# PolyChord/PolyChordLite

Measured on AMD Instinct MI355X. Metric: likelihood evals/sec, 20D Gaussian nlive=2000, higher is better.
Workload: dtype f64; 1 GPU; configs[1]: 20-D Gaussian, nlive=2000, num_repeats=40, one full run per step; batch_chains=1000, parallelism=repeat-sharded x1, mode=one run at a time per GPU; R runs in step: roofline.in_step

## Files before the change

include/polychord_hip.h:

```cpp
#ifndef POLYCHORD_HIP_H
#define POLYCHORD_HIP_H
#include <stdbool.h>
#ifdef __cplusplus
extern "C" {
#endif


typedef double (*polychord_loglike_fn)(double *theta, int nDims, double *phi, int nDerived);
typedef void (*polychord_prior_fn)(double *cube, double *theta, int nDims);
typedef void (*polychord_dumper_fn)(int ndead, int nlive, int npars, double *live, double *dead,
                                    double *logweights, double logZ, double logZerr);

void polychord_c_interface(
    polychord_loglike_fn loglikelihood, polychord_prior_fn prior, polychord_dumper_fn dumper,
    int nlive, int num_repeats, int nprior, int nfail, bool do_clustering, int feedback,
    double precision_criterion, double logzero, int max_ndead, double boost_posterior,
    bool posteriors, bool equals, bool cluster_posteriors, bool write_resume, bool write_paramnames,
    bool read_resume, bool write_stats, bool write_live, bool write_dead, bool write_prior,
    bool maximise, double compression_factor, bool synchronous, int nDims, int nDerived,
    char *base_dir, char *file_root, int nGrade, double *grade_frac, int *grade_dims, int n_nlives,
    double *loglikes, int *nlives, int seed, int *comm);

void polychord_c_interface_ini(polychord_loglike_fn loglikelihood, void (*setup_loglikelihood)(void),
                               char *inifile, int *comm);


enum { PCHIP_LIKE_CALLBACK = 0, PCHIP_LIKE_GAUSSIAN = 1, PCHIP_LIKE_RASTRIGIN = 2,
       PCHIP_LIKE_TWIN_GAUSSIAN = 3, PCHIP_LIKE_CORR_GAUSSIAN = 4, PCHIP_LIKE_SOURCE = 5 };

double polychord_hip_gaussian(double *theta, int nDims, double *phi, int nDerived);
double polychord_hip_rastrigin(double *theta, int nDims, double *phi, int nDerived);
double polychord_hip_twin_gaussian(double *theta, int nDims, double *phi, int nDerived);
double polychord_hip_corr_gaussian(double *theta, int nDims, double *phi, int nDerived);
void polychord_hip_set_gaussian(double mu, double sigma);
void polychord_hip_set_corr_gaussian(int nDims, const double *invcov_rowmajor, const double *mean, double logdetcov);
void polychord_hip_uniform_prior(double *cube, double *theta, int nDims);
void polychord_hip_set_uniform_prior(int nDims, const double *lo, const double *hi);
enum { PCHIP_PT_UNIFORM = 1, PCHIP_PT_LOG_UNIFORM = 2, PCHIP_PT_POWER_UNIFORM = 3, PCHIP_PT_GAUSSIAN = 4, PCHIP_PT_HALF_GAUSSIAN = 5,
       PCHIP_PT_EXPONENTIAL = 6, PCHIP_PT_SORTED_UNIFORM = 7, PCHIP_PT_SORTED_GAUSSIAN = 8, PCHIP_PT_SORTED_HALF_GAUSSIAN = 9,
       PCHIP_PT_SORTED_EXPONENTIAL = 10 };
typedef struct {
    int type;
    int block;
    int npar;
    double par[3];
} pchip_prior_entry;
void polychord_hip_table_prior(double *cube, double *theta, int nDims);
int  polychord_hip_set_table_prior(int nDims, const pchip_prior_entry *entries, const int *hyper);
typedef void (*polychord_batch_fn)(void *user, int n, int nDims, int nDerived, const double *cube, double *theta, double *phi,
                                   double *logL);
void polychord_hip_set_batch_callback(polychord_batch_fn fn, void *user);
void polychord_hip_request_stop(void);
int polychord_hip_resume_copy(const char *in, const char *out, int *counts);
int polychord_hip_ini_prior(const char *inifile, const double *cube, double *theta, int n);
double polychord_hip_inv_normal_cdf(double p);
void polychord_hip_set_option(const char *name, double value);
void polychord_hip_set_sub_clustering(int n, const int *dims);
int polychord_hip_ini_sub_clustering(const char *inifile, int *dims, int cap);
const char *polychord_hip_last_error(void);
void pchip_inject_fault(int kind);
void pchip_set_capacity(int clusters, int phantom_rows);
void pchip_trim_cache(void);

typedef struct {
    int nDims, nDerived;
    int nlive, num_repeats, nprior, nfail;
    int do_clustering;
    double precision_criterion, logzero;
    int max_ndead;
    double boost_posterior;
    int posteriors, equals, cluster_posteriors;
    double compression_factor;
    int n_nlives; const double *loglikes; const int *nlives;
    int seed;
    int batch;
    int device;
    int feedback;
    int profile;
    int force_general;
    int ablate;
    const char *resume_write;
    int sequential_rng;
    const char *resume_read;
    int nGrade; const int *grade_dims; const int *grade_repeats;
    int epoch_discard;
    int device_records;
    int n_sub_cluster; const int *sub_cluster_dims;
} pchip_settings;

typedef struct {
    int kind;
    double mu, sigma;
    const double *invcov;
    const double *mean;
    double logdetcov;
    polychord_loglike_fn fn;
    int source;
} pchip_like;

enum { PCHIP_PRIOR_CALLBACK = 0, PCHIP_PRIOR_BOX = 1, PCHIP_PRIOR_TABLE = 2, PCHIP_PRIOR_SOURCE = 3 };
typedef struct {
    int kind;
    const double *lo, *hi;
    polychord_prior_fn fn;
    const pchip_prior_entry *table;
    const int *hyper;
} pchip_prior;

typedef struct {
    double logZ, varlogZ;
    long ndead, nlike, niter, nbatches, nrounds, nupdates;
    int ncluster, ncluster_dead, nTotal, batch;
    double t_generate, t_loop, t_final, t_total;
    double t_setup, t_results, t_teardown;
    double k_time_s[8]; long k_launches[8];
    double *dead, *logweights;
    double *entry;
    double *live; int nlive_final;
    double *logZp, *varlogZp; int nZp;
    double *post_mean, *post_var;
    long nlike_grade[8];
    int *live_cluster;
    long nlike_failed;
    int ncluster_peak;
    int epoch_discard;
    double *d_records; long n_records, records_cap; int records_device;
    long path[24];
} pchip_result;
enum { PCHIP_PATH_CONSUME_PAR = 0,
       PCHIP_PATH_CONSUME_CL = 1,
       PCHIP_PATH_CONSUME_GENERAL = 2,
       PCHIP_PATH_CONSUME_FAST = 3,
       PCHIP_PATH_KILLOFF_PAR = 4, PCHIP_PATH_KILLOFF_CL = 5, PCHIP_PATH_KILLOFF_GENERAL = 6, PCHIP_PATH_KILLOFF_FAST = 7,
       PCHIP_PATH_UPDATE_FUSED = 8,
       PCHIP_PATH_UPDATE_STEPS = 9,
       PCHIP_PATH_SLICE_WAVE = 10,
       PCHIP_PATH_SLICE_LANE = 11,
       PCHIP_PATH_NN_LISTS = 12,
       PCHIP_PATH_NN_FALLBACKS = 13,
       PCHIP_PATH_POOL_MODE = 14,
       PCHIP_PATH_DEFER_UPDATE = 15,
       PCHIP_PATH_CONSUME_CL_SERIAL = 16,
       PCHIP_PATH_SUBCLUSTER_PASSES = 17,
       PCHIP_PATH_SUBCLUSTER_SPLITS = 18,
       PCHIP_PATH_SOURCE_KERNELS = 19,
       PCHIP_PATH_DEVICE_PRIOR = 20,
       PCHIP_PATH_SOURCE_TERMS = 21,
       PCHIP_PATH_SLICE_STEP = 22,
       PCHIP_PATH_COUNT = 24 };

typedef struct {
    int final_call;
    long ndiscarded;
    long ndead; int nlive, npars;
    const double *dead;
    const double *logpost;
    const double *live;
    const int *live_cluster;
    double logZ, logZerr;
    long nlike;
    int ngrade; const long *nlike_grade; const int *grade_dims, *grade_repeats;
    int ncluster, ncluster_dead;
    const int *nlive_p;
    const double *logZp, *logZperr;
    const double *logZp_dead, *logZperr_dead;
    const unsigned *dead_cluster;
    const unsigned *cluster_uid, *cluster_uid_dead;
    int nsplit;
    const unsigned *split_child, *split_parent;
    const double *split_logfrac;
    int n_extra; const double *extra, *extra_logpost; const unsigned *extra_cluster;
    const unsigned long long *extra_uid;
} pchip_update;
typedef void (*pchip_update_fn)(void *user, const pchip_update *u);

typedef struct {
    polychord_dumper_fn dumper;
    pchip_update_fn on_update;
    void *user;
} pchip_hooks;

#define PCHIP_ABI_VERSION 9
int  pchip_abi_version(void);
#define PCHIP_SOURCE_MAX_DERIVED 32
int  pchip_source_create(const char *source, const char *options, const double *data, long ndata);
void pchip_source_destroy(int handle);
int  pchip_source_create_terms(const char *source, const char *options, const double *data, long ndata, long nterms);
int  pchip_source_create_prior(const char *source, const char *options, const double *data, long ndata, long nterms);
int  pchip_source_prior_eval(int handle, const double *cubes, long n, int nDims, double *thetas);
int  pchip_source_eval(int handle, const double *thetas, long n, int nDims, int nDerived, double *logL, double *phi);
unsigned long pchip_sizeof(const char *struct_name);
void pchip_settings_default(pchip_settings *s, int nDims, int nDerived);
int  pchip_device_count(void);
int  pchip_run(const pchip_settings *s, const pchip_like *like, const pchip_prior *prior, pchip_result *out);
int  pchip_run_hooks(const pchip_settings *s, const pchip_like *like, const pchip_prior *prior,
                     const pchip_hooks *hooks, pchip_result *out);
void pchip_result_free(pchip_result *r);
int  pchip_maximise(polychord_loglike_fn loglikelihood, polychord_prior_fn prior, int nDims, int nDerived, double logzero,
                    const double *live, const int *live_cluster, int nlive, const double *post_mean, const char *path);
typedef struct {
    double logZ, varlogZ;
    long n; int nTotal, nruns;
    double *rows;
    double *logweights;
    int *nlive;
    double *post_mean, *post_var;
    double t_merge_s, t_runs_s;
    long nlike, ndead_all;
    double runs_logZ_mean, runs_logZ_sem;
    double logZ_replay, varlogZ_replay;
    int evidence_rule, nclustered;
} pchip_merged;
int  pchip_merge_records(int nDims, int nDerived, int nruns, const long *counts, const double *rows, const double *entry,
                         int on_device, int want_rows, pchip_merged *out);
int  pchip_merge_records_ex(int nDims, int nDerived, int nruns, const long *counts, const double *rows, const double *entry,
                            const double *ownw, const double *run_logZ, const double *run_varlogZ, const int *run_clustered,
                            int on_device, int want_rows, pchip_merged *out);
void pchip_merged_free(pchip_merged *m);
int  pchip_merged_write(const pchip_merged *m, int nDims, int nDerived, const char *base_dir, const char *file_root);
int  pchip_run_repeats(const pchip_settings *s, const pchip_like *like, const pchip_prior *prior, int nseeds, const int *seeds,
                       int ndevices, const int *devices, int max_in_flight, pchip_result *results, pchip_merged *merged);
int  pchip_run_repeats_ex(const pchip_settings *s, const pchip_like *like, const pchip_prior *prior, int nseeds, const int *seeds,
                          int ndevices, const int *devices, int max_in_flight, int want_rows, pchip_result *results, pchip_merged *merged);
int  pchip_run_in_step(const pchip_settings *s, const pchip_like *like, const pchip_prior *prior, int nseeds, const int *seeds,
                       int ndevices, const int *devices, int max_in_flight, int want_rows, pchip_result *results, pchip_merged *merged);

typedef struct pchip_comm pchip_comm;
#define PCHIP_COMM_ID_BYTES 128
int  pchip_comm_get_id(char *id128);
int  pchip_comm_create(const char *id128, int nranks, int rank, int device, pchip_comm **out);
void pchip_comm_destroy(pchip_comm *c);
int  pchip_comm_merge(pchip_comm *c, const pchip_result *run, double logzero, int nDims, int nDerived, int want_rows,
                      pchip_merged *out);
int  pchip_comm_merge_many(pchip_comm *c, const pchip_result *runs, int nruns, double logzero, int nDims, int nDerived, int want_rows,
                           pchip_merged *out);
typedef int (*pchip_allgather_fn)(void *user, const void *send, void *recv, unsigned long bytes);
int  pchip_comm_create_with(pchip_allgather_fn all_gather, void *user, int nranks, int rank, int device, pchip_comm **out);
const char *pchip_comm_library(void);

int  pchip_slice_chains(const pchip_settings *s, const pchip_like *like, const pchip_prior *prior,
                        unsigned batch, int nchains, const double *seeds, const double *chol,
                        double contour, double *babies_out, double *nhats_out, int *nlike_out);
int  pchip_prior_transform(const pchip_prior *prior, int nDims, int n, const double *cube, double *theta, int device);
int  pchip_update_factors(const pchip_settings *s, int ncluster, int nlive, const double *live, const int *live_cluster,
                          int nph, const double *phantom, const double *ph_logL, const int *ph_cluster, const double *threshold,
                          const double *shift, int path, double *cov, double *chol, int *count, double *shift_out, int *chol_suspect);

#ifdef __cplusplus
}
#endif
#endif
```

polychordlite_amd/_ctypes_api.py:

```python
import ctypes as C
import os

import numpy as np

_HERE = os.path.dirname(os.path.abspath(__file__))
LIB_PATH = os.environ.get("PCHIP_LIB") or os.path.join(_HERE, "libpolychord_hip.so")

LOGLIKE_FN = C.CFUNCTYPE(C.c_double, C.POINTER(C.c_double), C.c_int, C.POINTER(C.c_double), C.c_int)
PRIOR_FN = C.CFUNCTYPE(None, C.POINTER(C.c_double), C.POINTER(C.c_double), C.c_int)
DUMPER_FN = C.CFUNCTYPE(None, C.c_int, C.c_int, C.c_int, C.POINTER(C.c_double), C.POINTER(C.c_double),
                        C.POINTER(C.c_double), C.c_double, C.c_double)

LIKE_CALLBACK, LIKE_GAUSSIAN, LIKE_RASTRIGIN, LIKE_TWIN_GAUSSIAN, LIKE_CORR_GAUSSIAN, LIKE_SOURCE = range(6)
KERNEL_CLASSES = ("k_nhats", "k_slice", "k_consume", "k_apply", "k_clean", "k_covmats", "k_bases_side")
LIKE_KINDS = {"gaussian": LIKE_GAUSSIAN, "rastrigin": LIKE_RASTRIGIN, "twin_gaussian": LIKE_TWIN_GAUSSIAN,
              "corr_gaussian": LIKE_CORR_GAUSSIAN, "source": LIKE_SOURCE}


class Settings(C.Structure):
    _fields_ = [("nDims", C.c_int), ("nDerived", C.c_int), ("nlive", C.c_int), ("num_repeats", C.c_int),
                ("nprior", C.c_int), ("nfail", C.c_int), ("do_clustering", C.c_int),
                ("precision_criterion", C.c_double), ("logzero", C.c_double), ("max_ndead", C.c_int),
                ("boost_posterior", C.c_double), ("posteriors", C.c_int), ("equals", C.c_int),
                ("cluster_posteriors", C.c_int), ("compression_factor", C.c_double), ("n_nlives", C.c_int),
                ("loglikes", C.POINTER(C.c_double)), ("nlives", C.POINTER(C.c_int)), ("seed", C.c_int),
                ("batch", C.c_int), ("device", C.c_int), ("feedback", C.c_int), ("profile", C.c_int),
                ("force_general", C.c_int), ("ablate", C.c_int),
                ("resume_write", C.c_char_p), ("sequential_rng", C.c_int), ("resume_read", C.c_char_p),
                ("nGrade", C.c_int), ("grade_dims", C.POINTER(C.c_int)), ("grade_repeats", C.POINTER(C.c_int)),
                ("epoch_discard", C.c_int), ("device_records", C.c_int),
                ("n_sub_cluster", C.c_int), ("sub_cluster_dims", C.POINTER(C.c_int))]


class Like(C.Structure):
    _fields_ = [("kind", C.c_int), ("mu", C.c_double), ("sigma", C.c_double), ("invcov", C.POINTER(C.c_double)),
                ("mean", C.POINTER(C.c_double)), ("logdetcov", C.c_double), ("fn", C.c_void_p),
                ("source", C.c_int)]


class PriorEntry(C.Structure):
    _fields_ = [("type", C.c_int), ("block", C.c_int), ("npar", C.c_int), ("par", C.c_double * 3)]


class Prior(C.Structure):
    _fields_ = [("kind", C.c_int), ("lo", C.POINTER(C.c_double)), ("hi", C.POINTER(C.c_double)), ("fn", C.c_void_p),
                ("table", C.POINTER(PriorEntry)), ("hyper", C.POINTER(C.c_int))]


PRIOR_CALLBACK, PRIOR_BOX, PRIOR_TABLE, PRIOR_SOURCE = 0, 1, 2, 3
PRIOR_TYPES = {"uniform": 1, "log_uniform": 2, "power_uniform": 3, "gaussian": 4, "half_gaussian": 5, "exponential": 6,
               "sorted_uniform": 7, "sorted_gaussian": 8, "sorted_half_gaussian": 9, "sorted_exponential": 10}


class Result(C.Structure):
    _fields_ = [("logZ", C.c_double), ("varlogZ", C.c_double), ("ndead", C.c_long), ("nlike", C.c_long),
                ("niter", C.c_long), ("nbatches", C.c_long), ("nrounds", C.c_long), ("nupdates", C.c_long),
                ("ncluster", C.c_int), ("ncluster_dead", C.c_int), ("nTotal", C.c_int), ("batch", C.c_int),
                ("t_generate", C.c_double), ("t_loop", C.c_double), ("t_final", C.c_double), ("t_total", C.c_double),
                ("t_setup", C.c_double), ("t_results", C.c_double), ("t_teardown", C.c_double),
                ("k_time_s", C.c_double * 8), ("k_launches", C.c_long * 8),
                ("dead", C.POINTER(C.c_double)), ("logweights", C.POINTER(C.c_double)), ("entry", C.POINTER(C.c_double)),
                ("live", C.POINTER(C.c_double)), ("nlive_final", C.c_int),
                ("logZp", C.POINTER(C.c_double)), ("varlogZp", C.POINTER(C.c_double)), ("nZp", C.c_int),
                ("post_mean", C.POINTER(C.c_double)), ("post_var", C.POINTER(C.c_double)),
                ("nlike_grade", C.c_long * 8), ("live_cluster", C.POINTER(C.c_int)),
                ("nlike_failed", C.c_long), ("ncluster_peak", C.c_int), ("epoch_discard", C.c_int),
                ("d_records", C.c_void_p), ("n_records", C.c_long), ("records_cap", C.c_long), ("records_device", C.c_int),
                ("path", C.c_long * 24)]


PATH_NAMES = ("consume_par", "consume_cl", "consume_general", "consume_fast", "killoff_par", "killoff_cl", "killoff_general",
              "killoff_fast", "update_fused", "update_steps", "slice_wave", "slice_lane", "nn_lists", "nn_fallbacks", "pool_mode",
              "defer_update", "consume_cl_serial", "subcluster_passes", "subcluster_splits", "source_kernels", "device_prior", "source_terms", "slice_step")


_lib = None


def load():
    global _lib
    if _lib is not None:
        return _lib
    if not os.path.exists(LIB_PATH):
        raise ImportError(f"{LIB_PATH} is missing: build it with `python -m polychordlite_amd.build` "
                          "(hipcc --offload-arch=gfx950).  There is no CPU fallback.")
    lib = C.CDLL(LIB_PATH, mode=C.RTLD_GLOBAL)
    lib.pchip_settings_default.argtypes = [C.POINTER(Settings), C.c_int, C.c_int]
    lib.pchip_settings_default.restype = None
    lib.pchip_device_count.restype = C.c_int
    lib.pchip_run.argtypes = [C.POINTER(Settings), C.POINTER(Like), C.POINTER(Prior), C.POINTER(Result)]
    lib.pchip_run.restype = C.c_int
    lib.pchip_result_free.argtypes = [C.POINTER(Result)]
    lib.pchip_result_free.restype = None
    lib.pchip_slice_chains.argtypes = [C.POINTER(Settings), C.POINTER(Like), C.POINTER(Prior), C.c_uint, C.c_int,
                                       C.POINTER(C.c_double), C.POINTER(C.c_double), C.c_double,
                                       C.POINTER(C.c_double), C.POINTER(C.c_double), C.POINTER(C.c_int)]
    lib.pchip_slice_chains.restype = C.c_int
    lib.polychord_hip_set_gaussian.argtypes = [C.c_double, C.c_double]
    lib.polychord_hip_set_uniform_prior.argtypes = [C.c_int, C.POINTER(C.c_double), C.POINTER(C.c_double)]
    lib.polychord_hip_set_corr_gaussian.argtypes = [C.c_int, C.POINTER(C.c_double), C.POINTER(C.c_double), C.c_double]
    lib.polychord_hip_set_option.argtypes = [C.c_char_p, C.c_double]
    lib.polychord_hip_set_sub_clustering.argtypes = [C.c_int, C.POINTER(C.c_int)]
    lib.polychord_hip_set_sub_clustering.restype = None
    lib.polychord_hip_ini_sub_clustering.argtypes = [C.c_char_p, C.POINTER(C.c_int), C.c_int]
    lib.polychord_hip_ini_sub_clustering.restype = C.c_int
    lib.pchip_source_create.argtypes = [C.c_char_p, C.c_char_p, C.POINTER(C.c_double), C.c_long]
    lib.pchip_source_create.restype = C.c_int
    lib.pchip_source_create_terms.argtypes = [C.c_char_p, C.c_char_p, C.POINTER(C.c_double), C.c_long, C.c_long]
    lib.pchip_source_create_terms.restype = C.c_int
    lib.pchip_source_create_prior.argtypes = [C.c_char_p, C.c_char_p, C.POINTER(C.c_double), C.c_long, C.c_long]
    lib.pchip_source_create_prior.restype = C.c_int
    lib.pchip_source_prior_eval.argtypes = [C.c_int, C.POINTER(C.c_double), C.c_long, C.c_int, C.POINTER(C.c_double)]
    lib.pchip_source_prior_eval.restype = C.c_int
    lib.pchip_source_eval.argtypes = [C.c_int, C.POINTER(C.c_double), C.c_long, C.c_int, C.c_int, C.POINTER(C.c_double), C.POINTER(C.c_double)]
    lib.pchip_source_eval.restype = C.c_int
    lib.pchip_source_destroy.argtypes = [C.c_int]
    lib.pchip_source_destroy.restype = None
    lib.pchip_rtc_embedded_source.argtypes = [C.c_int, C.POINTER(C.c_char_p)]
    lib.pchip_rtc_embedded_source.restype = C.c_char_p
    lib.pchip_rtc_compile_check.argtypes = [C.c_int, C.c_char_p, C.c_char_p, C.c_char_p, C.c_int, C.POINTER(C.c_double)]
    lib.pchip_rtc_compile_check.restype = C.c_int
    lib.pchip_rtc_stats.argtypes = [C.POINTER(C.c_long), C.POINTER(C.c_double)]
    lib.pchip_rtc_stats.restype = None
    lib.polychord_hip_last_error.restype = C.c_char_p
    lib.polychord_hip_set_table_prior.argtypes = [C.c_int, C.POINTER(PriorEntry), C.POINTER(C.c_int)]
    lib.polychord_hip_set_table_prior.restype = C.c_int
    lib.polychord_hip_table_prior.argtypes = [C.POINTER(C.c_double), C.POINTER(C.c_double), C.c_int]
    lib.polychord_hip_table_prior.restype = None
    lib.pchip_prior_transform.argtypes = [C.POINTER(Prior), C.c_int, C.c_int, C.POINTER(C.c_double), C.POINTER(C.c_double), C.c_int]
    lib.pchip_prior_transform.restype = C.c_int
    pi = C.POINTER(C.c_int); pd = C.POINTER(C.c_double)
    lib.pchip_update_factors.argtypes = [C.POINTER(Settings), C.c_int, C.c_int, pd, pi, C.c_int, pd, pd, pi, pd, pd, C.c_int, pd, pd, pi, pd, pi]
    lib.pchip_update_factors.restype = C.c_int
    lib.pchip_sizeof.argtypes = [C.c_char_p]
    lib.pchip_sizeof.restype = C.c_ulong
    for name, cls in (("settings", Settings), ("result", Result), ("like", Like), ("prior", Prior)):
        if lib.pchip_sizeof(name.encode()) != C.sizeof(cls):
            raise ImportError(f"{LIB_PATH}: pchip_{name} is {lib.pchip_sizeof(name.encode())} bytes, this binding's mirror {C.sizeof(cls)} "
                              f"(library ABI version {lib.pchip_abi_version()}): rebuild with `python -m polychordlite_amd.build`")
    _lib = lib
    return lib


def dptr(a):
    return a.ctypes.data_as(C.POINTER(C.c_double))


def source_create(source, options=(), data=None, nterms=None, prior=False):
    lib = load()
    d = None if data is None else np.ascontiguousarray(np.ravel(data), dtype=np.float64)
    opts = " ".join(options) if not isinstance(options, str) else options
    args = (source.encode(), opts.encode(), dptr(d) if d is not None and d.size else None, 0 if d is None else int(d.size))
    if prior:
        h = lib.pchip_source_create_prior(*args, 0 if nterms is None else int(nterms))
    else:
        h = lib.pchip_source_create(*args) if nterms is None else lib.pchip_source_create_terms(*args, int(nterms))
    if h <= 0:
        log = lib.polychord_hip_last_error()
        raise RuntimeError("device source does not compile:\n" + (log.decode(errors="replace") if log else "(no log)"))
    return h


def source_eval(handle, thetas, nDerived=0):
    lib = load()
    t = np.ascontiguousarray(np.atleast_2d(thetas), dtype=np.float64)
    logL = np.empty(t.shape[0])
    phi = np.empty((t.shape[0], nDerived))
    rc = lib.pchip_source_eval(handle, dptr(t), t.shape[0], t.shape[1], nDerived, dptr(logL), dptr(phi) if nDerived > 0 else None)
    if rc != 0:
        msg = lib.polychord_hip_last_error()
        raise RuntimeError(f"pchip_source_eval failed with code {rc}" + (": " + msg.decode(errors="replace") if rc == 1 and msg else ""))
    return logL, phi


def source_prior_eval(handle, cubes):
    lib = load()
    c = np.ascontiguousarray(np.atleast_2d(cubes), dtype=np.float64)
    th = np.empty_like(c)
    rc = lib.pchip_source_prior_eval(handle, dptr(c), c.shape[0], c.shape[1], dptr(th))
    if rc != 0:
        msg = lib.polychord_hip_last_error()
        raise RuntimeError(f"pchip_source_prior_eval failed with code {rc}" + (": " + msg.decode(errors="replace") if rc == 1 and msg else ""))
    return th


def prior_table(entries, hyper=None):
    arr = (PriorEntry * len(entries))()
    for i, e in enumerate(entries):
        t, block, pars = (e[0], 1, e[1]) if len(e) == 2 else e
        pars = [float(v) for v in np.atleast_1d(pars)]
        arr[i].type = PRIOR_TYPES[t] if isinstance(t, str) else int(t)
        arr[i].block, arr[i].npar = int(block), len(pars)
        for k, v in enumerate(pars[:3]):
            arr[i].par[k] = v
    hy = None if hyper is None else np.ascontiguousarray(hyper, dtype=np.int32)
    return arr, hy


def set_table_prior(entries, hyper=None):
    lib = load()
    arr, hy = prior_table(entries, hyper)
    if lib.polychord_hip_set_table_prior(len(arr), arr, hy.ctypes.data_as(C.POINTER(C.c_int)) if hy is not None else None) != 0:
        msg = lib.polychord_hip_last_error()
        raise ValueError(msg.decode(errors="replace") if msg else "prior table refused")


def table_prior(cube):
    lib = load()
    c = np.ascontiguousarray(cube, dtype=np.float64)
    th = np.empty_like(c)
    lib.polychord_hip_table_prior(dptr(c), dptr(th), int(c.size))
    return th


def prior_transform(entries, cubes, hyper=None, device=-1):
    lib = load()
    c = np.ascontiguousarray(np.atleast_2d(cubes), dtype=np.float64)
    th = np.empty_like(c)
    arr, hy = prior_table(entries, hyper)
    P = Prior()
    P.kind, P.table = PRIOR_TABLE, arr
    if hy is not None:
        P.hyper = hy.ctypes.data_as(C.POINTER(C.c_int))
    rc = lib.pchip_prior_transform(C.byref(P), c.shape[1], c.shape[0], dptr(c), dptr(th), device)
    if rc != 0:
        msg = lib.polychord_hip_last_error()
        raise RuntimeError(f"pchip_prior_transform failed with code {rc}" + (": " + msg.decode(errors="replace") if rc == 1 and msg else ""))
    return th


def update_factors(live, live_cluster, phantom, ph_logL, ph_cluster, threshold, path, shift=None, ablate=0, device=-1):
    lib = load()
    x = np.ascontiguousarray(np.atleast_2d(live), dtype=np.float64)
    D = x.shape[1]
    ph = np.ascontiguousarray(np.reshape(phantom, (-1, D)), dtype=np.float64)
    lc = np.ascontiguousarray(live_cluster, dtype=np.int32)
    pl = np.ascontiguousarray(ph_logL, dtype=np.float64)
    pc = np.ascontiguousarray(ph_cluster, dtype=np.int32)
    thr = np.ascontiguousarray(np.atleast_1d(threshold), dtype=np.float64)
    nc = thr.size
    assert lc.shape == (x.shape[0],) and pl.shape == (ph.shape[0],) and pc.shape == (ph.shape[0],)
    sh = None if shift is None else np.ascontiguousarray(shift, dtype=np.float64)
    assert sh is None or sh.shape == (D,)
    s = Settings(); lib.pchip_settings_default(C.byref(s), D, 0)
    s.ablate, s.device = ablate, device
    cov = np.full((nc, D, D), np.nan); chol = np.full((nc, D, D), np.nan)
    count = np.full(nc, -1, dtype=np.int32); sho = np.full(D, np.nan); sus = C.c_int(-1)
    ip = lambda a: a.ctypes.data_as(C.POINTER(C.c_int))
    rc = lib.pchip_update_factors(C.byref(s), nc, x.shape[0], dptr(x), ip(lc), ph.shape[0], dptr(ph), dptr(pl), ip(pc), dptr(thr),
                                  dptr(sh) if sh is not None else None, path, dptr(cov), dptr(chol), ip(count), dptr(sho), C.byref(sus))
    if rc != 0:
        msg = lib.polychord_hip_last_error()
        raise RuntimeError(f"pchip_update_factors failed with code {rc}" + (": " + msg.decode(errors="replace") if rc == 1 and msg else ""))
    return dict(cov=cov, chol=chol, count=count, shift=sho, chol_suspect=sus.value)


def make_problem(kind, nDims, nDerived=0, lo=None, hi=None, mu=0.5, sigma=0.1, invcov=None, mean=None, logdet=0.0, source=0,
                 prior_table=None, hyper=None, prior_source=False):
    keep = []
    L = Like()
    L.kind = LIKE_KINDS[kind]
    L.source = source
    L.mu, L.sigma, L.logdetcov = mu, sigma, logdet
    if invcov is not None:
        ic = np.ascontiguousarray(invcov, dtype=np.float64)
        mn = np.ascontiguousarray(mean, dtype=np.float64)
        keep += [ic, mn]
        L.invcov, L.mean = dptr(ic), dptr(mn)
    P = Prior()
    P.kind = 1
    if prior_source:
        P.kind = PRIOR_SOURCE
        return L, P, keep
    if prior_table is not None:
        arr, hy = globals()["prior_table"](prior_table, hyper)
        keep += [arr, hy]
        P.kind, P.table = PRIOR_TABLE, arr
        if hy is not None:
            P.hyper = hy.ctypes.data_as(C.POINTER(C.c_int))
        return L, P, keep
    if lo is not None:
        lo_a = np.ascontiguousarray(np.broadcast_to(lo, (nDims,)), dtype=np.float64)
        hi_a = np.ascontiguousarray(np.broadcast_to(hi, (nDims,)), dtype=np.float64)
        keep += [lo_a, hi_a]
        P.lo, P.hi = dptr(lo_a), dptr(hi_a)
    return L, P, keep


def set_grades(settings, dims, repeats):
    gd = np.array(dims, dtype=np.int32)
    gr = np.array(repeats, dtype=np.int32)
    settings.nGrade = len(dims)
    settings.grade_dims = gd.ctypes.data_as(C.POINTER(C.c_int))
    settings.grade_repeats = gr.ctypes.data_as(C.POINTER(C.c_int))
    return gd, gr


def set_sub_clustering(settings, dims):
    sd = np.array(list(dims), dtype=np.int32)
    settings.n_sub_cluster = len(sd)
    settings.sub_cluster_dims = sd.ctypes.data_as(C.POINTER(C.c_int)) if len(sd) else None
    return sd


class _Owner:

    def __init__(self, lib, res):
        self.lib, self.res = lib, res

    def __del__(self):
        try:
            self.lib.pchip_result_free(C.byref(self.res))
        except Exception:
            pass


class _View:

    def __init__(self, owner, ptr, shape):
        self.owner = owner
        addr = C.cast(ptr, C.c_void_p).value or 0
        self.__array_interface__ = {"data": (addr, False), "shape": tuple(shape), "typestr": "<f8", "version": 3}


def _view(owner, ptr, shape):
    if int(np.prod(shape)) == 0:
        return np.zeros(shape)
    return np.asarray(_View(owner, ptr, shape))


def run(settings, like, prior):
    lib = load()
    r = Result()
    rc = lib.pchip_run(C.byref(settings), C.byref(like), C.byref(prior), C.byref(r))
    if rc != 0:
        raise RuntimeError(f"pchip_run failed with code {rc}")
    return result_dict(r, settings)


def result_dict(r, settings):
    lib = load()
    own = _Owner(lib, r)
    nT, nd, D = r.nTotal, r.ndead, settings.nDims
    out = dict(logZ=r.logZ, logZerr=float(np.sqrt(abs(r.varlogZ))), varlogZ=r.varlogZ, ndead=nd, nlike=r.nlike,
               niter=r.niter, nbatches=r.nbatches, nrounds=r.nrounds, nupdates=r.nupdates, ncluster=r.ncluster,
               ncluster_dead=r.ncluster_dead, nTotal=nT, batch=r.batch, t_generate=r.t_generate, t_loop=r.t_loop,
               t_final=r.t_final, t_total=r.t_total, t_setup=r.t_setup, t_results=r.t_results, t_teardown=r.t_teardown,
               kernel_time={n: {"total_s": r.k_time_s[i], "launches": r.k_launches[i]}
                            for i, n in enumerate(KERNEL_CLASSES) if r.k_launches[i] > 0},
               dead=_view(own, r.dead, (nd, nT)),
               logweights=_view(own, r.logweights, (nd,)),
               entry=_view(own, r.entry, (nd,)),
               live=_view(own, r.live, (r.nlive_final, nT)),
               logZp=np.ctypeslib.as_array(r.logZp, shape=(max(r.nZp, 1),))[:r.nZp].copy(),
               post_mean=np.ctypeslib.as_array(r.post_mean, shape=(D + settings.nDerived,)).copy(),
               post_var=np.ctypeslib.as_array(r.post_var, shape=(D + settings.nDerived,)).copy(),
               nlike_grade=[int(v) for v in r.nlike_grade], nlike_failed=r.nlike_failed, ncluster_peak=r.ncluster_peak, epoch_discard=r.epoch_discard, n_records=int(r.n_records) if r.d_records else None,
               path={n: int(r.path[i]) for i, n in enumerate(PATH_NAMES)},
               varlogZp=np.ctypeslib.as_array(r.varlogZp, shape=(max(r.nZp, 1),))[:r.nZp].copy(),
               logzero=settings.logzero,
               _owner=own)
    return out
```

polychordlite_amd/csrc/pc_engine.hip:

```cpp
#include "pc_state.h"
#include "pc_resume.h"
#include "pc_prior_table.h"
#include "pc_launch.h"
#include "pc_plan.h"
#include <cstdio>
#include <cstdlib>
#include <cstring>
#include <cstdarg>
#include <cstdint>
#include <new>
#include <cmath>
#include <vector>
#include <memory>
#include <string>
#include <chrono>
#include <algorithm>
#include <map>
#include <unordered_map>
#include <atomic>
#include <mutex>
#include <thread>
#include <functional>
#include <exception>
#include <ucontext.h>
// ... 212 lines not shown
    return two < 170e-6;
}
struct StreamClasses {
    std::mutex mm;
    std::map<void *, int> cls;
    std::vector<hipStream_t> reps;
    int known(hipStream_t x) { std::lock_guard<std::mutex> g(mm); auto it = cls.find((void *)x); return it == cls.end() ? -1 : it->second; }
    int classify(hipStream_t x)
    {
        std::lock_guard<std::mutex> g(mm);
        auto it = cls.find((void *)x);
        if (it != cls.end()) return it->second;
        int c = -1;
        for (size_t r = 0; r < reps.size() && c < 0; ++r) if (!streams_overlap_test(reps[r], x)) c = (int)r;
        if (c < 0) { c = (int)reps.size(); reps.push_back(x); }
        cls[(void *)x] = c;
        return c;
    }
};
static StreamClasses &sclasses() { static StreamClasses *p = new StreamClasses; return *p; }
static hipStream_t stream_avoiding(std::vector<int> avoid, bool known_only = false);
static hipStream_t stream_beside(std::initializer_list<hipStream_t> others, bool known_only = false)
{
    if (pc_env().side_pick_off) return hpool().get_stream();
    std::vector<int> avoid;
    for (hipStream_t o : others) if (o) { const int c = known_only ? sclasses().known(o) : sclasses().classify(o); if (c >= 0) avoid.push_back(c); }
    return stream_avoiding(avoid, known_only);
}
static hipStream_t stream_avoiding(std::vector<int> avoid, bool known_only)
{
    auto fits = [&](int c) { return c >= 0 && std::find(avoid.begin(), avoid.end(), c) == avoid.end(); };
    if (hipStream_t k = hpool().take_stream_if([&](hipStream_t x) { return fits(sclasses().known(x)); })) return k;
    if (known_only) {
        if (hipStream_t k = hpool().take_stream_if([&](hipStream_t x) { return sclasses().known(x) >= 0; })) return k;
        return hpool().get_stream();
    }
    std::vector<hipStream_t> tried;
    hipStream_t pick = nullptr;
    for (int k = 0; k < 8 && !pick; ++k) {
        hipStream_t c = hpool().take_stream_if([&](hipStream_t x) { return sclasses().known(x) < 0; });
        const bool dbg = pc_env().debug == 5;
        const auto q0 = std::chrono::steady_clock::now();
        const bool made = !c;
        if (!c) { HIPCHK(hipStreamCreate(&c)); }
        const auto q1 = std::chrono::steady_clock::now();
        const int cc = sclasses().classify(c);
        if (dbg) std::fprintf(stderr, "polychord_hip dbg stream_beside: try %d, %s stream %p (%.2f ms), class %d (%.2f ms), avoid %d\n", k, made ? "new" : "pooled", (void *)c, std::chrono::duration<double>(q1 - q0).count() * 1e3, cc, std::chrono::duration<double>(std::chrono::steady_clock::now() - q1).count() * 1e3, avoid.empty() ? -1 : avoid[0]);
        if (fits(cc)) pick = c; else tried.push_back(c);
    }
    if (!pick) { pick = tried.back(); tried.pop_back(); }
    for (hipStream_t t : tried) hpool().put_stream(t);
    return pick;
}
static hipStream_t side_stream_for(hipStream_t main_st) { return stream_beside({main_st}); }
struct CohortStreams {
    std::mutex m;
    std::vector<std::pair<int, int>> used;
    std::vector<int> busy(int dev, bool mains_only = false)
    {
        std::vector<int> b;
        for (auto &u : used) if (u.first == dev && (!mains_only || u.second >= 1000)) b.push_back(u.second % 1000);
        return b;
    }
    void take(int dev, int c, bool main_stream = false) { if (c >= 0) used.emplace_back(dev, c + (main_stream ? 1000 : 0)); }
    void give(int dev, int c, bool main_stream = false)
    {
        if (c < 0) return;
        const int v = c + (main_stream ? 1000 : 0);
        for (size_t i = 0; i < used.size(); ++i) if (used[i].first == dev && used[i].second == v) { used.erase(used.begin() + (long)i); return; }
    }
};
static CohortStreams &cstreams() { static CohortStreams *p = new CohortStreams; return *p; }
struct CohortLease {
    int dev, cls_main = -1, cls_side = -1; bool held = false;
    explicit CohortLease(int d) : dev(d) {}
    void hold(int cm, int cs) { cls_main = cm; cls_side = cs; held = true; }
    void release() { if (!held) return; held = false; std::lock_guard<std::mutex> gq(cstreams().m); cstreams().give(dev, cls_main, true); cstreams().give(dev, cls_side); }
    ~CohortLease() { release(); }
};
extern "C" void pc_prepare_streams(int dev, int want)
{
    if (hipSetDevice(dev) != hipSuccess) return;
    (void)hipDeviceSynchronize();
    std::lock_guard<std::mutex> gq(cstreams().m);
    std::vector<hipStream_t> have;
    while (hipStream_t k = hpool().take_stream_if([](hipStream_t x) { return sclasses().known(x) >= 0; })) have.push_back(k);
    for (int tries = 0; (int)have.size() < want && tries < 4 * want; ++tries) {
        hipStream_t c = hpool().take_stream_if([](hipStream_t x) { return sclasses().known(x) < 0; });
        if (!c && hipStreamCreate(&c) != hipSuccess) break;
        (void)sclasses().classify(c);
        have.push_back(c);
    }
    for (hipStream_t k : have) hpool().put_stream(k);
}
std::atomic<int> g_active_runs{0};
std::atomic<int> g_active_dev[64];

struct Timing { double t_gen = 0, t_loop = 0, t_final = 0, t_total = 0; long rounds = 0, updates = 0, batches = 0, compactions = 0; };

enum { KT_NHATS = 0, KT_SLICE, KT_CONSUME, KT_APPLY, KT_CLEAN, KT_COV, KT_SIDE , KT_N };
struct KTimer {
    bool on = false;
    unsigned mask = 0xFFFFFFFFu;
    unsigned stride = 1; unsigned seen[KT_N] = {0};
    hipStream_t st = nullptr;
    std::vector<hipEvent_t> pool; size_t used = 0;
    struct Span { int k; hipEvent_t a, b; bool side; };
    std::vector<Span> open;
    double total_ms[KT_N] = {0}; long launches[KT_N] = {0};
    hipEvent_t get() { if (used == pool.size()) pool.push_back(hpool().get_event()); return pool[used++]; }
    hipEvent_t begin(int k) { if (!on || !((mask >> k) & 1u) || (seen[k]++ % stride) != 0 || open.size() >= MAX_OPEN) return nullptr; hipEvent_t e = get(); HIPCHK(hipEventRecord(e, st)); return e; }
    void end(int k, hipEvent_t a) { if (!on || !a) return; hipEvent_t e = get(); HIPCHK(hipEventRecord(e, st)); open.push_back({k, a, e, false}); }
    hipEvent_t begin_on(int k, hipStream_t s2) { if (!on || !((mask >> k) & 1u) || (seen[k]++ % stride) != 0 || open.size() >= MAX_OPEN) return nullptr; hipEvent_t e = get(); HIPCHK(hipEventRecord(e, s2)); return e; }
    void end_on(int k, hipEvent_t a, hipStream_t s2) { if (!on || !a) return; hipEvent_t e = get(); HIPCHK(hipEventRecord(e, s2)); open.push_back({k, a, e, true}); }
    static constexpr size_t MAX_OPEN = 8192;
    void collect() {
        if (!on) return;
        for (auto &sp : open) { float ms = 0; if (sp.side) HIPCHK(hipEventSynchronize(sp.b)); HIPCHK(hipEventElapsedTime(&ms, sp.a, sp.b)); total_ms[sp.k] += ms; launches[sp.k]++; }
        open.clear(); used = 0;
    }
    void destroy() { for (auto e : pool) hpool().put_event(e); pool.clear(); }
};

static void h_philox(uint32_t c0, uint32_t c1, uint32_t c2, uint32_t c3, uint32_t k0, uint32_t k1, uint32_t o[4])
{
    for (int r = 0; r < 10; ++r) {
        const uint64_t p0 = (uint64_t)0xD2511F53u * c0, p1 = (uint64_t)0xCD9E8D57u * c2;
        const uint32_t n0 = (uint32_t)(p1 >> 32) ^ c1 ^ k0, n1 = (uint32_t)p1, n2 = (uint32_t)(p0 >> 32) ^ c3 ^ k1, n3 = (uint32_t)p0;
        c0 = n0; c1 = n1; c2 = n2; c3 = n3; k0 += 0x9E3779B9u; k1 += 0xBB67AE85u;
    }
    o[0] = c0; o[1] = c1; o[2] = c2; o[3] = c3;
}
static double h_uniform(uint32_t k0, uint32_t k1, uint32_t dom, uint32_t shi, uint32_t slo, uint32_t idx)
{
    uint32_t o[4];
    h_philox(idx >> 1, slo, shi, dom, k0, k1, o);
    const uint64_t w = (idx & 1u) ? (((uint64_t)o[2] << 32) | o[3]) : (((uint64_t)o[0] << 32) | o[1]);
    return ((double)(w >> 11) + 0.5) * (1.0 / 9007199254740992.0);
}

#include "pc_fiber.h"

#include "pc_cohort.h"

#include "pc_split.h"

struct DbgSpan {
    std::atomic<long long> &ns; std::chrono::steady_clock::time_point t0 = std::chrono::steady_clock::now();
    ~DbgSpan() { ns += std::chrono::duration_cast<std::chrono::nanoseconds>(std::chrono::steady_clock::now() - t0).count(); }
};
static std::atomic<long long> g_dbg_compact_ns{0}, g_dbg_nursery_ns{0}, g_dbg_capacity_ns{0}, g_dbg_endb_ns{0}, g_dbg_destroy_ns{0}, g_dbg_evwait_ns{0}, g_dbg_d1{0}, g_dbg_d2{0};
struct Engine {
    Cohort *co = nullptr;
    Fiber *fib = nullptr;
    pchip_settings cfg{};
    std::atomic<int> stop{0};
    polychord_batch_fn batch_fn = nullptr; void *batch_user = nullptr;
    polychord_loglike_fn cb_like = nullptr; polychord_prior_fn cb_prior = nullptr;
    bool callback_mode = false;
    void *d_cs = nullptr; double *d_x0s = nullptr, *d_prop = nullptr;
    int *d_decks = nullptr;
    double *hp_prop = nullptr, *hp_ans = nullptr, *d_ans = nullptr; int *hp_need = nullptr;
    long long cb_evals = 0; long cb_ticks = 0;
    std::vector<int> cb_idx; std::vector<double> cb_c, cb_t, cb_p, cb_l;
    polychord_dumper_fn dumper = nullptr;
    pchip_update_fn on_update = nullptr; void *hook_user = nullptr;
    long ndiscarded = 0;
    bool resume_static = true; unsigned resume_batch0 = 0;
    bool nph_stale = false;
    std::vector<double> hm_dead, hm_logw; int hm_ndead = 0;
    std::vector<unsigned> hm_cuid;
    std::vector<double> pp_rows, pp_logpost; std::vector<unsigned> pp_cuid; std::vector<unsigned long long> pp_uid; int nd_last_update = 0;
    std::vector<unsigned> split_child, split_parent; std::vector<double> split_logfrac;
    std::vector<double> h_lo, h_hi;
    PcState S{};
    hipStream_t st = nullptr;
    hipStream_t st_copy = nullptr;
    bool st_copy_shared = false;
    hipStream_t st_side = nullptr;
    hipEvent_t ev_main = nullptr;
    static constexpr int RAW_RING = 4;
    struct RawSlot { hipEvent_t ready = nullptr, consumed = nullptr; unsigned batch = 0; int B = 0; bool valid = false, waited = false, used = false; int co_seq = 0; };
    RawSlot ring[RAW_RING];
    int raw_depth = 2;
    double *h_dead = nullptr; size_t h_dead_cap = 0, h_dead_copied = 0;
    PcCtl *h_ctl = nullptr;
    PcCtl *h_note = nullptr;
    unsigned note_seq = 0;
    hipEvent_t ev_apply = nullptr;
    double *raw_buf[RAW_RING] = {nullptr, nullptr, nullptr, nullptr};
    double *ph2 = nullptr, *phL2 = nullptr; unsigned *phC2 = nullptr; unsigned long long *phU2 = nullptr;
    unsigned char *keep = nullptr; int *blk = nullptr, *d_total = nullptr;
    double *psum = nullptr, *mean = nullptr, *pcov = nullptr; int *pcnt = nullptr, *count = nullptr;
    size_t cov_chunks_cap = 0;
    double *upd_part = nullptr, *upd_shift = nullptr; size_t upd_part_cap = 0;
    PcPriorTable ptab; bool have_ptab = false;
    double *d_lo = nullptr, *d_hi = nullptr, *d_invcovT = nullptr, *d_mean = nullptr, *d_src = nullptr;
    double *d_dynL = nullptr; int *d_dynN = nullptr; double *d_logn = nullptr;
    ClusterUpdate<Engine> clus{*this};
    Engine() = default; Engine(const Engine &) = delete; Engine &operator=(const Engine &) = delete;
    std::vector<int> sub_dims; int *c_subdims = nullptr;
    long nsplits = 0; int ncluster_peak = 1;
    bool src_terms = false;
    long path[PCHIP_PATH_COUNT] = {};
    Cohort::Note step_note;
    Timing tm;
    KTimer kt;
    int B = 0, dev = 0;
    bool cb_auto_batch = false; int B_small = 1; double cb_eval_seconds = -1.0;
    long long nlike_g[PC_MAX_GRADE] = {0};
    std::vector<int> h_nlike_g;

    void alloc_phantom_side(int Pcap)
    {
        ph2 = dalloc<double>((size_t)Pcap * S.nT); phL2 = dalloc<double>(Pcap); phC2 = dalloc<unsigned>(Pcap);
        phU2 = dalloc<unsigned long long>(Pcap); keep = dalloc<unsigned char>(Pcap); blk = dalloc<int>((Pcap + 255) / 256 + 1);
    }

    std::vector<void *> setup_staged;
    void upload(void *dst, const void *src, size_t bytes)
    {
        void *h = halloc<char>(bytes);
        setup_staged.push_back(h);
        std::memcpy(h, src, bytes);
        HIPCHK(hipMemcpyAsync(dst, h, bytes, hipMemcpyHostToDevice, st));
    }
    void setup(const pchip_settings &c, const pchip_like &like, const pchip_prior &prior)
    {
        cfg = c;
        { std::lock_guard<std::mutex> g(g_cb_mutex); batch_fn = g_batch_fn; batch_user = g_batch_user; }
        int ndev = 0;
        if (hipGetDeviceCount(&ndev) != hipSuccess || ndev == 0) {
            engine_fail(PC_RC_DEVICE, "no HIP device available -- this engine has no CPU path");
        }
        dev = c.device >= 0 ? c.device % ndev : 0;
        HIPCHK(hipSetDevice(dev));
        st = co ? co->st : hpool().get_stream();
        st_copy = (co && co->stc[0]) ? co->stc[(co->n_stc++) & 1] : (co ? hpool().get_stream() : stream_beside({st}));
        st_copy_shared = co && co->stc[0];
        kt.on = c.profile != 0 && !co; kt.st = st;
        kt.mask = (c.profile == 1) ? 0xFFFFFFFFu : (((unsigned)c.profile >> 1) & 0x7Fu);
        kt.stride = std::max(1u, ((unsigned)c.profile >> 8) & 0xFFu);
        const int D = c.nDims, nDer = c.nDerived;
        S.D = D; S.nDer = nDer; S.nT = 2 * D + nDer + 2; S.nr = c.num_repeats; S.N = c.nlive;
        S.ngrade = 1; S.g_off[0] = 0; S.g_nr[0] = c.num_repeats;
        for (int g = 1; g < PC_MAX_GRADE; ++g) { S.g_off[g] = 0; S.g_nr[g] = 0; }
        if (c.nGrade > 1 && c.grade_dims && c.grade_repeats) {
            if (c.nGrade > PC_MAX_GRADE) engine_fail(PC_RC_SETTINGS, "at most %d parameter grades", PC_MAX_GRADE);
            S.ngrade = c.nGrade;
            int off = 0, tot = 0;
            for (int g = 0; g < c.nGrade; ++g) {
                if (c.grade_dims[g] < 1 || c.grade_repeats[g] < 1) engine_fail(PC_RC_SETTINGS, "every grade needs at least one parameter and one repeat");
                S.g_off[g] = off; off += c.grade_dims[g]; S.g_nr[g] = c.grade_repeats[g]; tot += c.grade_repeats[g];
            }
            if (off != D) engine_fail(PC_RC_SETTINGS, "grade_dims must sum to nDims");
            S.nr = tot; cfg.num_repeats = tot;
        }
        S.nb_total = 0; S.n_dev = 0;
        for (int g = 0, col = 0; g < PC_MAX_GRADE; ++g) {
            const int Dg = D - S.g_off[g];
            S.g_nb[g] = g < S.ngrade ? (S.g_nr[g] + Dg - 1) / Dg : 0;
            S.g_col0[g] = col; S.g_e0[g] = (int)S.n_dev;
            col += S.g_nr[g]; S.nb_total += S.g_nb[g]; S.n_dev += (unsigned)S.g_nb[g] * Dg * Dg;
        }
        sub_dims.clear();
        if (c.n_sub_cluster < 0 || (c.n_sub_cluster > 0 && !c.sub_cluster_dims)) engine_fail(PC_RC_SETTINGS, "n_sub_cluster = %d without a list of coordinates", c.n_sub_cluster);
        for (int k = 0; k < c.n_sub_cluster; ++k) {
            const int d = c.sub_cluster_dims[k];
            if (d < 0 || d >= D) engine_fail(PC_RC_SETTINGS, "sub-clustering coordinate %d out of range (nDims = %d; the indices are 0-based)", d, D);
            if (std::find(sub_dims.begin(), sub_dims.end(), d) != sub_dims.end()) engine_fail(PC_RC_SETTINGS, "sub-clustering coordinate %d given twice", d);
            sub_dims.push_back(d);
        }
        S.ch_nlike_g = nullptr;
        std::memset(nlike_g, 0, sizeof(nlike_g));
        S.p0 = D; S.d0 = 2 * D; S.b0 = 2 * D + nDer; S.l0 = S.b0 + 1;
        int nmax = c.nlive;
        for (int i = 0; i < c.n_nlives; ++i) nmax = std::max(nmax, c.nlives[i]);
        const int nprior = c.nprior <= 0 ? c.nlive : c.nprior;
        S.Ncap = std::max(nmax, nprior);
        B = c.batch > 0 ? c.batch : std::max(1, std::min(1024, c.nlive / 2));
        if (B > 65535) engine_fail(PC_RC_LIMIT, "batch = %d chains per nursery: at most 65535", B);
        if (c.sequential_rng) B = 1;
        cb_auto_batch = c.batch <= 0 && !c.sequential_rng && (like.kind == PC_LIKE_CALLBACK || (prior.kind != 1 && prior.kind != PCHIP_PRIOR_TABLE && prior.kind != PCHIP_PRIOR_SOURCE));
        if (cb_auto_batch) B_small = std::max(1, std::min(64, c.nlive / 4));
        S.B = B;
        S.maxc = c.do_clustering ? std::max(2, g_cap_clusters.load()) : 4;
        S.maxc_dead = 4096;
        S.Pcap = (int)std::min<long long>(2000000000LL / S.nT, 4LL * S.nr * S.Ncap + 4LL * B * S.nr + 1024);
        if (g_cap_phantoms.load() > 0) S.Pcap = std::max(g_cap_phantoms.load(), B * S.nr + 16);
        S.Dcap = 64 * S.Ncap + 4 * B + 1024;
        S.k0 = (uint32_t)c.seed; S.k1 = 0x504F4C59u;
        S.logzero = c.logzero; S.use_prec = c.precision_criterion > 0;
        S.log_prec = S.use_prec ? std::log(c.precision_criterion) : 0.0;
        S.log_cf = std::log(c.compression_factor);
        S.max_ndead = c.max_ndead; S.nfail = c.nfail <= 0 ? c.nlive : c.nfail;
        S.seed_override = 0; S.ablate = c.ablate; S.seq_mode = c.sequential_rng ? 1 : 0;
        S.epoch_discard = c.epoch_discard ? 1 : 0;
        if (S.seq_mode) { cfg.batch = 1; cfg.force_general = 1; }
        S.n_nlives = c.n_nlives;
        if (c.n_nlives > 0) {
            d_dynL = dalloc<double>(c.n_nlives); d_dynN = dalloc<int>(c.n_nlives);
            upload(d_dynL, c.loglikes, sizeof(double) * c.n_nlives);
            upload(d_dynN, c.nlives, sizeof(int) * c.n_nlives);
        }
        S.dyn_loglikes = d_dynL; S.dyn_nlives = d_dynN;
        S.like.kind = like.kind; S.like.mu = like.mu; S.like.sigma = like.sigma; S.like.logdetcov = like.logdetcov;
// ... 875 lines not shown
    void write_resume()
    {
        if (!cfg.resume_write) return;
        PcResume r;
        export_resume(r);
        std::string err;
        if (!pc_resume_write(cfg.resume_write, r, cfg.logzero, err)) engine_fail(PC_RC_RESUME, "%s", err.c_str());
        write_sidecar(std::string(cfg.resume_write) + ".hip", r.ndead, r.ncluster, r.ncluster_dead);
    }

    bool import_resume(const PcResume &r, std::string &err)
    {
        const int D = S.D, nT = S.nT, nc = r.ncluster, Ncap = S.Ncap;
        if (r.nDims != D || r.nDerived != S.nDer) { err = "resume file has different nDims / nDerived"; return false; }
        if (nc > S.maxc) grow_clusters(nc);
        if (r.ncluster_dead + nc + 8 > S.maxc_dead) grow_dead_clusters(2 * (r.ncluster_dead + nc + 8));
        const int maxc = S.maxc;
        int ntot = 0, nph = 0;
        for (int c = 0; c < nc; ++c) { ntot += r.nlive[c]; nph += r.nphantom[c]; }
        if (ntot > Ncap || (nc >= 1 && ntot < 1)) { err = "resume file: live point counts do not fit this run's settings"; return false; }
        if (nph + (long long)B * S.nr > S.Pcap) { h_ctl->nphantom = 0; grow_phantoms(nph + (long long)B * S.nr); }
        if ((long long)r.ndead + B + Ncap + 16 > S.Dcap) { h_ctl->ndead = 0; grow_dead(2 * (r.ndead + B + Ncap + 16)); }
        std::vector<double> rows((size_t)Ncap * nT, 0.0), lL(Ncap, PC_HUGE), entry(Ncap, cfg.logzero);
        std::vector<int> lc(Ncap, -1), lp(Ncap, 0), cl((size_t)maxc * Ncap, 0), cn(maxc, 0), imin(maxc, 0);
        std::vector<unsigned> uid(maxc, 0u);
        const Sidecar sc = cfg.resume_read ? read_sidecar(std::string(cfg.resume_read) + ".hip", r.ndead, nc, std::min(r.ncluster_dead, S.maxc_dead)) : Sidecar{};
        std::vector<double> logLp(maxc, cfg.logzero), lref(maxc, 0.0), lsum(maxc, 0.0);
        int slot = 0;
        for (int c = 0; c < nc; ++c) {
            cn[c] = r.nlive[c]; uid[c] = sc.ok ? sc.uid[c] : (unsigned)(c + 1);
            double lo = PC_HUGE, hi = -PC_HUGE;
            for (int k = 0; k < r.nlive[c]; ++k, ++slot) {
                const double *row = r.live[c].data() + (size_t)k * nT;
                std::memcpy(rows.data() + (size_t)slot * nT, row, sizeof(double) * nT);
                lL[slot] = row[S.l0]; lc[slot] = c; lp[slot] = k; entry[slot] = row[S.b0]; cl[(size_t)c * Ncap + k] = slot;
                if (row[S.l0] < lo) { lo = row[S.l0]; imin[c] = slot; }
                hi = std::max(hi, row[S.l0]);
            }
            logLp[c] = r.nlive[c] ? lo : cfg.logzero;
            lref[c] = r.nlive[c] ? hi : 0.0;
            for (int k = 0; k < r.nlive[c]; ++k) lsum[c] += std::exp(r.live[c][(size_t)k * nT + S.l0] - lref[c]);
        }
        ul(S.live, rows); ul(S.live_logL, lL); ul(S.live_entry, entry); ul(S.live_cluster, lc); ul(S.live_pos, lp);
        { std::vector<int> none(Ncap, -1); ul(S.slot_src, none); }
        ul(S.cl_list, cl); ul(S.cl_n, cn); ul(S.cl_uid, uid); ul(S.imin_slot, imin); ul(S.logLp, logLp); ul(S.lse_ref, lref); ul(S.lse_sum, lsum);
        auto put = [&](double *dst, const std::vector<double> &v) { std::vector<double> t(maxc, cfg.logzero); std::copy(v.begin(), v.end(), t.begin()); ul(dst, t); };
        put(S.logZp, r.logZp); put(S.logZXp, r.logZXp); put(S.logZp2, r.logZp2); put(S.logZpXp, r.logZpXp);
        { std::vector<double> t(maxc, 0.0); std::copy(r.logXp.begin(), r.logXp.end(), t.begin()); ul(S.logXp, t); }
        std::vector<double> xq((size_t)maxc * maxc, 0.0);
        for (int q = 0; q < nc; ++q) for (int p = 0; p < nc; ++p) xq[(size_t)p * maxc + q] = r.logXpXq[(size_t)q * nc + p];
        ul(S.XpXq, xq);
        std::vector<double> cov((size_t)maxc * D * D, 0.0), ch((size_t)maxc * D * D, 0.0);
        for (int c = 0; c < maxc; ++c) for (int a = 0; a < D; ++a) { cov[((size_t)c * D + a) * D + a] = 1.0; ch[((size_t)c * D + a) * D + a] = 1.0; }
        for (int c = 0; c < nc; ++c) for (int j = 0; j < D; ++j) for (int a = 0; a < D; ++a) {
            cov[((size_t)c * D + a) * D + j] = r.covmat[((size_t)c * D + j) * D + a];
            ch[((size_t)c * D + a) * D + j] = r.cholesky[((size_t)c * D + j) * D + a];
        }
        ul(S.cov, cov); ul(S.chol, ch);
        const int ncd = std::min(r.ncluster_dead, S.maxc_dead);
        { std::vector<double> a(r.logZp_dead.begin(), r.logZp_dead.begin() + ncd), b(r.logZp2_dead.begin(), r.logZp2_dead.begin() + ncd); ul(S.logZp_dead, a); ul(S.logZp2_dead, b); }
        if (sc.ok) ul(S.cl_uid_dead, sc.uid_dead);
        std::vector<double> ph((size_t)std::max(1, nph) * nT), phL(std::max(1, nph));
        std::vector<unsigned> phC(std::max(1, nph)); std::vector<unsigned long long> phU(std::max(1, nph));
        int j = 0;
        for (int c = 0; c < nc; ++c)
            for (int k = 0; k < r.nphantom[c]; ++k, ++j) {
                std::memcpy(ph.data() + (size_t)j * nT, r.phantom[c].data() + (size_t)k * nT, sizeof(double) * nT);
                phL[j] = ph[(size_t)j * nT + S.l0]; phC[j] = uid[c]; phU[j] = 0xFFFFFFFF00000000ull | (unsigned)j;
            }
        if (nph) { ul(S.phantom, ph); ul(S.ph_logL, phL); ul(S.ph_cuid, phC); ul(S.ph_uid, phU); }
        if (r.ndead) {
            ul(S.dead, r.dead); ul(S.dead_logw, r.logweights);
            std::vector<double> z(r.ndead, 0.0), en(r.ndead);
            for (int i = 0; i < r.ndead; ++i) en[i] = r.dead[(size_t)i * nT + S.b0];
            ul(S.dead_postX, z); ul(S.dead_postZ, z); ul(S.dead_entry, en);
            std::vector<unsigned> du(r.ndead, 0u);
            if (sc.ok) du = sc.dead_cuid;
            ul(S.dead_cuid, du);
        }
        PcCtl c0 = *h_ctl;
        c0.status = nc >= 1 ? PC_ST_RUNNING : PC_ST_DONE; c0.ncluster = nc; c0.ncluster_dead = ncd; c0.ndead = r.ndead; c0.nphantom = nph;
        c0.logZ = r.logZ; c0.logZ2 = r.logZ2; c0.logX_last_update = r.logX_last_update; c0.next_cluster_uid = sc.ok ? sc.next_uid : (unsigned)nc + 1;
        c0.nlike = 0;
        for (size_t g = 0; g < r.nlike.size(); ++g) { c0.nlike += r.nlike[g]; if (g >= 1 && g < PC_MAX_GRADE) nlike_g[g] = r.nlike[g]; }
        c0.nlike_device = c0.nlike; c0.i_nursery = 0; c0.failures = 0;
        HIPCHK(hipMemcpy(S.ctl, &c0, sizeof(PcCtl), hipMemcpyHostToDevice));
        *h_ctl = c0;
        return true;
    }

    struct ActiveRun {
        int d; std::atomic<int> *flag;
        ActiveRun(int dv, std::atomic<int> *f) : d(dv & 63), flag(f) { g_active_runs.fetch_add(1); g_active_dev[d].fetch_add(1); std::lock_guard<std::mutex> g(g_run_mutex); g_run_stop.push_back(flag); }
        ~ActiveRun() { g_active_runs.fetch_sub(1); g_active_dev[d].fetch_sub(1); std::lock_guard<std::mutex> g(g_run_mutex); g_run_stop.erase(std::find(g_run_stop.begin(), g_run_stop.end(), flag)); }
    };
    std::unique_ptr<ActiveRun> active_run;
    using clk = std::chrono::steady_clock;
    clk::time_point r_t0, r_t1, r_t2;
    unsigned r_batch = 0; bool r_sort_valid = false, r_fresh = false; int r_nursery_left = 0;
    PcRunPlan plan{};
    int r_rc = 0;

    int run(pchip_result *out)
    {
        int rc = begin();
        if (rc >= 0) return rc;
        while (true) {
            if (!round_enqueue()) break;
            while (!round_ready()) __builtin_ia32_pause();
            if (!round_finish()) break;
        }
        if (r_rc != 0) return r_rc;
        return end(out);
    }

    int begin()
    {
        active_run.reset(new ActiveRun(dev, &stop));
        r_t0 = clk::now();
        h_dead_cap = (size_t)S.Dcap; h_dead = halloc<double>(h_dead_cap * S.nT); h_dead_copied = 0;
        bool resumed = false;
        if (cfg.resume_read) {
            if (FILE *probe = std::fopen(cfg.resume_read, "r")) {
                std::fclose(probe);
                PcResume rs; std::string err;
                if (!pc_resume_read(cfg.resume_read, rs, err) || !import_resume(rs, err)) { std::fprintf(stderr, "polychord_hip: %s\n", err.c_str()); return 6; }
                resumed = true;
                int ntot = 0;
                for (int v : rs.nlive) ntot += v;
                if (ntot > cfg.nlive && rs.ncluster == 1) { pc_count(path, PcTrimLive{}); pc_launch_consume(&S, 2, 0, st); read_ctl(); ntot = cfg.nlive; }
                resume_static = (ntot == cfg.nlive);
                resume_batch0 = (unsigned)rs.ndead;
            }
        }
        if (!resumed) { if (callback_mode) generate_live_callback(); else generate_live(); }
        if (stop.load(std::memory_order_relaxed)) return 5;
        if (cb_auto_batch && !(cb_eval_seconds >= 0.0 && cb_eval_seconds < 2e-6)) { B = B_small; S.B = B; }
        r_t1 = clk::now();
        r_batch = resume_batch0;
        r_sort_valid = false;
        r_nursery_left = 0;
        make_plan();
        S.defer_update = plan.defer ? 1 : 0; S.pool = plan.pool ? 1 : 0;
        if (S.pool) {
            pool_cursor = h_ctl->nphantom;
            babies_own = S.babies;
            if (g_cap_phantoms.load() <= 0) {
                size_t free_b = 0, total_b = 0;
                (void)hipMemGetInfo(&free_b, &total_b);
                const double need = 2.0 * 2.0 * (double)S.Pcap * ((double)S.nT * 8.0 + 24.0);
                if (need < 0.4 * (double)free_b) grow_phantoms(2LL * S.Pcap);
            }
        }
        r_rc = 0;
        return -1;
    }

    void make_plan()
    {
        const int nprior0 = cfg.nprior <= 0 ? cfg.nlive : cfg.nprior;
        PcRunFacts f{};
        f.ablate = cfg.ablate; f.force_general = cfg.force_general;
        f.fixed_nlive = (cfg.n_nlives == 0) && (nprior0 >= cfg.nlive) && resume_static;
        f.par_fits = pc_par_fits(&S) != 0; f.fast_fits = pc_fast_fits(&S) != 0; f.fused_fits_one = pc_update_fused_ok(&S, 1) != 0;
        f.clustering = cfg.do_clustering != 0; f.boost = cfg.boost_posterior != 0.0;
        f.dumper = dumper != nullptr; f.on_update = on_update != nullptr; f.resume_write = cfg.resume_write != nullptr;
        f.seq_mode = S.seq_mode != 0; f.posteriors = cfg.posteriors || cfg.equals;
        f.callback = callback_mode;
        plan = pc_plan_run(f);
    }
    bool other_active() const { return g_active_dev[dev & 63].load(std::memory_order_relaxed) > 1; }
    bool cohort_general_ok() const
    {
        return !pc_env().cohort_general_off && S.ngrade <= 1 && !S.seq_mode && S.like.kind != PC_LIKE_CORR_GAUSSIAN && S.like.kind != PC_LIKE_CALLBACK;
    }
    PcNurseryFacts nursery_facts(unsigned batch) const
    {
        PcNurseryFacts f{};
        f.in_step = co != nullptr; f.other_active = other_active(); f.callback = callback_mode; f.D = S.D;
        f.ring = raw_buf[1] != nullptr;
        const RawSlot &rs = ring[batch % raw_depth];
        f.slot_ready = rs.valid && rs.batch == batch && rs.B == B;
        f.second_stream = co && co->st2 && raw_depth >= 2;
        f.splittable = pc_nhats_splittable(&S) != 0; f.fusable = pc_slice_fusable(&S) != 0; f.bases_t = pc_bases_t_ok(&S) != 0;
        f.slice_t = pc_slice_t_ok(&S, h_ctl->ncluster) != 0;
        f.cohort_general = cohort_general_ok();
        f.traits = launch_traits();
        return f;
    }
    bool enqueue_nursery()
    {
        unsigned &batch = r_batch; int &nursery_left = r_nursery_left;
        if (S.pool) {
            if (pool_cursor + (long long)B * S.nr > S.Pcap) pool_compact();
            S.pool_base = (int)pool_cursor; S.pool_rows = B * S.nr; S.babies = S.phantom + (size_t)pool_cursor * S.nT;
            pool_cursor += (long long)B * S.nr;
        }
        {
            hipEvent_t e0 = kt.begin(KT_NHATS);
            const PcNurseryChoice ch = pc_choose_nursery(plan, nursery_facts(batch));
            pc_count(path, ch);
            pc_count_step(path, ch);
            int bases_seq = 0;
            switch (ch.bases) {
            case PC_BASES_READY: case PC_BASES_PART1: case PC_BASES_PART1_STEP: {
                RawSlot &rs = ring[batch % raw_depth];
                S.nhat_raw = raw_buf[batch % raw_depth];
                if (ch.bases == PC_BASES_READY) { if (!rs.waited) HIPCHK(hipStreamWaitEvent(st, rs.ready, 0)); bases_seq = rs.co_seq; }
                else {
                    if (rs.valid) HIPCHK(hipStreamWaitEvent(st, rs.ready, 0));
                    if (ch.bases == PC_BASES_PART1_STEP) co->rec(rec_bases(S, batch, B));
                    else (void)pc_launch_nhats_part(&S, batch, B, 1, st, ch.packed ? 1 : 0);
                }
                rs.valid = false;
                if (ch.part2) { if (co) { co->flush(); co->wait_next(); } (void)pc_launch_nhats_part(&S, batch, B, 2, st, 0); }
                break;
            }
            case PC_BASES_NHATS_G: co->rec(rec_nhats_g(S, batch, B)); break;
            case PC_BASES_WHOLE:
                if (co) co->flush();
                if (pc_launch_nhats(&S, batch, B, st)) { std::fprintf(stderr, "polychord_hip: nDims unsupported\n"); r_rc = 3; return false; }
                break;
            }
            kt.end(KT_NHATS, e0);
            hipEvent_t e1 = kt.begin(KT_SLICE);
            switch (ch.sampler) {
            case PC_SAMPLER_CALLBACK:
                if (co) co->flush();
                slice_callback(batch);
                if (stop.load(std::memory_order_relaxed)) { r_rc = 5; return false; }
                break;
            case PC_SAMPLER_LANE: { Cohort::Rec r = rec_slice(S, batch, B, bases_seq); r.note = co ? &step_note : nullptr; (void)stage(r); break; }
            case PC_SAMPLER_WAVE_STEP: co->rec(rec_slice_g(S, batch, B, ch.fused, ch.fused ? bases_seq : 0, &step_note)); break;
            case PC_SAMPLER_WAVE:
                if (co) { co->flush(); co->wait_next(); }
                if (ch.fused ? pc_launch_slice_fused(&S, batch, B, st) : pc_launch_slice(&S, batch, B, st)) {
                    if (pc_rtc_wanted(&S) && pc_rtc_error()) { std::fprintf(stderr, "polychord_hip: %s\n", pc_rtc_error()); r_rc = 1; return false; }
                    std::fprintf(stderr, "polychord_hip: nDims unsupported\n"); r_rc = 3; return false;
                }
                break;
            }
            if (ch.ahead == PC_AHEAD_STEP) bases_ahead(batch);
            kt.end(KT_SLICE, e1);
            if (ch.ahead == PC_AHEAD_SIDE) side_prefetch(batch);
            if (S.ngrade > 1) HIPCHK(hipMemcpyAsync(h_nlike_g.data(), S.ch_nlike_g, sizeof(int) * h_nlike_g.size(), hipMemcpyDeviceToHost, st));
            batch++; tm.batches++;
            S.nn_valid = 0; nursery_left = B;
        }
        return true;
    }

    void bases_ahead(unsigned cur)
    {
        const unsigned x = cur + 1;
        RawSlot &rn = ring[x % raw_depth];
        if (rn.valid && rn.batch == x && rn.B == B) return;
        PcState S1 = S; S1.nhat_raw = raw_buf[x % raw_depth];
        co->rec(rec_bases_next(S1, x, B));
        rn.valid = true; rn.batch = x; rn.B = B; rn.waited = true; rn.co_seq = co->seq_for_next();
    }

    void ensure_side()
    {
        if (st_side) return;
        st_side = stream_beside({st, st_copy}); ev_main = hpool().get_sync_event();
        for (int r = 0; r < raw_depth; ++r) { ring[r].ready = hpool().get_sync_event(); ring[r].consumed = hpool().get_sync_event(); }
    }
    hipEvent_t ev_presort_a = nullptr, ev_presort_b = nullptr;
    bool presorted = false;
    void presort_live()
    {
        presorted = false;
        if (pc_env().presort_off || co || other_active() || callback_mode || S.seq_mode || !S.nn_list || h_ctl->ncluster < 2) return;
        ensure_side();
        if (!ev_presort_a) { ev_presort_a = hpool().get_sync_event(); ev_presort_b = hpool().get_sync_event(); }
        HIPCHK(hipEventRecord(ev_presort_a, st)); HIPCHK(hipStreamWaitEvent(st_side, ev_presort_a, 0));
        if (pc_launch_sort_live(&S, st_side) != 0) return;
        HIPCHK(hipEventRecord(ev_presort_b, st_side));
        presorted = true;
    }
    void side_prefetch(unsigned cur)
    {
        const unsigned batch = cur;
        {
        ensure_side();
        const bool side_free = pc_env().side_free || (S.D > 64 && !pc_env().side_ordered);
        RawSlot &cur = ring[batch % raw_depth];
        if (side_free) { HIPCHK(hipEventRecord(cur.consumed, st)); cur.used = true; }
        if (!side_free) { HIPCHK(hipEventRecord(ev_main, st)); HIPCHK(hipStreamWaitEvent(st_side, ev_main, 0)); }
        const unsigned xmax = batch + (unsigned)raw_depth - (side_free ? 0u : 1u);
        for (unsigned x = batch + 1; x <= xmax; ++x) {
            RawSlot &rs = ring[x % raw_depth];
            if (rs.valid && rs.batch == x && rs.B == B) continue;
            if (rs.valid) continue;
            if (rs.used) HIPCHK(hipStreamWaitEvent(st_side, rs.consumed, 0));
            PcState S1 = S; S1.nhat_raw = raw_buf[x % raw_depth];
            hipEvent_t es = kt.begin_on(KT_SIDE, st_side);
            (void)pc_launch_nhats_part(&S1, x, B, 1, st_side, (cfg.ablate & PC_ABL_BASES_PACKED) ? 1 : 0);
            kt.end_on(KT_SIDE, es, st_side);
            HIPCHK(hipEventRecord(rs.ready, st_side));
            rs.valid = true; rs.batch = x; rs.B = B; rs.waited = false;
        }
    }
    }

    PcContractFacts contract_facts(int nursery_left) const
    {
        PcContractFacts f{};
        f.ncluster = h_ctl->ncluster; f.nursery_left = nursery_left;
        f.in_step = co != nullptr; f.cohort_general = cohort_general_ok();
        f.nn_lists = S.nn_list && !pc_env().nn_lists_off; f.nn_valid = S.nn_valid != 0;
        f.cl_fits = f.ncluster > 1 && pc_consume_cl_fits(&S, f.ncluster) != 0;
        f.clp_fits = f.cl_fits && pc_consume_clp_fits(&S, f.ncluster) != 0;
        return f;
    }
    bool round_enqueue()
    {
        unsigned &batch = r_batch; bool &sort_valid = r_sort_valid; int &nursery_left = r_nursery_left;
        {
            if (h_ctl->status == PC_ST_DONE) return false;
            if (h_ctl->status == PC_ST_ERROR) { std::fprintf(stderr, "polychord_hip: device error %d\n", h_ctl->error); r_rc = 2; return false; }
            if (step_note.failed) {
                if (pc_rtc_wanted(&S) && pc_rtc_error()) { std::fprintf(stderr, "polychord_hip: %s\n", pc_rtc_error()); r_rc = 1; return false; }
                std::fprintf(stderr, "polychord_hip: nDims unsupported\n"); r_rc = 3; return false;
            }
            bool fresh_nursery = false;
            if (h_ctl->i_nursery == 0) {
                fresh_nursery = true;
                DbgSpan dbg_t{g_dbg_nursery_ns};
                if (plan.cl_ok) presort_live();
                if (!enqueue_nursery()) return false;
            }
            if (fresh_nursery) { DbgSpan dbg_t{g_dbg_capacity_ns}; ensure_capacity(); }
            hipEvent_t e2 = kt.begin(KT_CONSUME);
            int rc2 = 0;
            const PcContractChoice ch = pc_choose_contract(plan, contract_facts(nursery_left));
            pc_count(path, ch);
            launch_stamp();
            if (presorted && (co || !(h_ctl->ncluster > 1))) { HIPCHK(hipStreamWaitEvent(st, ev_presort_b, 0)); presorted = false; }
            switch (ch.kind) {
            case PC_CONTRACT_PAR:
                S.nn_valid = 0;
                if (!sort_valid) { rc2 = stage(rec_sort(S)); sort_valid = true; }
                rc2 = rc2 || stage(rec_consume(S));
                break;
            case PC_CONTRACT_FAST:
                if (co) co->flush();
                sort_valid = false; S.nn_valid = 0;
                rc2 = pc_launch_consume_fast(&S, 0, st); pc_launch_ph_prepare(&S, st);
                break;
            case PC_CONTRACT_CL_STEP:
                sort_valid = false;
                if (ch.want_nn) { co->rec(rec_nn(S, nursery_left)); S.nn_valid = 1; }
                co->rec(rec_sort(S));
                co->rec(rec_consume_cl(S, h_ctl->ncluster > 64));
                break;
            case PC_CONTRACT_CL: case PC_CONTRACT_GENERAL: {
                sort_valid = false;
                if (co) co->flush();
                bool sorted_now = false;
                if (presorted) { HIPCHK(hipStreamWaitEvent(st, ev_presort_b, 0)); sorted_now = fresh_nursery; presorted = false; }
                if (ch.want_nn) {
                    if (!sorted_now) sorted_now = pc_launch_sort_live(&S, st) == 0;
                    pc_launch_nn_lists(&S, nursery_left, sorted_now ? 1 : 0, st);
                    S.nn_valid = 1;
                }
                if (ch.kind == PC_CONTRACT_CL) rc2 = (sorted_now ? 0 : pc_launch_sort_live(&S, st)) || pc_launch_consume_cl(&S, h_ctl->ncluster, st);
                else rc2 = pc_launch_consume(&S, 0, (h_ctl->ncluster > 1) ? 1 : 0, st);
                break;
            }
            }
            if (rc2) { std::fprintf(stderr, "polychord_hip: nlive too large for the LDS-resident contraction\n"); r_rc = 4; return false; }
            kt.end(KT_CONSUME, e2);
            hipEvent_t e3 = kt.begin(KT_APPLY);
            (void)stage(rec_apply(S, batch - 1, B));
            kt.end(KT_APPLY, e3);
            if (st_side) { RawSlot &rs = ring[batch % raw_depth]; if (rs.valid && rs.batch == batch && !rs.waited) { HIPCHK(hipStreamWaitEvent(st, rs.ready, 0)); rs.waited = true; } }
            r_fresh = fresh_nursery;
            ready_spins = 0;
        }
        return true;
    }

    bool finish_may_wait() const
    {
        const bool upd = h_ctl->status == PC_ST_UPDATE || (h_ctl->upd_pending && h_ctl->status == PC_ST_RUNNING);
        return upd && pc_choose_update(plan, update_facts(1)).may_wait;
    }
    bool round_finish()
    {
        unsigned &batch = r_batch; int &nursery_left = r_nursery_left; const bool fresh_nursery = r_fresh;
        (void)batch;
        {
            if (fresh_nursery && h_ctl->status == PC_ST_DONE && h_ctl->i_nursery == B) tm.batches--;
            nursery_left = h_ctl->i_nursery;
            tally_grades();
            tm.rounds++;
            if (h_ctl->status == PC_ST_UPDATE || (h_ctl->upd_pending && h_ctl->status == PC_ST_RUNNING)) {
                do_update(h_ctl->status != PC_ST_UPDATE); h_ctl->status = PC_ST_RUNNING; h_ctl->upd_pending = 0;
                if ((size_t)h_ctl->ndead >= h_dead_copied + 4 * (size_t)cfg.nlive) {
                if (!ev_apply) ev_apply = hpool().get_sync_event();
                HIPCHK(hipEventRecord(ev_apply, st));
                stream_dead();
                }
            }
        }
        return true;
    }

    struct EndState {
        double *hlive = nullptr; int *hcl = nullptr; double *d_pmax = nullptr, *h_part = nullptr, *h_zp = nullptr;
        int nc_end = 0, ncd_max = 0, pmD = 0, pm_nb = 0, pm_pw = 0; clk::time_point t2;
    } es;
    hipStream_t st_fin = nullptr; hipEvent_t ev_fin = nullptr;
    void end_a(bool fused_final = false)
    {
        if (co && !fused_final) co->flush();
        bool &sort_valid = r_sort_valid;
        es.t2 = clk::now();
        st_fin = st;
        if (co && fused_final && !pc_env().cohort_final_aside_off && st_copy && st_copy != st && h_ctl->ncluster > 1) {
            ev_fin = hpool().get_sync_event();
            HIPCHK(hipEventRecord(ev_fin, st));
            HIPCHK(hipStreamWaitEvent(st_copy, ev_fin, 0));
            st_fin = st_copy;
        }
        hipStream_t st = st_fin;
        const int nT = S.nT;
        es.hlive = halloc<double>((size_t)S.Ncap * nT); es.hcl = halloc<int>(S.Ncap);
        HIPCHK(hipMemcpyAsync(es.hlive, S.live, sizeof(double) * (size_t)S.Ncap * nT, hipMemcpyDeviceToHost, st));
        HIPCHK(hipMemcpyAsync(es.hcl, S.live_cluster, sizeof(int) * S.Ncap, hipMemcpyDeviceToHost, st));
        es.nc_end = h_ctl->ncluster;
        if (h_ctl->ncluster == 0) {
        } else if (plan.par_ok && h_ctl->ncluster == 1) {
            path[PCHIP_PATH_KILLOFF_PAR]++;
            if (co && sort_valid) { co->rec(rec_final(S)); if (!fused_final) co->flush(); }
            else {
            if (!sort_valid) (void)pc_launch_sort_live(&S, st);
            (void)pc_launch_final_par(&S, st);
            }
        } else if (h_ctl->ncluster > 1 && pc_launch_killoff_cl(&S, h_ctl->ncluster, st) == 0) {
            path[PCHIP_PATH_KILLOFF_CL]++;
        } else if (plan.fast_ok && h_ctl->ncluster == 1 && pc_launch_consume_fast(&S, 1, st) == 0) path[PCHIP_PATH_KILLOFF_FAST]++;
        else { path[PCHIP_PATH_KILLOFF_GENERAL]++; pc_launch_consume(&S, 1, (h_ctl->ncluster > 1 && !S.seq_mode) ? 1 : 0, st); }
        if (!fused_final) end_a2();
    }
    void end_a2()
    {
        hipStream_t st = st_fin ? st_fin : this->st;
        es.pmD = S.D + S.nDer; es.pm_nb = pc_post_blocks(); es.pm_pw = 3 * es.pmD + 1;
        es.ncd_max = std::min(h_ctl->ncluster_dead + h_ctl->ncluster, S.maxc_dead);
        es.d_pmax = dalloc<double>(2 * (size_t)es.pm_nb); es.h_part = halloc<double>((size_t)es.pm_nb * es.pm_pw);
        es.h_zp = halloc<double>(2 * (size_t)std::max(1, es.ncd_max));
        pc_launch_post_moments(&S, -1, es.d_pmax, es.h_part, st);
        if (es.ncd_max > 0) {
            HIPCHK(hipMemcpyAsync(es.h_zp, S.logZp_dead, sizeof(double) * es.ncd_max, hipMemcpyDeviceToHost, st));
            HIPCHK(hipMemcpyAsync(es.h_zp + es.ncd_max, S.logZp2_dead, sizeof(double) * es.ncd_max, hipMemcpyDeviceToHost, st));
        }
        HIPCHK(hipMemcpyAsync(h_ctl, S.ctl, sizeof(PcCtl), hipMemcpyDeviceToHost, st));
        if (ev_fin) HIPCHK(hipEventRecord(ev_fin, st));
    }
    void end_wait_aside() { if (ev_fin) { HIPCHK(hipEventSynchronize(ev_fin)); hpool().put_sync_event(ev_fin); ev_fin = nullptr; } }
    int end(pchip_result *out) { end_a(); HIPCHK(hipStreamSynchronize(st)); end_wait_aside(); return end_b(out); }
    int end_b(pchip_result *out)
    {
        struct HostBuf { EndState &e; ~HostBuf() { if (e.hlive) hfree(e.hlive); if (e.hcl) hfree(e.hcl); e.hlive = nullptr; e.hcl = nullptr; } } hb{es};
        double *hlive = es.hlive; int *hcl = es.hcl; double *d_pmax = es.d_pmax, *h_part = es.h_part, *h_zp = es.h_zp;
        const int nc_end = es.nc_end, ncd_max = es.ncd_max, pmD = es.pmD, pm_nb = es.pm_nb, pm_pw = es.pm_pw, nT = S.nT;
        const auto t0 = r_t0, t1 = r_t1; auto t2 = es.t2;
        HIPCHK(hipGetLastError());
        nph_stale = false;
        kt.collect();
        if (cfg.boost_posterior != 0.0 && (cfg.posteriors || cfg.equals) && h_ctl->nphantom > 0) {
            pc_launch_clean(&S, h_ctl->nphantom, keep, blk, d_total, ph2, phL2, phC2, phU2, nullptr, st);
            collect_phantom_posteriors(h_ctl->nphantom);
        }
        call_dumper(1);
        write_resume();
        auto t3 = clk::now();
        tm.t_gen = std::chrono::duration<double>(t1 - t0).count();
        tm.t_loop = std::chrono::duration<double>(t2 - t1).count();
        tm.t_final = std::chrono::duration<double>(t3 - t2).count();
        tm.t_total = std::chrono::duration<double>(t3 - t0).count();
        std::memset(out, 0, sizeof(*out));
        out->logZ = std::max(-PC_HUGE, 2 * h_ctl->logZ - 0.5 * h_ctl->logZ2);
        out->varlogZ = h_ctl->logZ2 - 2 * h_ctl->logZ;
        out->ndead = h_ctl->ndead; out->nlike = h_ctl->nlike; out->niter = h_ctl->niter;
        out->nlike_failed = h_ctl->nlike_failed; out->ncluster_peak = ncluster_peak; out->epoch_discard = S.epoch_discard;
        path[PCHIP_PATH_NN_FALLBACKS] = (long)h_ctl->nn_fallbacks; path[PCHIP_PATH_POOL_MODE] = S.pool; path[PCHIP_PATH_DEFER_UPDATE] = S.defer_update;
        path[PCHIP_PATH_SLICE_STEP] = step_note.shared;
        for (int k = 0; k < PCHIP_PATH_COUNT; ++k) out->path[k] = path[k];
        grade_counts(out->nlike_grade);
        out->ncluster = nc_end; out->ncluster_dead = h_ctl->ncluster_dead; out->nbatches = tm.batches;
        out->nrounds = tm.rounds; out->nupdates = tm.updates; out->nTotal = nT; out->batch = B;
        out->t_generate = tm.t_gen; out->t_loop = tm.t_loop; out->t_final = tm.t_final; out->t_total = tm.t_total;
        for (int k = 0; k < KT_N; ++k) { out->k_time_s[k] = kt.total_ms[k] * 1e-3; out->k_launches[k] = kt.launches[k]; }
        const int dbg_lvl = pc_env().debug;
        if (dbg_lvl >= 3) std::fprintf(stderr, "polychord_hip dbg general: term %lld identify %lld kill+add %lld tail %lld cycles; %lld chains identified from the candidate lists, %lld of them fell back to the full search\n", h_ctl->gen_cyc[0], h_ctl->gen_cyc[1], h_ctl->gen_cyc[2], h_ctl->gen_cyc[3], h_ctl->nn_walks, h_ctl->nn_fallbacks);
        if (dbg_lvl == 4) std::fprintf(stderr, "polychord_hip dbg par: stage+search %lld rank-sort %lld accept %lld merge+slots %lld evidence %lld triggers %lld publish %lld cycles\n", h_ctl->dbg[0], h_ctl->dbg[1], h_ctl->dbg[2], h_ctl->dbg[3], h_ctl->dbg[4], h_ctl->dbg[5], h_ctl->dbg[6]);
        if (dbg_lvl == 4) std::fprintf(stderr, "polychord_hip dbg par: %lld evidence scans as pairs (terms beyond one scale)\n", h_ctl->dbg[7]);
        if (dbg_lvl == 4 && h_ctl->wave_cyc[0]) std::fprintf(stderr, "polychord_hip dbg clp (several clusters; the line above then reads: decisions | order of deaths + slots | counts + volumes | volume sum + step 0's phantoms | prefix sums + commit | waves 1-3 | write back | passes): wave 1 %lld wave 2 %lld wave 3 %lld phantom wave %lld cycles\n", h_ctl->wave_cyc[0], h_ctl->wave_cyc[1], h_ctl->wave_cyc[2], h_ctl->wave_cyc[3]);
        if (dbg_lvl == 2) std::fprintf(stderr, "polychord_hip dbg: loop cycles %lld passB %lld (%lld flushes) accept-steps %lld (%lld) ins-rescan %lld (%lld) reject-steps cycles %lld\n", h_ctl->dbg[0], h_ctl->dbg[1], h_ctl->dbg[4], h_ctl->dbg[2], h_ctl->dbg[3], h_ctl->dbg[5], h_ctl->dbg[6], h_ctl->dbg[7]);
        if ((size_t)h_ctl->ndead > h_dead_cap) {
            HIPCHK(hipStreamSynchronize(st_copy));
            hfree(h_dead); h_dead_cap = (size_t)h_ctl->ndead; h_dead = halloc<double>(h_dead_cap * nT); h_dead_copied = 0;
        }
        stream_dead();
        out->dead = h_dead; h_dead = nullptr;
        out->logweights = halloc<double>(std::max(1, h_ctl->ndead));
        HIPCHK(hipMemcpyAsync(out->logweights, S.dead_logw, sizeof(double) * h_ctl->ndead, hipMemcpyDeviceToHost, st_copy));
        out->entry = halloc<double>(std::max(1, h_ctl->ndead));
        HIPCHK(hipMemcpyAsync(out->entry, S.dead_entry, sizeof(double) * h_ctl->ndead, hipMemcpyDeviceToHost, st_copy));
        int nl = 0;
        for (int s = 0; s < S.Ncap; ++s) nl += hcl[s] >= 0;
        out->nlive_final = nl;
        out->live = (double *)std::malloc(sizeof(double) * (size_t)std::max(1, nl) * nT);
        out->live_cluster = (int *)std::malloc(sizeof(int) * (size_t)std::max(1, nl));
        for (int s = 0, k = 0; s < S.Ncap; ++s) if (hcl[s] >= 0) { std::memcpy(out->live + (size_t)k * nT, hlive + (size_t)s * nT, sizeof(double) * nT); out->live_cluster[k] = hcl[s]; k++; }
        const int ncd = std::min(h_ctl->ncluster_dead, S.maxc_dead);
        out->nZp = ncd;
        out->logZp = (double *)std::malloc(sizeof(double) * std::max(1, ncd));
        out->varlogZp = (double *)std::malloc(sizeof(double) * std::max(1, ncd));
        if (ncd > ncd_max) engine_fail(PC_RC_DEVICE, "more retired clusters (%d) than the final stage could have left (%d)", ncd, ncd_max);
        for (int i = 0; i < ncd; ++i) { const double zp = h_zp[i], zp2 = h_zp[ncd_max + i]; out->logZp[i] = 2 * zp - 0.5 * zp2; out->varlogZp[i] = zp2 - 2 * zp; }
        hfree(h_zp);
        const int D = pmD, nb = pm_nb, pw = pm_pw;
        out->post_mean = (double *)std::calloc(D, sizeof(double)); out->post_var = (double *)std::calloc(D, sizeof(double));
        double sw = 0.0;
        for (int b = 0; b < nb; ++b) {
            sw += h_part[(size_t)b * pw + 2 * D];
            for (int d = 0; d < D; ++d) { out->post_mean[d] += h_part[(size_t)b * pw + d]; out->post_var[d] += h_part[(size_t)b * pw + D + d]; }
        }
        for (int d = 0; d < D; ++d) {
            const double dm = out->post_mean[d] / sw;
            out->post_mean[d] = h_part[2 * D + 1 + d] + dm;
            out->post_var[d] = std::max(0.0, out->post_var[d] / sw - dm * dm);
        }
        dfree(d_pmax); hfree(h_part);
        long long *h_nrec = nullptr;
        if (cfg.device_records && h_ctl->ndead > 0) {
            const long long cap = h_ctl->ndead;
            double *blk_rec = (double *)pc_cache_dev_alloc(pc_records_block_bytes(cap, nT));
            if (!blk_rec) engine_fail(PC_RC_MEMORY, "no device memory for the run's records (%lld rows)", cap);
            h_nrec = halloc<long long>(1);
            if (pc_pack_lived_device(S.dead, S.dead_logw, S.dead_entry, cap, nT, cfg.logzero, blk_rec, cap, h_nrec, st_copy) != 0) { pc_cache_dev_free(blk_rec); hfree(h_nrec); engine_fail(PC_RC_DEVICE, "packing the run's records"); }
            out->d_records = blk_rec; out->records_cap = (long)cap; out->records_device = dev;
        }
        HIPCHK(hipStreamSynchronize(st_copy));
        if (h_nrec) { out->n_records = (long)*h_nrec; hfree(h_nrec); }
        active_run.reset();
        return 0;
    }

    void destroy(bool streams_idle = false)
    {
        active_run.reset();
        if (!streams_idle) {
        if (st) (void)hipStreamSynchronize(st);
        if (st_copy) (void)hipStreamSynchronize(st_copy);
        if (st_side) (void)hipStreamSynchronize(st_side);
        }
        const auto dq0 = std::chrono::steady_clock::now();
        std::vector<void *> blocks; blocks.reserve(160);
        struct Batch { std::vector<void *> &b; Batch(std::vector<void *> &v) : b(v) { tl_dfree_batch = &b; } ~Batch() { tl_dfree_batch = nullptr; dcache().put_many(b); b.clear(); } };
        {
        Batch batch_guard(blocks);
        if (raw_buf[0]) { S.nhat_raw = raw_buf[0]; for (int r = 1; r < RAW_RING; ++r) dfree(raw_buf[r]); raw_buf[0] = nullptr; }
        if (babies_own) { S.babies = babies_own; babies_own = nullptr; }
        double **dd[] = { &S.live, &S.live_logL, &S.logZp, &S.logXp, &S.logZXp, &S.logZp2, &S.logZpXp, &S.logLp, &S.XpXq,
                          &S.lse_ref, &S.lse_sum, &S.death_thr, &S.chol, &S.cov, &S.logZp_dead, &S.logZp2_dead, &S.phantom,
                          &S.ph_logL, &S.dead, &S.dead_logw, &S.dead_postX, &S.dead_postZ, &S.babies, &S.baby_logL, &S.baby_logL_T,
                          &S.ch_contour, &S.nhat, &S.nhat_w, &S.nhat_raw, &S.nhat_Ms, &S.ch_My, &S.live_entry, &S.dead_entry, &ph2, &phL2, &psum, &mean,
                          &pcov, &d_lo, &d_hi, &d_invcovT, &d_mean, &d_dynL, &d_src };
        for (auto p : dd) dfree(*p);
        int **ii[] = { &S.live_cluster, &S.live_pos, &S.cl_list, &S.cl_n, &S.imin_slot, &S.ch_cluster, &S.ch_epoch, &S.ch_nlike,
                       &S.ch_seed_slot, &S.slot_src, &S.slot_step, &S.slot_dead, &S.sort_slot, &blk, &d_total, &pcnt, &count, &d_dynN };
        for (auto p : ii) dfree(*p);
        { char *cs = (char *)d_cs; dfree(cs); d_cs = nullptr; }
        dfree(d_x0s); dfree(d_prop); dfree(d_ans); dfree(d_decks);
        if (hp_prop) { hfree(hp_prop); hp_prop = nullptr; } if (hp_ans) { hfree(hp_ans); hp_ans = nullptr; } if (hp_need) { hfree(hp_need); hp_need = nullptr; }
        dfree(upd_part); dfree(upd_shift); upd_part_cap = 0;
        clus.release(); dfree(c_subdims);
        for (void *h : staged_up) hfree(h);
        staged_up.clear();
        for (const Fetch &f : fetching) hfree(f.h);
        fetching.clear();
        dfree(d_logn); dfree(S.ch_nlike_g); dfree(S.nn_list); dfree(S.nn_slot_owner); dfree(S.nn_chain_slot); dfree(S.nn_pts); dfree(S.nn_code);
        unsigned **uu[] = { &S.cl_uid, &S.ph_cuid, &S.dead_cuid, &phC2, &S.cl_uid_dead };
        for (auto p : uu) dfree(*p);
        dfree(S.ph_uid); dfree(S.sort_key); dfree(S.plan); dfree(phU2); dfree(keep); dfree(S.ctl);
        }
        const auto dq1 = std::chrono::steady_clock::now();
        kt.destroy();
        if (h_dead) { hfree(h_dead); h_dead = nullptr; }
        for (void *h : setup_staged) hfree(h);
        setup_staged.clear();
        if (h_ctl) hfree(h_ctl); h_ctl = nullptr;
        if (h_note) hfree((void *)h_note); h_note = nullptr;
        if (ev_apply) { hpool().put_sync_event(ev_apply); ev_apply = nullptr; }

        if (st) { if (!streams_idle) (void)hipStreamSynchronize(st); if (!co) hpool().put_stream(st); } st = nullptr;
        if (st_copy) { if (!streams_idle) (void)hipStreamSynchronize(st_copy); if (!st_copy_shared) hpool().put_stream(st_copy); } st_copy = nullptr;
        if (st_side) {
            if (!streams_idle) (void)hipStreamSynchronize(st_side); hpool().put_stream(st_side); hpool().put_sync_event(ev_main);
            if (ev_presort_a) { hpool().put_sync_event(ev_presort_a); hpool().put_sync_event(ev_presort_b); ev_presort_a = ev_presort_b = nullptr; }
            for (int r = 0; r < RAW_RING; ++r) { if (ring[r].ready) hpool().put_sync_event(ring[r].ready); if (ring[r].consumed) hpool().put_sync_event(ring[r].consumed); ring[r] = RawSlot(); }
        }
        st_side = nullptr; ev_main = nullptr;
        const auto dq2 = std::chrono::steady_clock::now();
        g_dbg_d1 += std::chrono::duration_cast<std::chrono::nanoseconds>(dq1 - dq0).count();
        g_dbg_d2 += std::chrono::duration_cast<std::chrono::nanoseconds>(dq2 - dq1).count();
    }
};

}

#include "pc_step.h"

extern "C" {

void polychord_hip_request_stop(void) { std::lock_guard<std::mutex> g(g_run_mutex); for (auto *f : g_run_stop) f->store(1); }
void pchip_inject_fault(int kind) { g_inject_fault = kind; }
void *pc_cache_dev_alloc(size_t bytes) { try { return dcache().get(bytes); } catch (const EngineError &) { (void)hipGetLastError(); return nullptr; } }
void pc_cache_dev_free(void *p) { if (p && !dcache().put(p)) (void)hipFree(p); }
void *pc_cache_host_alloc(size_t bytes) { try { return hcache().get(bytes); } catch (const EngineError &) { (void)hipGetLastError(); return nullptr; } }
void pc_cache_host_free(void *p) { if (p && !hcache().put(p)) (void)hipHostFree(p); }
void pchip_trim_cache(void) { (void)hipDeviceSynchronize(); dcache().trim(); hcache().trim(); }
void pchip_set_capacity(int clusters, int phantom_rows) { if (clusters > 0) g_cap_clusters = clusters; if (phantom_rows >= 0) g_cap_phantoms = phantom_rows; }
void polychord_hip_set_batch_callback(polychord_batch_fn fn, void *user) { std::lock_guard<std::mutex> g(g_cb_mutex); g_batch_fn = fn; g_batch_user = user; }

double polychord_hip_keyed_uniform(unsigned seed, unsigned dom, unsigned shi, unsigned slo, unsigned idx)
{
    return h_uniform(seed, 0x504F4C59u, dom, shi, slo, idx);
}

void pchip_settings_default(pchip_settings *s, int nDims, int nDerived)
{
    std::memset(s, 0, sizeof(*s));
    s->nDims = nDims; s->nDerived = nDerived; s->nlive = 500; s->num_repeats = 5 * nDims; s->nprior = -1; s->nfail = -1;
    s->precision_criterion = 0.001; s->logzero = -1e30; s->max_ndead = -1; s->compression_factor = 0.36787944117144233;
    s->seed = -1; s->batch = 0; s->device = -1;
}

int pchip_device_count(void)
{
    int n = 0;
    if (hipGetDeviceCount(&n) != hipSuccess) return 0;
    return n;
}

int pchip_run(const pchip_settings *s, const pchip_like *like, const pchip_prior *prior, pchip_result *out)
{
    return pchip_run_hooks(s, like, prior, nullptr, out);
}

int pchip_run_hooks(const pchip_settings *s, const pchip_like *like, const pchip_prior *prior, const pchip_hooks *hooks, pchip_result *out)
{
    if (s->num_repeats < 1) { std::fprintf(stderr, "polychord_hip: You need to set num_repeats. Suggestion: 5*nDims\n"); return 1; }
    if (s->num_repeats > 64 * PC_MASK_WORDS) { std::fprintf(stderr, "polychord_hip: num_repeats > %d unsupported\n", 64 * PC_MASK_WORDS); return 1; }
    if (like->kind == PC_LIKE_CALLBACK && !like->fn) { std::fprintf(stderr, "polychord_hip: callback likelihood without a function pointer\n"); return 1; }
    using clk = std::chrono::steady_clock;
    auto t0 = clk::now();
    std::memset(out, 0, sizeof(*out));
    Engine E;
    if (hooks) { E.dumper = hooks->dumper; E.on_update = hooks->on_update; E.hook_user = hooks->user; }
    int rc;
    auto t1 = t0, t2 = t0;
    try {
        E.setup(*s, *like, *prior);
        t1 = clk::now();
        rc = E.run(out);
        t2 = clk::now();
    } catch (const EngineError &e) {
        std::fprintf(stderr, "polychord_hip: %s\n", e.msg.c_str());
        (void)hipGetLastError();
        rc = e.code;
        pchip_result_free(out);
        t2 = clk::now();
    } catch (const std::bad_alloc &) {
        std::fprintf(stderr, "polychord_hip: out of host memory\n");
        rc = PC_RC_MEMORY;
        pchip_result_free(out);
        t2 = clk::now();
    } catch (...) {
        pchip_result_free(out);
        E.destroy();
        throw;
    }
    E.destroy();
    auto t3 = clk::now();
    if (rc == 0) {
        out->t_setup = std::chrono::duration<double>(t1 - t0).count();
        out->t_teardown = std::chrono::duration<double>(t3 - t2).count();
        out->t_results = std::chrono::duration<double>(t2 - t1).count() - out->t_total;
    }
    return rc;
}

void pchip_result_free(pchip_result *r)
{
    hfree(r->dead); hfree(r->logweights); hfree(r->entry); std::free(r->live); std::free(r->logZp); std::free(r->varlogZp);
    if (r->d_records) pc_cache_dev_free(r->d_records);
    std::free(r->post_mean); std::free(r->post_var); std::free(r->live_cluster);
    std::memset(r, 0, sizeof(*r));
}

int pchip_slice_chains(const pchip_settings *s, const pchip_like *like, const pchip_prior *prior, unsigned batch,
                       int nchains, const double *seeds, const double *chol, double contour, double *babies_out,
                       double *nhats_out, int *nlike_out)
{
    if (like->kind == PCHIP_LIKE_SOURCE || (s->ablate & PC_ABL_RTC_BUILTINS)) {
        std::fprintf(stderr, "polychord_hip: pchip_slice_chains does not take a device source likelihood (or settings.ablate bit 15)\n");
        return 1;
    }
    pchip_settings c = *s;
    c.nlive = nchains; c.nprior = nchains; c.batch = nchains; c.do_clustering = 0;
    Engine E;
    int rc;
    try {
        E.setup(c, *like, *prior);
        PcState &S = E.S;
        const int nT = S.nT, D = S.D, nr = S.nr;
        HIPCHK(hipMemcpy(S.live, seeds, sizeof(double) * (size_t)nchains * nT, hipMemcpyHostToDevice));
        std::vector<double> ll(nchains); std::vector<int> idn(nchains), zero(nchains, 0);
        for (int i = 0; i < nchains; ++i) { ll[i] = seeds[(size_t)i * nT + S.l0]; idn[i] = i; }
        HIPCHK(hipMemcpy(S.live_logL, ll.data(), sizeof(double) * nchains, hipMemcpyHostToDevice));
        HIPCHK(hipMemcpy(S.live_cluster, zero.data(), sizeof(int) * nchains, hipMemcpyHostToDevice));
        HIPCHK(hipMemcpy(S.live_pos, idn.data(), sizeof(int) * nchains, hipMemcpyHostToDevice));
        HIPCHK(hipMemcpy(S.cl_list, idn.data(), sizeof(int) * nchains, hipMemcpyHostToDevice));
        HIPCHK(hipMemcpy(S.cl_n, &nchains, sizeof(int), hipMemcpyHostToDevice));
        HIPCHK(hipMemcpy(S.logLp, &contour, sizeof(double), hipMemcpyHostToDevice));
        HIPCHK(hipMemcpy(S.chol, chol, sizeof(double) * D * D, hipMemcpyHostToDevice));
        S.seed_override = 1;
        rc = pc_launch_nhats(&S, batch, nchains, E.st) || pc_launch_slice(&S, batch, nchains, E.st);
// ... 194 lines not shown
```

polychordlite_amd/csrc/pc_launch.h:

```cpp
#pragma once
#include "pc_state.h"
#include "../../include/polychord_hip.h"
#include <cstddef>

static inline int pc_slice_phi_lds(const PcState *S)
{
    const size_t sh0 = sizeof(double) * ((size_t)S->D + S->nr) + 16, tb = sizeof(double) * (size_t)S->nr * (S->D + 1);
    return (S->nDer > 0 && sh0 + tb <= 48 * 1024) ? 1 : 0;
}

extern "C" {

void pc_abi_set_last_error(const char *msg);
void pc_launch_slice_tick(const PcState *S, unsigned batch, int nchains, void *cs, double *x0s, int *decks, double *prop, const double *ev_logL,
                          const double *ev_theta, const double *ev_phi, int first, double *prop_host, int *need_host, hipStream_t st);
size_t pc_chain_state_size(void);
int pc_launch_killoff_cl(const PcState *S, int nc, hipStream_t st);
int pc_consume_cl_fits(const PcState *S, int nc);
int pc_consume_clp_fits(const PcState *S, int nc);
int pc_launch_consume_cl_many(const PcState *S, const PcManyRec *dR, int R, int wide, hipStream_t st);
int pc_launch_consume_cl(const PcState *S, int nc, hipStream_t st);
int pc_launch_knn_cluster_sub(const int *d_desc, int nb, int mmax, const double *Sm, const int *pool, int *knn, int *labels, int *out, hipStream_t st);
int pc_launch_knn_cluster_sub_many(const PcManyRec *dR, int R, int nb_max, int mmax, hipStream_t st);
void pc_launch_remap_chains(const PcState *S, const int *map, int nold, int n, hipStream_t st);
void pc_launch_shift_mats(const PcState *S, int p, int nc, hipStream_t st);
int pc_launch_knn_cluster_batch(const PcState *S, const int *h_desc, const int *d_desc, int nd, double *Sm, int *knn, int *labels, int *out, const int *dims, int ndims, hipStream_t st);
int pc_launch_knn_cluster_batch_dev(const PcState *S, const int *d_desc, int nd, int nmax, double *Sm, int *knn, int *labels, int *out, const int *dims, int ndims, hipStream_t st);
int pc_launch_knn_cluster_batch_many(const PcState *S, const PcManyRec *dR, int R, int nd_max, int nmax, int any_sub, hipStream_t st);
void pc_launch_rebuild(const PcState *S, int nc, hipStream_t st);
void pc_launch_ph_rehome(const PcState *S, int nph, int nc, const unsigned *old_uids, int nold_uids, int *counts, hipStream_t st);
void pc_launch_nn_lists(const PcState *S, int nleft, int use_rank, hipStream_t st);
int pc_launch_nn_lists_many(const PcState *S, const PcManyRec *dR, int R, int nleft_max, int use_rank, hipStream_t st);
int pc_launch_consume(const PcState *S, int final_mode, int wide, hipStream_t st);
void pc_launch_apply(const PcState *S, unsigned batch, int nchains, hipStream_t st);
int pc_launch_apply_many(const PcState *S, const PcManyRec *dR, int R, unsigned batch, int nchains, hipStream_t st);
int pc_launch_clean_many(const PcManyRec *dR, int R, int nblk_max, hipStream_t st);
void pc_launch_install_live(const PcState *S, const double *rows, int n, hipStream_t st);
void pc_launch_clean(const PcState *S, int nph, unsigned char *keep, int *blk, int *d_total, double *ph2, double *phL2, unsigned *phC2, unsigned long long *phU2, int *dst_index, hipStream_t st);
void pc_launch_reset_thresholds(const PcState *S, hipStream_t st);
int pc_launch_reset_thresholds_many(const PcState *S, const PcManyRec *dR, int R, hipStream_t st);
int pc_cov_nchunk(const PcState *S, int nph);
int pc_launch_covmats(const PcState *S, int nph, int nc, double *psum, int *pcnt, double *mean, int *count, double *pcov, hipStream_t st);
void pc_launch_scan_blocks(int *blk, int nblk, int *total, int *total2, hipStream_t st);
void pc_launch_chol_only(const PcState *S, const double *ncov, const int *count, hipStream_t st);
void pc_launch_init_state(const PcState *S, double logzero, hipStream_t st);
int pc_post_blocks(void);
void pc_launch_post_moments(const PcState *S, int nd, double *pmax, double *part, hipStream_t st);
void pc_prepare_streams(int dev, int want);
void *pc_cache_dev_alloc(size_t bytes);
void pc_cache_dev_free(void *p);
void *pc_cache_host_alloc(size_t bytes);
void pc_cache_host_free(void *p);
int pc_run_many(const pchip_settings *s, const pchip_like *like, const pchip_prior *prior, int nseeds, const int *seeds, int device, int max_in_flight, pchip_result *results);
int pc_fast_fits(const PcState *S);
int pc_launch_sort_live(const PcState *S, hipStream_t st);
int pc_launch_sort_live_many(const PcState *S, const PcManyRec *dR, int R, hipStream_t st);
int pc_launch_consume_fast(const PcState *S, int final_mode, hipStream_t st);
void pc_launch_ph_prepare(const PcState *S, hipStream_t st);
size_t pc_records_block_bytes(long long cap, int nT);
int pc_pack_lived_device(const double *dead, const double *logw, const double *entry, long long nd, int nT, double logzero, double *block, long long cap, long long *h_count, hipStream_t st);
int pc_par_fits(const PcState *S);
int pc_launch_consume_par(const PcState *S, hipStream_t st);
int pc_launch_consume_par_many(const PcState *S, const PcManyRec *dR, int R, hipStream_t st);
int pc_launch_final_par(const PcState *S, hipStream_t st);
int pc_launch_final_par_many(const PcManyRec *dR, int R, hipStream_t st);
int pc_rtc_launch(const PcState *S, const char *expr, dim3 grid, dim3 block, size_t sh, hipStream_t st, void **args);
const char *pc_rtc_error(void);
int pc_rtc_source_data(int id, const double **data, long long *n);
long pc_rtc_source_terms(int id);
int pc_rtc_source_has_prior(int id);
int pc_rtc_wanted(const PcState *S);
int pc_launch_generate_live(const PcState *S, int attempt0, int n, double *rows, double *rows_logL, hipStream_t st);
int pc_nhats_splittable(const PcState *S);
int pc_launch_nhats_part(const PcState *S, unsigned batch, int nchains, int part, hipStream_t st, int packed);
int pc_launch_nhats(const PcState *S, unsigned batch, int nchains, hipStream_t st);
int pc_slice_fusable(const PcState *S);
int pc_launch_slice_fused(const PcState *S, unsigned batch, int nchains, hipStream_t st);
int pc_launch_slice_many(const PcState *S, const PcManyRec *dR, int R, int nchains, int fused, hipStream_t st);
int pc_launch_slice_step(const PcState *S, const PcManyRec *dR, int R, int nchains, int fused, hipStream_t st);
int pc_launch_nhats_many(const PcState *S, const PcManyRec *dR, int R, int nchains, hipStream_t st);
int pc_launch_slice(const PcState *S, unsigned batch, int nchains, hipStream_t st);
int pc_launch_prior_transform(const PcState *S, int n, const double *cubes, double *thetas, hipStream_t st);
int pc_launch_source_eval(const PcState *S, int n, const double *thetas, double *logL, double *phi, hipStream_t st);
int pc_launch_source_prior_eval(const PcState *S, int n, const double *cubes, double *thetas, hipStream_t st);
int pc_bases_t_ok(const PcState *S);
int pc_launch_bases_t(const PcState *S, unsigned batch, int nchains, hipStream_t st);
int pc_launch_bases_t_many(const PcState *S, const PcManyRec *dR, int R, unsigned batch, int nchains, hipStream_t st);
int pc_slice_t_ok(const PcState *S, int ncluster);
int pc_launch_slice_t(const PcState *S, unsigned batch, int nchains, hipStream_t st);
int pc_launch_slice_t_many(const PcState *S, const PcManyRec *dR, int R, unsigned batch, int nchains, hipStream_t st);
int pc_update_fused_ok(const PcState *S, int nc);
int pc_update_fused_blocks(const PcState *S, int nph);
int pc_update_fused_entries(const PcState *S);
#define PC_UPD_CTR_INTS 2048
void pc_launch_update_fused(const PcState *S, int nph, unsigned char *keep, int *blk, int *d_total, double *ph2, double *phL2, unsigned *phC2,
                            unsigned long long *phU2, double *part, double *shift, int deferred, hipStream_t st);
int pc_update_fused_grid(const PcState *S, int nph, int deferred);
int pc_launch_update_fused_many(const PcState *S, const PcManyRec *dR, int R, int nblk_max, int G, int deferred, hipStream_t st);

}
```

polychordlite_amd/csrc/pc_par.hip:

```cpp
#include "pc_state.h"
#include "pc_launch.h"
#include "pc_keys.h"

typedef unsigned long long u64;
#define PAR_NT 1024
#define PAR_W 16

__device__ __forceinline__ int prefix_bits(const u64 *words, int t)
{
    int c = 0;
    const int wq = t >> 6;
    #pragma unroll
    for (int x = 0; x < PAR_W; ++x) {
        u64 v = words[x];
        if (x > wq) v = 0ull; else if (x == wq) v &= (1ull << (t & 63)) - 1ull;
        c += __popcll(v);
    }
    return c;
}

__device__ __forceinline__ int prefix_cum(const u64 *words, const int *cum, int t)
{
    const int wq = t >> 6;
    return (wq >= PAR_W) ? cum[PAR_W] : cum[wq] + __popcll(words[wq] & ((1ull << (t & 63)) - 1ull));
}
#define PAR_WAVE_ORDER() asm volatile("" ::: "memory")

__device__ __forceinline__ void ls_comb(double &m, double &s, double m2, double s2)
{
    const double e = exp(-fabs(m - m2));
    s = (m >= m2) ? s + s2 * e : s * e + s2;
    m = fmax(m, m2);
}
__device__ __forceinline__ double ls_val(double m, double s) { return s > 0.0 ? m + log(s) : NEGBIG; }

#define PAR_SCAN_LEVEL(AM, AS, BM, BS, CTRL, PRED) { \
        const double oam = dpp_f64<CTRL>(AM), oas = dpp_f64<CTRL>(AS), obm = dpp_f64<CTRL>(BM), obs = dpp_f64<CTRL>(BS); \
        double nam = AM, nas = AS, nbm = BM, nbs = BS; \
        ls_comb(nam, nas, oam, oas); ls_comb(nbm, nbs, obm, obs); \
        if (PRED) { AM = nam; AS = nas; BM = nbm; BS = nbs; } }
#define PAR_SCAN_LEVEL1(AM, AS, CTRL, PRED) { \
        const double oam = dpp_f64<CTRL>(AM), oas = dpp_f64<CTRL>(AS); \
        double nam = AM, nas = AS; \
        ls_comb(nam, nas, oam, oas); \
        if (PRED) { AM = nam; AS = nas; } }
__device__ __forceinline__ void block_scan_ls3(double &am, double &as, double &bm, double &bs, double &cm, double &cs, int tid, int nact,
                                               double *X0, double *X1, double *X2, double *X3, double *Xc, double *Xcs, double *wtot)
{
    const int lane = tid & 63, wv = tid >> 6;
    const bool three = Xc != nullptr;
    X0[tid] = am; X1[tid] = as; X2[tid] = bm; X3[tid] = bs;
    if (three) { Xc[tid] = cm; Xcs[tid] = cs; }
    __syncthreads();
    double a_m[4], a_s[4], b_m[4], b_s[4];
    double tam = NEGBIG, tas = 0.0, tbm = NEGBIG, tbs = 0.0;
    const int t4 = (tid & 255) * 4;
    const bool has = t4 < nact;
    const int lr = lane & 15;
    if (wv < 4) {
        #pragma unroll
        for (int u = 0; u < 4; ++u) {
            a_m[u] = has ? X0[t4 + u] : NEGBIG; a_s[u] = has ? X1[t4 + u] : 0.0;
            b_m[u] = has ? X2[t4 + u] : NEGBIG; b_s[u] = has ? X3[t4 + u] : 0.0;
        }
        #pragma unroll
        for (int u = 1; u < 4; ++u) { ls_comb(a_m[u], a_s[u], a_m[u - 1], a_s[u - 1]); ls_comb(b_m[u], b_s[u], b_m[u - 1], b_s[u - 1]); }
        tam = a_m[3]; tas = a_s[3]; tbm = b_m[3]; tbs = b_s[3];
        PAR_SCAN_LEVEL(tam, tas, tbm, tbs, 0x111, lr >= 1)
        PAR_SCAN_LEVEL(tam, tas, tbm, tbs, 0x112, lr >= 2)
        PAR_SCAN_LEVEL(tam, tas, tbm, tbs, 0x114, lr >= 4)
        PAR_SCAN_LEVEL(tam, tas, tbm, tbs, 0x118, lr >= 8)
        PAR_SCAN_LEVEL(tam, tas, tbm, tbs, 0x142, (lane >> 4) & 1)
        PAR_SCAN_LEVEL(tam, tas, tbm, tbs, 0x143, lane >= 32)
        if (lane == 63) { wtot[wv] = tam; wtot[4 + wv] = tas; wtot[8 + wv] = tbm; wtot[12 + wv] = tbs; }
    } else if (three && wv < 8) {
        #pragma unroll
        for (int u = 0; u < 4; ++u) { a_m[u] = has ? Xc[t4 + u] : NEGBIG; a_s[u] = has ? Xcs[t4 + u] : 0.0; }
        #pragma unroll
        for (int u = 1; u < 4; ++u) ls_comb(a_m[u], a_s[u], a_m[u - 1], a_s[u - 1]);
        tam = a_m[3]; tas = a_s[3];
        PAR_SCAN_LEVEL1(tam, tas, 0x111, lr >= 1)
        PAR_SCAN_LEVEL1(tam, tas, 0x112, lr >= 2)
        PAR_SCAN_LEVEL1(tam, tas, 0x114, lr >= 4)
        PAR_SCAN_LEVEL1(tam, tas, 0x118, lr >= 8)
        PAR_SCAN_LEVEL1(tam, tas, 0x142, (lane >> 4) & 1)
        PAR_SCAN_LEVEL1(tam, tas, 0x143, lane >= 32)
        if (lane == 63) { wtot[16 + wv - 4] = tam; wtot[20 + wv - 4] = tas; }
    }
    __syncthreads();
    if (wv < 4) {
        double eam = __shfl_up(tam, 1), eas = __shfl_up(tas, 1), ebm = __shfl_up(tbm, 1), ebs = __shfl_up(tbs, 1);
        if (lane == 0) { eam = NEGBIG; eas = 0.0; ebm = NEGBIG; ebs = 0.0; }
        for (int x = 0; x < wv; ++x) { ls_comb(eam, eas, wtot[x], wtot[4 + x]); ls_comb(ebm, ebs, wtot[8 + x], wtot[12 + x]); }
        if (has) {
            #pragma unroll
            for (int u = 0; u < 4; ++u) {
                ls_comb(a_m[u], a_s[u], eam, eas); ls_comb(b_m[u], b_s[u], ebm, ebs);
                X0[t4 + u] = a_m[u]; X1[t4 + u] = a_s[u]; X2[t4 + u] = b_m[u]; X3[t4 + u] = b_s[u];
            }
        }
    } else if (three && wv < 8) {
        double eam = __shfl_up(tam, 1), eas = __shfl_up(tas, 1);
        if (lane == 0) { eam = NEGBIG; eas = 0.0; }
        for (int x = 0; x < wv - 4; ++x) ls_comb(eam, eas, wtot[16 + x], wtot[20 + x]);
        if (has) {
            #pragma unroll
            for (int u = 0; u < 4; ++u) { ls_comb(a_m[u], a_s[u], eam, eas); Xc[t4 + u] = a_m[u]; Xcs[t4 + u] = a_s[u]; }
        }
    }
    __syncthreads();
    am = X0[tid]; as = X1[tid]; bm = X2[tid]; bs = X3[tid];
    if (three) { cm = Xc[tid]; cs = Xcs[tid]; }
    __syncthreads();
}
__device__ __forceinline__ void block_scan_ls2(double &am, double &as, double &bm, double &bs, int tid, int nact,
                                               double *X0, double *X1, double *X2, double *X3, double *wtot)
{
    double cm = NEGBIG, cs = 0.0;
    block_scan_ls3(am, as, bm, bs, cm, cs, tid, nact, X0, X1, X2, X3, nullptr, nullptr, wtot);
}

__device__ __forceinline__ int wave_scan_i32(int v, int lane)
{
    v += dpp_i32<0x111>(v); v += dpp_i32<0x112>(v); v += dpp_i32<0x114>(v); v += dpp_i32<0x118>(v);
    { const int t = dpp_i32<0x142>(v); if ((lane >> 4) & 1) v += t; }
    { const int t = dpp_i32<0x143>(v); if (lane >= 32) v += t; }
    return v;
}
__device__ __forceinline__ double wave_scan_f64(double v, int lane)
{
    v += dpp_f64<0x111>(v); v += dpp_f64<0x112>(v); v += dpp_f64<0x114>(v); v += dpp_f64<0x118>(v);
    { const double t = dpp_f64<0x142>(v); if ((lane >> 4) & 1) v += t; }
    { const double t = dpp_f64<0x143>(v); if (lane >= 32) v += t; }
    return v;
}
#define PAR_LIN_SPAN 300.0
template <int NSEQ, int NC>
__device__ __forceinline__ bool block_scan_lin(double (&m)[NSEQ], double (&s)[NSEQ], int tid, double *sc ,
                                               const double *cv = nullptr, const int *cq = nullptr, double *uexp = nullptr)
{
    const int lane = tid & 63, wv = tid >> 6;
    double *ref = sc + NSEQ * PAR_W;
    if (tid == 0) {
        #pragma unroll
        for (int q = 0; q < NSEQ; ++q) ref[q] = m[q];
        ref[NSEQ] = 0.0;
    }
    pc_lds_barrier();
    if (NC > 0 && wv == PAR_W - 1 && lane < NC) uexp[lane] = exp(-fabs(ref[cq[lane]] - cv[lane]));
    double inc[NSEQ], R[NSEQ];
    bool bad = false;
    #pragma unroll
    for (int q = 0; q < NSEQ; ++q) {
        R[q] = ref[q];
        const bool has = s[q] != 0.0 && m[q] > 0.5 * NEGBIG;
        const double d = m[q] - R[q];
        bad = bad || (has && !(fabs(d) <= PAR_LIN_SPAN));
        inc[q] = wave_scan_f64(has ? s[q] * exp(d) : 0.0, lane);
        if (lane == 63) sc[q * PAR_W + wv] = inc[q];
    }
    if (__ballot(bad) != 0ull && lane == 0) ref[NSEQ] = 1.0;
    pc_lds_barrier();
    const bool ok = ref[NSEQ] == 0.0;
    if (ok) {
        #pragma unroll
        for (int q = 0; q < NSEQ; ++q) {
            const double t = sc[q * PAR_W + (lane & 15)];
            double pre = t;
            pre += dpp_f64<0x111>(pre); pre += dpp_f64<0x112>(pre); pre += dpp_f64<0x114>(pre); pre += dpp_f64<0x118>(pre);
            s[q] = inc[q] + readlane_f64(pre - t, wv);
            m[q] = R[q];
        }
    }
    pc_lds_barrier();
    return ok;
}

__device__ __forceinline__ double block_scan_add(double v, int lane, int wv, double *wtot)
{
    v = wave_scan_f64(v, lane);
    if (lane == 63) wtot[wv] = v;
    __syncthreads();
    double p = 0.0;
    for (int x = 0; x < wv; ++x) p += wtot[x];
    __syncthreads();
    return v + p;
}

__device__ __forceinline__ void consume_par_body(const PcState &S)
{
    extern __shared__ __attribute__((aligned(16))) char smem[];
    const int tid = threadIdx.x, lane = tid & 63, wv = tid >> 6;
    const int Ncap = S.Ncap, nr = S.nr, NS = (Ncap + 63) & ~63;
    const int Bh = S.B;
    double bl = 0.0; int ep = 0, nl = 0;
    if (tid < Bh) { const int wh = Bh - 1 - tid; bl = S.baby_logL_T[(size_t)(nr - 1) * Bh + wh]; ep = S.ch_epoch[wh]; nl = S.ch_nlike[wh]; }
    PcCtl *ctl = S.ctl;
    const int T = ctl->i_nursery;
    const int n = S.cl_n[0];
    u64 *sSortK = (u64 *)smem;
    u64 *cK = sSortK + NS;
    u64 *srtK = cK + PAR_NT;
    u64 *uKey = srtK + PAR_NT;
    u64 *Gm = uKey + PAR_NT + 64;
    u64 *accR = Gm + PAR_NT;
    u64 *amask = accR + PAR_W;
    u64 *vmask = amask + PAR_W;
    double *sZi = (double *)(vmask + PAR_W);
    double *wtot = sZi + PAR_NT;
    double *fin = wtot + 64;
    int *sSort = (int *)(fin + 16);
    int *srtT = sSort + NS;
    int *rnk = srtT + PAR_NT;
    int *rlo = rnk + PAR_NT;
    int *uSrc = rlo + PAR_NT;
    int *slotA = uSrc + PAR_NT + 64;
    int *parA = slotA + PAR_NT;
    int *accStep = parA + PAR_NT;
    int *ish = accStep + PAR_NT;
    int *hist = ish + 16;
    double *X5 = (double *)(hist + NS + 64);
    double *sLse = (double *)Gm;

    const int epoch = ctl->admin_epoch;
    const int ndead0 = ctl->ndead, fail0 = ctl->failures, nph0 = ctl->nphantom;
    const long long nlike0 = ctl->nlike, niter0 = ctl->niter;
    const double logZ0 = ctl->logZ, logZ20 = ctl->logZ2;
    const double Xp0 = S.logXp[0], Zp0 = S.logZp[0], ZXp0 = S.logZXp[0], Zp20 = S.logZp2[0], ZpXp0 = S.logZpXp[0], XX0 = S.XpXq[0];
    const double lseRef0 = S.lse_ref[0], lseSum0 = S.lse_sum[0];
    const unsigned cuid = S.cl_uid[0];
    const double log2v = 0.6931471805599453;
    __shared__ int cumA[PAR_W + 1], cumV[PAR_W + 1], cumR[PAR_W + 1];
    __shared__ double ulog[4];
    if (wv == PAR_W - 1 && lane < 4) ulog[lane] = log(lane == 3 ? lseSum0 : (double)n + (double)lane);

    long long cyc[9]; int ncy = 0;
    cyc[ncy++] = clock64();
    for (int s = tid; s < Ncap; s += PAR_NT) { S.slot_src[s] = -1; if (S.defer_update) S.slot_step[s] = -1; }
    for (int i = tid; i < NS; i += PAR_NT) { sSortK[i] = (i < n) ? S.sort_key[i] : KEY_HUGE; sSort[i] = S.sort_slot[i]; }
    const bool inT = tid < T;
    const int w = T - 1 - tid;
    u64 ck = KEY_HUGE; bool valid = false;
    if (T != Bh && inT) { bl = S.baby_logL_T[(size_t)(nr - 1) * S.B + w]; ep = S.ch_epoch[w]; nl = S.ch_nlike[w]; }
    if (inT) { ck = d2key(bl); valid = ep == epoch; } else nl = 0;
    cK[tid] = ck;
    for (int i = tid; i < NS + 64; i += PAR_NT) hist[i] = 0;
    {
        const u64 vm = __ballot(valid);
        if (lane == 0) { vmask[wv] = vm; accR[wv] = 0ull; amask[wv] = 0ull; }
    }
    if (tid == 0) { ish[0] = (T << 2) | 3; ish[1] = 0; ish[3] = 0; }
    __syncthreads();
    const double l0 = ulog[0], l1 = ulog[1], l2 = ulog[2], d01 = l0 - l1, d02 = l0 - l2;

    int rl = 0, rp = 0;
    if (inT) {
        int lo = 0, hi = n;
        while (lo < hi) { const int mid = (lo + hi) >> 1; if (sSortK[mid] < ck) lo = mid + 1; else hi = mid; }
        rl = lo; rp = lo;
        while (rp < n && sSortK[rp] == ck) rp++;
    }
    rlo[tid] = rl;

    cyc[ncy++] = clock64();
    int myoff = 0;
    if (inT) myoff = atomicAdd(&hist[rl], 1);
    __syncthreads();
    {
        const int nb = n + 2;
        const int per = (nb + PAR_NT - 1) / PAR_NT, b0 = tid * per;
        int sum = 0;
        for (int x = 0; x < per; ++x) if (b0 + x < nb) sum += hist[b0 + x];
        int inc = sum;
        inc = wave_scan_i32(inc, lane);
        if (lane == 63) accStep[wv] = inc;
        __syncthreads();
        int run = inc - sum;
        for (int x = 0; x < wv; ++x) run += accStep[x];
        for (int x = 0; x < per; ++x) if (b0 + x < nb) { const int cnt = hist[b0 + x]; hist[b0 + x] = run; run += cnt; }
    }
    __syncthreads();
    if (inT) srtT[hist[rl] + myoff] = tid;
    __syncthreads();
    int rho = tid;
    if (inT) {
        const int g0 = hist[rl], g1 = hist[rl + 1];
        int below = 0;
        for (int x = g0; x < g1; ++x) {
            const int o = srtT[x];
            const u64 ko = cK[o];
            below += (ko < ck) || (ko == ck && o > tid);
        }
        rho = g0 + below;
    }
    rnk[tid] = rho;

    cyc[ncy++] = clock64();
    {
        u64 G = 0ull;
        #pragma unroll
        for (int j = 0; j < 64; ++j) {
            const int rj = __builtin_amdgcn_readlane(rho, j);
            if (j < lane && rj > rho) G |= 1ull << j;
        }
        Gm[tid] = G;
    }
    __syncthreads();
    if (wv == 0) {
        const int nch = (T + 63) >> 6;
        int *cum = accStep;
        if (lane < PAR_W) cum[lane] = 0;
        __threadfence_block();
        int rho_t = rnk[lane], r = rlo[lane], tot = 0;
        u64 Gt = Gm[lane];
        for (int c = 0; c < nch; ++c) {
            const int tn = (c + 1 < nch) ? (c + 1) * 64 + lane : lane;
            const int nrho = rnk[tn], nr2 = rlo[tn];
            const u64 nG = Gm[tn];
            const bool v = (vmask[c] >> lane) & 1ull;
            const int wq = rho_t >> 6, bq = rho_t & 63;
            const int P = tot - cum[wq] - __popcll(accR[wq] & (((1ull << bq) << 1) - 1ull));
            u64 am = __ballot(v && r > P);
            for (int it = 0; it < 66; ++it) {
                const bool a = v && r > P + __popcll(Gt & am);
                const u64 nm = __ballot(a);
                if (nm == am) break;
                am = nm;
            }
            if ((am >> lane) & 1ull) atomicOr(&accR[wq], 1ull << bq);
            if (lane == 0) amask[c] = am;
            tot += __popcll(am);
            PAR_WAVE_ORDER();
            {
                int cw = (lane < PAR_W) ? __popcll(accR[lane]) : 0, inc = cw;
                inc += dpp_i32<0x111>(inc); inc += dpp_i32<0x112>(inc); inc += dpp_i32<0x114>(inc); inc += dpp_i32<0x118>(inc);
                if (lane < PAR_W) cum[lane] = inc - cw;
            }
            PAR_WAVE_ORDER();
            rho_t = nrho; r = nr2; Gt = nG;
        }
        {
            const int ca = (lane < PAR_W) ? __popcll(amask[lane]) : 0, cv = (lane < PAR_W) ? __popcll(vmask[lane]) : 0,
                      cr = (lane < PAR_W) ? __popcll(accR[lane]) : 0;
            int ia = ca, iv = cv, ir = cr;
            ia += dpp_i32<0x111>(ia); ia += dpp_i32<0x112>(ia); ia += dpp_i32<0x114>(ia); ia += dpp_i32<0x118>(ia);
            iv += dpp_i32<0x111>(iv); iv += dpp_i32<0x112>(iv); iv += dpp_i32<0x114>(iv); iv += dpp_i32<0x118>(iv);
            ir += dpp_i32<0x111>(ir); ir += dpp_i32<0x112>(ir); ir += dpp_i32<0x114>(ir); ir += dpp_i32<0x118>(ir);
            if (lane < PAR_W) { cumA[lane] = ia - ca; cumV[lane] = iv - cv; cumR[lane] = ir - cr; }
            if (lane == PAR_W - 1) { cumA[PAR_W] = ia; cumV[PAR_W] = iv; cumR[PAR_W] = ir; }
        }
    }
    __syncthreads();

    cyc[ncy++] = clock64();
    const u64 amw = amask[wv], ltm = (1ull << lane) - 1ull;
    const bool acc = (amw >> lane) & 1ull;
    const int kt = cumA[wv] + __popcll(amw & ltm);
    const int K = cumA[PAR_W];
    const int vp = cumV[wv] + __popcll(vmask[wv] & ltm);
    int pos = 0, q = 0;
    if (acc) {
        q = cumR[rho >> 6] + __popcll(accR[rho >> 6] & ((1ull << (rho & 63)) - 1ull));
        pos = q + rp;
        accStep[kt] = tid; srtK[q] = ck;
    }
    __syncthreads();
    const u64 *aK = srtK;

    for (int idx = tid; idx <= K && idx < n; idx += PAR_NT) {
        const u64 sk = sSortK[idx];
        int lo = 0, hi = K;
        while (lo < hi) { const int mid = (lo + hi) >> 1; if (aK[mid] < sk) lo = mid + 1; else hi = mid; }
        const int p2 = idx + lo;
        if (p2 <= K) { uKey[p2] = sk; uSrc[p2] = sSort[idx]; }
    }
    if (acc && pos <= K) { uKey[pos] = ck; uSrc[pos] = -(1 + tid); }
    __syncthreads();

    const u64 gk = inT ? uKey[kt] : KEY_HUGE;
    const int src = acc ? uSrc[kt] : 0;
    slotA[tid] = (acc && src >= 0) ? src : -1;
    parA[tid] = (acc && src < 0) ? (-src - 1) : -1;
    __syncthreads();
    for (int it = 0; it < 12; ++it) {
        const int p = parA[tid];
        int ns = -1, np = -1;
        const bool act = p >= 0;
        if (act) { const int pp = parA[p]; if (pp < 0) ns = slotA[p]; else np = pp; }
        if (!__syncthreads_or(act)) break;
        if (act) { if (np < 0) { slotA[tid] = ns; parA[tid] = -1; } else parA[tid] = np; }
        __syncthreads();
    }

    cyc[ncy++] = clock64();
#ifdef PAR_DBG_EVID
    long long ecy[9]; ecy[0] = clock64();
#endif
    const bool isd = tid < K;
    double L = NEGBIG, Ladd = NEGBIG;
    if (isd) { L = key2d(uKey[tid]); Ladd = key2d(cK[accStep[tid]]); }
    const double jd = (double)tid;
    const double Xb = Xp0 + jd * d01, XXb = XX0 + jd * d02;
    const double Sd = (jd + 1.0) * d01;
#ifdef PAR_DBG_EVID
    ecy[1] = clock64();
#endif
    double tM = isd ? Xb + L - l1 : NEGBIG, tS = isd ? 1.0 : 0.0;
    double vM = isd ? (XXb + L + l0 - l1 - l2) - Sd : NEGBIG, vS = tS;
    double *X0 = (double *)srtK, *X1 = (double *)Gm, *X2 = sZi, *X3 = (double *)rnk;
    double lsM = NEGBIG, lsS = 0.0;
    if (isd) {
        const double dl = L - Ladd, e = exp(-fabs(dl));
        lsM = fmax(Ladd, L); lsS = (dl <= 0.0) ? 1.0 - e : e - 1.0;
    }
    __shared__ double lsc[4 * PAR_W];
    const bool lin_on = !(S.ablate & PC_ABL_PAIR_SCANS);
    __shared__ double ucv[4], uexp[4];
    __shared__ int ucq[4];
    bool lin1 = false;
    auto comb_u = [&](double &m, double &s, double m2, double s2, int c) __attribute__((always_inline)) {
        if (lin1) { const double e = uexp[c]; s = (m >= m2) ? s + s2 * e : s * e + s2; m = fmax(m, m2); }
        else ls_comb(m, s, m2, s2);
    };
    int npair = 0;
    {
        double mm[3] = {tM, vM, lsM}, ss[3] = {tS, vS, lsS};
        if (tid < 4) { ucv[tid] = tid == 0 ? logZ0 : tid == 1 ? ZXp0 : tid == 2 ? ZpXp0 : lseRef0; ucq[tid] = tid == 0 ? 0 : tid == 3 ? 2 : 1; }
        lin1 = lin_on && block_scan_lin<3, 4>(mm, ss, tid, lsc, ucv, ucq, uexp);
        if (lin1) { tM = mm[0]; tS = ss[0]; vM = mm[1]; vS = ss[1]; lsM = mm[2]; lsS = ss[2]; }
        else {
            npair++;
            __syncthreads();
            block_scan_ls3(tM, tS, vM, vS, lsM, lsS, tid, K, X0, X1, X2, X3, (double *)cK, X5, wtot);
        }
    }
#ifdef PAR_DBG_EVID
    ecy[2] = clock64();
#endif
    const bool wact = wv * 64 < K;
    double Zi = NEGBIG;
    double zxM = vM, zxS = vS, zpxM = vM, zpxS = vS;
    if (wact) {
        double ziM = tM, ziS = tS;
        comb_u(ziM, ziS, logZ0, 1.0, 0);
        Zi = ls_val(ziM, ziS);
        comb_u(zxM, zxS, ZXp0, 1.0, 1); comb_u(zpxM, zpxS, ZpXp0, 1.0, 2);
    }
    if (lane == 63) { wtot[wv] = zxM; wtot[PAR_W + wv] = zxS; wtot[2 * PAR_W + wv] = zpxM; wtot[3 * PAR_W + wv] = zpxS; }
    __syncthreads();
    double pzxM = __shfl_up(zxM, 1), pzxS = __shfl_up(zxS, 1), pzpxM = __shfl_up(zpxM, 1), pzpxS = __shfl_up(zpxS, 1);
    if (lane == 0) {
        pzxM = wv ? wtot[wv - 1] : ZXp0; pzxS = wv ? wtot[PAR_W + wv - 1] : 1.0;
        pzpxM = wv ? wtot[2 * PAR_W + wv - 1] : ZpXp0; pzpxS = wv ? wtot[3 * PAR_W + wv - 1] : 1.0;
    }
    __syncthreads();
#ifdef PAR_DBG_EVID
    ecy[3] = clock64();
#endif
    const double cz = log2v + XXb + 2 * L - l1 - l2;
    const double cw = log2v + L - l1 + jd * d01;
    double wM = isd ? cw + pzxM : NEGBIG, wS = isd ? pzxS : 0.0;
    double wpM = isd ? cw + pzpxM : NEGBIG, wpS = isd ? pzpxS : 0.0;
    if (isd) { ls_comb(wM, wS, cz, 1.0); ls_comb(wpM, wpS, cz, 1.0); }
    {
        double mm[2] = {wM, wpM}, ss[2] = {wS, wpS};
        if (lin_on && block_scan_lin<2, 0>(mm, ss, tid, lsc)) { wM = mm[0]; wS = ss[0]; wpM = mm[1]; wpS = ss[1]; }
        else { npair++; block_scan_ls2(wM, wS, wpM, wpS, tid, K, X0, X1, X2, X3, wtot); }
    }
#ifdef PAR_DBG_EVID
    ecy[4] = clock64();
#endif
    if (wact) comb_u(lsM, lsS, lseRef0, lseSum0, 3);
#ifdef PAR_DBG_EVID
    ecy[5] = clock64(); ecy[6] = ecy[5];
#endif
    const double lse_log0 = lseRef0 + ulog[3];
    const double lsei = wact ? lsM + log(lsS) : NEGBIG;
    sZi[tid] = Zi; sLse[tid] = lsei;
    __syncthreads();
#ifdef PAR_DBG_EVID
    ecy[7] = clock64();
#endif

    cyc[ncy++] = clock64();
    const bool defer = S.defer_update != 0;
    int kupd = 0x7fffffff;
    {
        const double tx = ctl->logX_last_update + S.log_cf;
        double kf = ceil((Xp0 - tx) / (-d01));
        if (kf < 1.0) kf = 1.0;
        if (kf < 2.0e9) {
            kupd = (int)kf;
            while (kupd > 1 && Xp0 + (double)(kupd - 1) * d01 <= tx) kupd--;
            while (Xp0 + (double)kupd * d01 > tx) kupd++;
        }
    }
    int tlw = -1;
    for (int x = wv - 1; x >= 0; --x) { const u64 word = amask[x]; if (word) { tlw = x * 64 + 63 - __clzll((long long)word); break; } }
    parA[tid] = vp;
    __syncthreads();
    auto check = [&](int t, int kb, int vb, int tl) __attribute__((always_inline)) {
        const int ndead_b = ndead0 + vb;
        const int fb = (tl >= 0) ? vb - parA[tl] - 1 : fail0 + vb;
        bool more = true;
        if (S.max_ndead == 0) more = false;
        else if (S.max_ndead > 0 && ndead_b >= S.max_ndead) more = false;
        else if (S.use_prec) {
            const double lse_b = kb ? sLse[kb - 1] : lse_log0, Zb = kb ? sZi[kb - 1] : logZ0;
            const double live = lse_b - l0 + Xp0 + (double)kb * d01;
            more = !(live < S.log_prec + Zb);
        }
        int code = 0x7fffffff;
        const bool tv = t < T && ((vmask[t >> 6] >> (t & 63)) & 1ull), ta = t < T && ((amask[t >> 6] >> (t & 63)) & 1ull);
        if (!more || fb > S.nfail) code = (t << 2) | 1;
        else if (tv && ndead_b >= S.Dcap) code = (t << 2) | 2;
        else if (!defer && ta && kb + 1 == kupd) code = ((t + 1) << 2) | 0;
        if (code != 0x7fffffff) atomicMin(&ish[0], code);
    };
    {
        const u64 mw = amask[wv] & ((1ull << lane) - 1ull);
        const int tl = mw ? wv * 64 + 63 - __clzll((long long)mw) : tlw;
        if (tid < T) check(tid, kt, vp, tl);
        if (tid == T - 1) {
            const int tl2 = acc ? tid : tl;
            check(T, kt + (acc ? 1 : 0), vp + (valid ? 1 : 0), tl2);
        }
    }
    __syncthreads();

    cyc[ncy++] = clock64();
#ifdef PAR_DBG_PUBLISH
    long long pcy[8]; pcy[0] = clock64();
#endif
    const int code = ish[0];
    const int ts = code >> 2, pri = code & 3;
    const int Kp = prefix_cum(amask, cumA, ts), vps = prefix_cum(vmask, cumV, ts);
    const int status = (pri == 0) ? PC_ST_UPDATE : (pri == 1) ? PC_ST_DONE : (pri == 2) ? PC_ST_ERROR : PC_ST_RUNNING;
    __shared__ unsigned note_early[8];
    __shared__ int marks_sh[2];
    if (tid == 0) {
        int Kl = 0, marks = 0;
        if (defer && Kp >= kupd) {
            Kl = kupd; marks = 1;
            for (;;) {
                const double txn = (Xp0 + (double)Kl * d01) + S.log_cf;
                const double est = (double)Kl + S.log_cf / d01;
                int kn = !(est < (double)(Kp + 1)) ? Kp + 1 : (int)est;
                if (kn < Kl + 1) kn = Kl + 1;
                while (kn > Kl + 1 && !(Xp0 + (double)(kn - 1) * d01 > txn)) kn--;
                while (kn <= Kp && Xp0 + (double)kn * d01 > txn) kn++;
                if (kn > Kp) break;
                Kl = kn; marks++;
            }
        }
        marks_sh[0] = Kl; marks_sh[1] = marks;
        const unsigned err = (pri == 2) ? PC_ERR_DEAD_CAP : PC_ERR_NONE;
        note_early[0] = (unsigned)status | (err << 8) | ((unsigned)(marks > 0) << 17) | ((unsigned)(marks > 0x3FFF ? 0x3FFF : marks) << 18);
        note_early[1] = (unsigned)(T - ts) & 0xFFFFu; note_early[2] = (unsigned)(ndead0 + vps);
        note_early[3] = (unsigned)(S.pool ? S.pool_base + S.pool_rows : nph0 + ts * nr);
        note_early[4] = 1u | ((unsigned)(ctl->ncluster_dead & 0xFFFF) << 16);
    }
    pc_lds_barrier();
    if (S.ctl_host && tid < PC_NOTE_WORDS)
        ((volatile unsigned long long *)S.ctl_host)[tid] = ((unsigned long long)S.notify_seq << 32) | note_early[tid];
    if (Kp > 0 && tid == Kp - 1) {
        double m = tM, q = tS;
        ls_comb(m, q, Zp0, 1.0);
        fin[0] = Zi; fin[1] = ls_val(m, q); fin[2] = Sd + ls_val(zxM, zxS); fin[3] = Sd + ls_val(zpxM, zpxS);
        ls_comb(wM, wS, logZ20, 1.0); ls_comb(wpM, wpS, Zp20, 1.0);
        fin[4] = ls_val(wM, wS); fin[5] = ls_val(wpM, wpS); fin[6] = lsM; fin[7] = L; fin[8] = lsS;
    }
    {
        int nls = (inT && tid < ts) ? nl : 0, nlf = (inT && tid < ts && !acc) ? nl : 0;
        nls = (int)wave_sum<4>((double)nls); nlf = (int)wave_sum<4>((double)nlf);
        if (lane == 0 && nls) atomicAdd(&ish[1], nls);
        if (lane == 0 && nlf) atomicAdd(&ish[3], nlf);
    }
    if (inT && tid < ts) {
        PcPlanHead h;
        h.ph_cuid = cuid; h.contour = valid ? key2d(gk) : PC_HUGE; h.dead_idx = valid ? ndead0 + vp : -1;
        h.dead_src = -(1 + w); h.logw = S.logzero; h.postX = 0.0; h.postXs = 1.0; h.postZ = 0.0; h.dead_cuid = 0xFFFFFFFFu;
        if (acc) {
            const double Xd = Xp0 + (double)kt * d01;
            h.dead_src = (src >= 0) ? src : -(1 + (T - 1 - (-src - 1)));
            if (S.pool && src >= 0) S.slot_dead[src] = w;
            h.logw = Xd - l1; h.postX = Xd + d01; h.postZ = sZi[kt]; h.dead_cuid = cuid;
        }
        h.ph_base = S.pool ? S.pool_base + w * nr : nph0 + tid * nr; h.ph_count = -2;
        *static_cast<PcPlanHead *>(S.plan + w) = h;
    }
#ifdef PAR_DBG_PUBLISH
    pcy[1] = clock64();
#endif
    if (tid == 0) ish[2] = S.pool ? S.pool_base + S.pool_rows : nph0 + ts * nr;
    const bool accT = acc && tid < ts;
    int pos2 = pos;
    if (ts >= T) {
        if (acc) srtK[q] = ck;
    } else {
        if (lane == 0) accR[wv] = 0ull;
        pc_lds_barrier();
        if (accT) atomicOr(&accR[rho >> 6], 1ull << (rho & 63));
        pc_lds_barrier();
        if (accT) { const int q2 = prefix_bits(accR, rho); pos2 = q2 + rp; srtK[q2] = ck; }
    }
#ifdef PAR_DBG_PUBLISH
    pcy[2] = clock64(); pcy[3] = pcy[2];
#endif
    pc_lds_barrier();
    if (accT && pos2 >= Kp) {
        const int sl = slotA[tid];
        S.live_logL[sl] = key2d(ck); S.slot_src[sl] = w;
        if (defer) S.slot_step[sl] = tid;
        S.sort_key[pos2 - Kp] = ck; S.sort_slot[pos2 - Kp] = sl;
    }
#ifdef PAR_DBG_PUBLISH
    pcy[4] = clock64();
#endif
    for (int idx = tid; idx < n; idx += PAR_NT) {
        const u64 sk = sSortK[idx];
        int lo = 0, hi = Kp;
        while (lo < hi) { const int mid = (lo + hi) >> 1; if (aK[mid] < sk) lo = mid + 1; else hi = mid; }
        const int p2 = idx + lo;
        if (p2 >= Kp) { S.sort_key[p2 - Kp] = sk; S.sort_slot[p2 - Kp] = sSort[idx]; }
    }
#ifdef PAR_DBG_PUBLISH
    pcy[5] = clock64();
#endif
    if (tid == 0) {
        const double Xp = Xp0 + (double)Kp * d01, XX = XX0 + (double)Kp * d02;
        const double lse_m = Kp ? fin[6] : lseRef0, lse_s = Kp ? fin[8] : lseSum0;
        const int usrc = uSrc[Kp];
        S.logLp[0] = key2d(uKey[Kp]); S.imin_slot[0] = (usrc >= 0) ? usrc : slotA[-usrc - 1];
        S.logXp[0] = Xp; S.XpXq[0] = XX;
        if (Kp) { S.logZp[0] = fin[1]; S.logZXp[0] = fin[2]; S.logZpXp[0] = fin[3]; S.logZp2[0] = fin[5]; S.death_thr[0] = fin[7]; }
        S.lse_ref[0] = lse_m; S.lse_sum[0] = lse_s;
        int tl = -1;
        for (int x = PAR_W - 1; x >= 0; --x) {
            u64 word = amask[x];
            if (x > (ts >> 6)) word = 0ull; else if (x == (ts >> 6)) word &= (1ull << (ts & 63)) - 1ull;
            if (word) { tl = x * 64 + 63 - __clzll((long long)word); break; }
        }
        ctl->failures = (tl >= 0) ? vps - prefix_cum(vmask, cumV, tl) - 1 : fail0 + vps;
        ctl->status = status; ctl->error = (pri == 2) ? PC_ERR_DEAD_CAP : PC_ERR_NONE;
        ctl->i_nursery = T - ts; ctl->ndead = ndead0 + vps; ctl->seg_hi = T - 1; ctl->seg_lo = T - ts; ctl->cluster_deleted = 0;
        ctl->nlike = nlike0 + ish[1]; ctl->niter = niter0 + ts; ctl->nphantom = ish[2]; ctl->nlike_failed += ish[3];
        if (Kp) { ctl->logZ = fin[0]; ctl->logZ2 = fin[4]; }
        if (pri == 0) ctl->logX_last_update = Xp;
        ctl->upd_pending = 0; ctl->upd_marks = 0;
        if (marks_sh[1] > 0) {
            const int Kl = marks_sh[0], marks = marks_sh[1];
            ctl->upd_pending = 1; ctl->upd_marks = marks;
            ctl->upd_tmark = accStep[Kl - 1] + 1; ctl->upd_T = T; ctl->upd_ts = ts; ctl->upd_nph0 = S.pool ? S.pool_base : nph0;
            ctl->upd_thr = key2d(uKey[Kl - 1]); ctl->upd_keep_thr = (Kp > Kl) ? 1 : 0;
            ctl->logX_last_update = Xp0 + (double)Kl * d01;
        }
        if (S.use_prec) ctl->live_logZ = (Kp ? sLse[Kp - 1] : lseRef0 + ulog[3]) - l0 + Xp;
        cyc[ncy++] = clock64();
#ifdef PAR_NO_DBG
#elif defined(PAR_DBG_EVID)
        for (int x = 0; x < 7; ++x) ctl->dbg[x] += ecy[x + 1] - ecy[x];
#elif defined(PAR_DBG_PUBLISH)
        pcy[6] = clock64();
        for (int x = 0; x < 6; ++x) ctl->dbg[x] += pcy[x + 1] - pcy[x];
#else
        for (int x = 0; x + 1 < ncy && x < 8; ++x) ctl->dbg[x] += cyc[x + 1] - cyc[x];
        ctl->dbg[7] += npair;
#endif
    }
}
__global__ __launch_bounds__(PAR_NT) void k_consume_par(PcState S) { consume_par_body(S); }
__global__ __launch_bounds__(PAR_NT) void k_consume_par_many(const PcManyRec *R) { consume_par_body(pc_many_state(R, blockIdx.y)); }


__device__ __forceinline__ void final_par_body(const PcState &S)
{
    __shared__ __attribute__((aligned(16))) double X0[PAR_NT], X1[PAR_NT], X2[PAR_NT], X3[PAR_NT];
    __shared__ double wtot[64];
    __shared__ double carry[12];
    const int tid = threadIdx.x, lane = tid & 63, wv = tid >> 6;
    PcCtl *ctl = S.ctl;
    const int n0 = S.cl_n[0], nT = S.nT, ndead0 = ctl->ndead;
    const unsigned cuid = S.cl_uid[0];
    const double log2v = 0.6931471805599453;
    if (ndead0 + n0 > S.Dcap) { if (tid == 0) { ctl->status = PC_ST_ERROR; ctl->error = PC_ERR_DEAD_CAP; } return; }
    if (tid == 0) {
        carry[0] = ctl->logZ; carry[1] = ctl->logZ2; carry[2] = S.logXp[0]; carry[3] = S.XpXq[0]; carry[4] = S.logZp[0];
        carry[5] = S.logZXp[0]; carry[6] = S.logZp2[0]; carry[7] = S.logZpXp[0]; carry[8] = S.death_thr[0];
    }
    __syncthreads();
    for (int base = 0; base < n0; base += PAR_NT) {
        const int m = min(PAR_NT, n0 - base), i = base + tid;
        const bool on = tid < m;
        const double logZ0 = carry[0], logZ20 = carry[1], Xp0 = carry[2], XX0 = carry[3], Zp0 = carry[4], ZXp0 = carry[5],
                     Zp20 = carry[6], ZpXp0 = carry[7];
        const int slot = on ? S.sort_slot[i] : 0;
        const double L = on ? key2d(S.sort_key[i]) : NEGBIG;
        const int myn = n0 - i;
        const double a0 = on ? log((double)myn) : 0.0, a1 = on ? log((double)myn + 1.0) : 0.0, a2 = on ? log((double)myn + 2.0) : 0.0;
        const double e01 = a0 - a1, e02 = a0 - a2;
        const double sx = block_scan_add(e01, lane, wv, wtot), sxx = block_scan_add(e02, lane, wv, wtot);
        const double Xb = Xp0 + (sx - e01), XXb = XX0 + (sxx - e02), Sd = sx;
        double tM = on ? Xb + L - a1 : NEGBIG, tS = on ? 1.0 : 0.0;
        double vM = on ? (XXb + L + a0 - a1 - a2) - Sd : NEGBIG, vS = tS;
        block_scan_ls2(tM, tS, vM, vS, tid, m, X0, X1, X2, X3, wtot);
        double ziM = tM, ziS = tS;
        ls_comb(ziM, ziS, logZ0, 1.0);
        const double Zi = ls_val(ziM, ziS);
        double zxM = vM, zxS = vS, zpxM = vM, zpxS = vS;
        ls_comb(zxM, zxS, ZXp0, 1.0); ls_comb(zpxM, zpxS, ZpXp0, 1.0);
        X0[tid] = zxM; X1[tid] = zxS; X2[tid] = zpxM; X3[tid] = zpxS;
        __syncthreads();
        const double SdPrev = Sd - e01;
        double pzxM = tid ? X0[tid - 1] : ZXp0, pzxS = tid ? X1[tid - 1] : 1.0;
        double pzpxM = tid ? X2[tid - 1] : ZpXp0, pzpxS = tid ? X3[tid - 1] : 1.0;
        __syncthreads();
        const double cz = log2v + XXb + 2 * L - a1 - a2;
        const double cw = log2v + L - a1 + SdPrev;
        double wM = on ? cw + pzxM : NEGBIG, wS = on ? pzxS : 0.0;
        double wpM = on ? cw + pzpxM : NEGBIG, wpS = on ? pzpxS : 0.0;
        if (on) { ls_comb(wM, wS, cz, 1.0); ls_comb(wpM, wpS, cz, 1.0); }
        block_scan_ls2(wM, wS, wpM, wpS, tid, m, X0, X1, X2, X3, wtot);
        if (on) {
            const int di = ndead0 + i;
            S.dead_logw[di] = Xb - a1; S.dead_postX[di] = Xb + e01; S.dead_postZ[di] = Zi;
            S.dead_cuid[di] = cuid; S.dead_entry[di] = S.live_entry[slot];
            S.live_logL[slot] = PC_HUGE; S.live_cluster[slot] = -1; S.slot_src[slot] = -1;
        }
        __syncthreads();
        if (tid == m - 1) {
            double a = tM, b = tS;
            ls_comb(a, b, Zp0, 1.0);
            ls_comb(wM, wS, logZ20, 1.0); ls_comb(wpM, wpS, Zp20, 1.0);
            carry[0] = Zi; carry[1] = ls_val(wM, wS); carry[2] = Xp0 + sx; carry[3] = XX0 + sxx; carry[4] = ls_val(a, b);
            carry[5] = Sd + ls_val(zxM, zxS); carry[6] = ls_val(wpM, wpS); carry[7] = Sd + ls_val(zpxM, zpxS); carry[8] = L;
        }
        __syncthreads();
        for (int r = wv; r < m; r += PAR_NT / 64) {
            const int sl = S.sort_slot[base + r];
            const double *row = S.live + (size_t)sl * nT;
            double *dst = S.dead + (size_t)(ndead0 + base + r) * nT;
            for (int e = lane; e < nT; e += 64) dst[e] = row[e];
        }
    }
    if (tid == 0) {
        const int ncd = ctl->ncluster_dead;
        if (ncd < S.maxc_dead) { S.logZp_dead[ncd] = carry[4]; S.logZp2_dead[ncd] = carry[6]; S.cl_uid_dead[ncd] = cuid; }
        S.logLp[0] = PC_HUGE; S.imin_slot[0] = -1; S.logXp[0] = carry[2]; S.XpXq[0] = carry[3]; S.logZp[0] = carry[4];
        S.logZXp[0] = carry[5]; S.logZp2[0] = carry[6]; S.logZpXp[0] = carry[7]; S.death_thr[0] = carry[8]; S.cl_n[0] = 0;
        ctl->status = PC_ST_DONE; ctl->error = PC_ERR_NONE; ctl->ndead = ndead0 + n0; ctl->ncluster = 0; ctl->ncluster_dead = ncd + 1;
        ctl->logZ = carry[0]; ctl->logZ2 = carry[1]; ctl->cluster_deleted = 0;
    }
}
__global__ __launch_bounds__(PAR_NT) void k_final_par(PcState S) { final_par_body(S); }
__global__ __launch_bounds__(PAR_NT) void k_final_par_many(const PcManyRec *R) { final_par_body(pc_many_state(R, blockIdx.y)); }


static size_t par_lds(const PcState *S)
{
    const size_t NS = ((size_t)S->Ncap + 63) & ~(size_t)63;
    return 8 * (NS + 4 * PAR_NT + 64 + 3 * PAR_W + PAR_NT + 64 + 16 + PAR_NT) + 4 * (2 * NS + 7 * PAR_NT + 2 * 64 + 16) + 64;
}

#define PAR_STATIC_LDS 2048
extern "C" int pc_par_fits(const PcState *S) { return par_lds(S) + PAR_STATIC_LDS <= 160 * 1024 && S->B <= PAR_NT; }

extern "C" int pc_launch_consume_par(const PcState *S, hipStream_t st)
{
    const size_t sh = par_lds(S);
    if (sh + PAR_STATIC_LDS > 160 * 1024 || S->B > PAR_NT) return 1;
    pc_need_dyn_lds((const void *)k_consume_par, sh);
    hipLaunchKernelGGL(k_consume_par, dim3(1), dim3(PAR_NT), sh, st, *S);
    return 0;
}

extern "C" int pc_launch_consume_par_many(const PcState *S, const PcManyRec *dR, int R, hipStream_t st)
{
    const size_t sh = par_lds(S);
    if (sh + PAR_STATIC_LDS > 160 * 1024 || S->B > PAR_NT) return 1;
    pc_need_dyn_lds((const void *)k_consume_par_many, sh);
    hipLaunchKernelGGL(k_consume_par_many, dim3(1, R), dim3(PAR_NT), sh, st, dR);
    return 0;
}

extern "C" int pc_launch_final_par(const PcState *S, hipStream_t st)
{
    hipLaunchKernelGGL(k_final_par, dim3(1), dim3(PAR_NT), 0, st, *S);
    return 0;
}
extern "C" int pc_launch_final_par_many(const PcManyRec *dR, int R, hipStream_t st)
{
    hipLaunchKernelGGL(k_final_par_many, dim3(1, R), dim3(PAR_NT), 0, st, dR);
    return 0;
}
```

polychordlite_amd/csrc/pc_state.h:

```cpp
#pragma once
#include "pc_dev.h"

enum { PC_ST_RUNNING = 0, PC_ST_DONE = 1, PC_ST_UPDATE = 2, PC_ST_ERROR = 4 };
enum { PC_ERR_NONE = 0, PC_ERR_PHANTOM_CAP = 1, PC_ERR_DEAD_CAP = 2, PC_ERR_CLUSTER_CAP = 3, PC_ERR_NOSLOT = 4 };

enum { PC_ABL_FUNCTOR = 1 << 0, PC_ABL_NO_POOL = 1 << 1, PC_ABL_NO_DEFER = 1 << 2, PC_ABL_NO_FUSED_UPDATE = 1 << 3, PC_ABL_PAIR_SCANS = 1 << 4,
       PC_ABL_CONSUME_GENERAL = 1 << 5, PC_ABL_SLICE_LANE = 1 << 6, PC_ABL_BASES_PACKED = 1 << 7, PC_ABL_CL_END_AT_DEATH = 1 << 8,
       PC_ABL_KILLOFF_GENERAL = 1 << 9, PC_ABL_CONSUME_CL_SERIAL = 1 << 10, PC_ABL_RETIRED_11 = 1 << 11, PC_ABL_RETIRED_12 = 1 << 12,
       PC_ABL_NO_HELPER = 1 << 13, PC_ABL_QC_BY_CHAIN = 1 << 14, PC_ABL_RTC_BUILTINS = 1 << 15, PC_ABL_UPDATE_CHAIN = 1 << 16, PC_ABL_TRACE_CHOL = 1 << 30 };

#define PC_MASK_WORDS 16

struct PcCtl {
    int status;
    int error;
    int i_nursery;
    int admin_epoch;
    int failures;
    int ncluster;
    int ncluster_dead;
    int ndead;
    int nphantom;
    int seg_hi, seg_lo;
    int cluster_deleted;
    unsigned batch_id;
    unsigned next_cluster_uid;
    long long nlike;
    long long niter;
    long long nlike_device;
    long long nlike_failed;
    double logZ, logZ2;
    double logX_last_update;
    double live_logZ;
    unsigned long long seq;
    long long dbg[8];
    long long gen_cyc[4];
    long long nn_walks, nn_fallbacks;
    int upd_pending, upd_marks;
    int upd_tmark;
    int upd_T, upd_ts;
    int upd_nph0;
    int upd_keep_thr, upd_pad;
    double upd_thr;
    int chol_suspect, chol_pad;
    long long wave_cyc[4];
};

#define PC_MAX_GRADE 8
#define PC_NN_K 8
#define PC_NN_NONE (-2147483647 - 1)
#define PC_CUID_NONE 0xFFFFFFFEu

struct alignas(16) PcPlanHead {
    int dead_idx;
    int dead_src;
    int ph_base;
    unsigned dead_cuid;
    unsigned ph_cuid;
    int ph_count;
    double logw;
    double postX, postZ;
    double postXs;
    double contour;
};
struct alignas(16) PcPlan : PcPlanHead {
    unsigned long long ph_mask[PC_MASK_WORDS];
};
static_assert(sizeof(PcPlanHead) == 64 && sizeof(PcPlan) == 64 + 8 * PC_MASK_WORDS, "plan record layout");

struct PcState {
    int D, nDer, nT, nr, N, Ncap, B, maxc, Pcap, Dcap;
    int b0, l0, p0, d0;
    uint32_t k0, k1;
    double logzero, log_prec, log_cf;
    int use_prec, max_ndead, nfail;
    int n_nlives; const double *dyn_loglikes; const int *dyn_nlives;
    PcLike like; PcPrior prior;
    double *live;
    double *live_logL;
    int *live_cluster;
    int *live_pos;
    double *live_entry;
    int *cl_list;
    int *cl_n;
    double *logZp, *logXp, *logZXp, *logZp2, *logZpXp, *logLp, *XpXq ;
    int *imin_slot;
    double *lse_ref, *lse_sum;
    double *death_thr;
    unsigned *cl_uid;
    double *chol, *cov;
    double *logZp_dead, *logZp2_dead;
    unsigned *cl_uid_dead;
    int maxc_dead;
    double *phantom;
    double *ph_logL;
    unsigned *ph_cuid;
    unsigned long long *ph_uid;
    double *dead;
    double *dead_logw;
    double *dead_postX, *dead_postZ;
    unsigned *dead_cuid;
    double *dead_entry;
    double *babies;
    double *baby_logL;
    double *baby_logL_T;
    int *ch_cluster, *ch_epoch, *ch_nlike, *ch_seed_slot;
    double *ch_contour;
    double *nhat;
    double *nhat_w;
    double *nhat_raw;
    double *nhat_Ms;
    double *ch_My;
    PcPlan *plan;
    int *sort_slot;
    unsigned long long *sort_key;
    int *slot_src;
    int *slot_dead;
    int *slot_step;
    int defer_update;
    int pool, pool_base, pool_rows;
    int ngrade, nb_total; unsigned n_dev;
    int g_off[PC_MAX_GRADE], g_nr[PC_MAX_GRADE], g_nb[PC_MAX_GRADE], g_col0[PC_MAX_GRADE], g_e0[PC_MAX_GRADE];
    int *ch_nlike_g;
    const double *logn;
    int *nn_list;
    int *nn_slot_owner;
    int *nn_chain_slot;
    double *nn_pts;
    int *nn_code;
    int nn_valid;
    int ablate;
    int seq_mode;
    int epoch_discard;
    int seed_override;
    PcCtl *ctl;
    PcCtl *ctl_host; unsigned notify_seq;
    int src_id, src_pad;
    const double *src_data; long long src_ndata;
};

struct PcManyRec { PcState S; void *p[10]; int ia[6]; int pad[2]; };
enum { PC_REC_I_BATCH = 0, PC_REC_I_BASES_SEQ = 3 };
enum { PC_REC_KEEP = 0, PC_REC_BLK = 1, PC_REC_TOTAL = 2, PC_REC_PH2 = 3, PC_REC_PHL2 = 4, PC_REC_PHC2 = 5, PC_REC_PHU2 = 6, PC_REC_PART = 7, PC_REC_SHIFT = 8 };
enum { PC_REC_I_ROWS = 1, PC_REC_I_BLOCKS = 2 };
enum { PC_REC_I_NLEFT = 1 };
enum { PC_REC_DESC = 0, PC_REC_SM = 1, PC_REC_KNN = 2, PC_REC_LAB = 3, PC_REC_OUT = 4, PC_REC_DIMS = 5 };
enum { PC_REC_I_ND = 1, PC_REC_I_NMAX = 2, PC_REC_I_ND_SUB = 3 };
enum { PC_REC_G_DESC = 0, PC_REC_G_SM = 1, PC_REC_G_POOL = 2, PC_REC_G_KNN = 3, PC_REC_G_LAB = 4, PC_REC_G_OUT = 5 };
enum { PC_REC_I_NB = 1, PC_REC_I_MMAX = 2 };

#ifdef __HIPCC__
template <class T, class B> __device__ __forceinline__ T *pc_as_global(T *p, const B * )
{
    typedef __attribute__((address_space(1))) char gchar;
    return (T *)(gchar *)(uintptr_t)p;
}
static_assert(sizeof(PcState) == 968, "PcState changed: add the new pointer members to pc_many_state, then update this size");
__device__ __forceinline__ PcState pc_many_state(const PcManyRec *R, int run)
{
    PcState S = R[run].S;
#define G(f) S.f = pc_as_global(S.f, R)
    G(like.invcov); G(like.mean); G(prior.lo); G(prior.hi); G(dyn_loglikes); G(dyn_nlives); G(live); G(live_logL);
    G(live_cluster); G(live_pos); G(live_entry); G(cl_list); G(cl_n); G(logZp); G(logXp); G(logZXp);
    G(logZp2); G(logZpXp); G(logLp); G(XpXq); G(imin_slot); G(lse_ref); G(lse_sum); G(death_thr);
    G(cl_uid); G(chol); G(cov); G(logZp_dead); G(logZp2_dead); G(cl_uid_dead); G(phantom); G(ph_logL);
    G(ph_cuid); G(ph_uid); G(dead); G(dead_logw); G(dead_postX); G(dead_postZ); G(dead_cuid); G(dead_entry);
    G(babies); G(baby_logL); G(baby_logL_T); G(ch_cluster); G(ch_epoch); G(ch_nlike); G(ch_seed_slot); G(ch_contour);
    G(nhat); G(nhat_w); G(nhat_raw); G(nhat_Ms); G(ch_My); G(plan); G(sort_slot); G(sort_key);
    G(slot_src); G(slot_dead); G(slot_step); G(ch_nlike_g); G(logn); G(nn_list); G(nn_slot_owner); G(nn_chain_slot);
    G(nn_pts); G(nn_code); G(ctl); G(ctl_host); G(src_data);
#undef G
    return S;
}
struct PcManyView { PcState S; void *p[10]; int ia[6]; };
__device__ __forceinline__ PcManyView pc_many_view(const PcManyRec *R, int run)
{
    PcManyView v;
    v.S = pc_many_state(R, run);
#pragma unroll
    for (int i = 0; i < 10; ++i) v.p[i] = pc_as_global(R[run].p[i], R);
#pragma unroll
    for (int i = 0; i < 6; ++i) v.ia[i] = R[run].ia[i];
    return v;
}
#endif

#define PC_NOTE_WORDS 5
__device__ __forceinline__ void pc_publish_ctl(const PcState &S)
{
    __shared__ unsigned pc_note_sh[8];
    if (!S.ctl_host) return;
    if (threadIdx.x == 0) {
        const PcCtl *c = S.ctl;
        pc_note_sh[0] = (unsigned)c->status | ((unsigned)c->error << 8) | ((unsigned)(c->cluster_deleted != 0) << 16) |
                        ((unsigned)(c->upd_pending != 0) << 17) | ((unsigned)(c->upd_marks > 0x3FFF ? 0x3FFF : c->upd_marks) << 18);
        pc_note_sh[1] = (unsigned)c->i_nursery & 0xFFFFu;
        pc_note_sh[2] = (unsigned)c->ndead; pc_note_sh[3] = (unsigned)c->nphantom;
        pc_note_sh[4] = (unsigned)c->ncluster | ((unsigned)(c->ncluster_dead & 0xFFFF) << 16);
    }
    __syncthreads();
    if (threadIdx.x < PC_NOTE_WORDS)
        ((volatile unsigned long long *)S.ctl_host)[threadIdx.x] = ((unsigned long long)S.notify_seq << 32) | pc_note_sh[threadIdx.x];
}

__device__ __forceinline__ int pc_sel(const int (&a)[PC_MAX_GRADE], int g)
{
    int r = a[0];
#pragma unroll
    for (int k = 1; k < PC_MAX_GRADE; ++k) r = (g == k) ? a[k] : r;
    return r;
}
__device__ __forceinline__ int pc_grade_of(const PcState &S, int col)
{
    int g = 0;
#pragma unroll
    for (int k = 1; k < PC_MAX_GRADE; ++k) if (k < S.ngrade && col >= S.g_col0[k]) g = k;
    return g;
}
__device__ __forceinline__ void pc_grade_of_basis(const PcState &S, int block, int &g, int &b)
{
    g = 0; b = block;
#pragma unroll
    for (int k = 0; k + 1 < PC_MAX_GRADE; ++k) if (g == k && k + 1 < S.ngrade && b >= S.g_nb[k]) { b -= S.g_nb[k]; g = k + 1; }
}

__device__ __forceinline__ double pc_seq_uniform(const PcState &S, unsigned long long n)
{
    return pc_uniform(S.k0, S.k1, PC_DOM_SEQ, (uint32_t)(n >> 32), 0u, (uint32_t)n);
}
#ifndef __HIPCC_RTC__
#include <mutex>
#include <map>
#include <utility>
inline void pc_need_dyn_lds(const void *kernel, size_t bytes)
{
    static std::mutex mtx;
    static std::map<std::pair<const void *, int>, size_t> mark;
    thread_local std::map<std::pair<const void *, int>, size_t> seen;
    int dev = 0;
    (void)hipGetDevice(&dev);
    const auto key = std::make_pair(kernel, dev);
    size_t &mine = seen[key];
    if (bytes <= mine) return;
    std::lock_guard<std::mutex> g(mtx);
    size_t &m = mark[key];
    if (bytes > m) { (void)hipFuncSetAttribute(kernel, hipFuncAttributeMaxDynamicSharedMemorySize, (int)bytes); m = bytes; }
    mine = m;
}
#endif
```

Before: 1.321 billion likelihood evals/s.

## Compute consume evidence scans in a second workgroup beside the next consume

The single-cluster parallel consume kernel now launches two workgroups. The first records the accepted deaths' likelihoods into a double-buffered side record, and the second computes the previous step's evidence scans (logZ, variance and lse terms) alongside it. A guard decides whether the deferred evidence can be trusted for the termination test; if it cannot, the main workgroup catches up inline first. A trailing kernel flushes the pending evidence before the final kill-off. This aims to take the evidence block-scans off the serial critical path of each consume step, at the cost of extra LDS, a second workgroup and more complex state handoff.

```diff
diff --git a/include/polychord_hip.h b/include/polychord_hip.h
--- a/include/polychord_hip.h
+++ b/include/polychord_hip.h
@@ -147,6 +147,7 @@
        PCHIP_PATH_DEVICE_PRIOR = 20,
        PCHIP_PATH_SOURCE_TERMS = 21,
        PCHIP_PATH_SLICE_STEP = 22,
+       PCHIP_PATH_EVIDENCE_BESIDE = 23,
        PCHIP_PATH_COUNT = 24 };
 
 typedef struct {
diff --git a/polychordlite_amd/_ctypes_api.py b/polychordlite_amd/_ctypes_api.py
--- a/polychordlite_amd/_ctypes_api.py
+++ b/polychordlite_amd/_ctypes_api.py
@@ -72,6 +72,7 @@
 PATH_NAMES = ("consume_par", "consume_cl", "consume_general", "consume_fast", "killoff_par", "killoff_cl", "killoff_general",
               "killoff_fast", "update_fused", "update_steps", "slice_wave", "slice_lane", "nn_lists", "nn_fallbacks", "pool_mode",
               "defer_update", "consume_cl_serial", "subcluster_passes", "subcluster_splits", "source_kernels", "device_prior", "source_terms", "slice_step")
+PATH_NAMES_MORE = ("evidence_beside",)
 
 
 _lib = None
@@ -356,7 +357,7 @@
                post_mean=np.ctypeslib.as_array(r.post_mean, shape=(D + settings.nDerived,)).copy(),
                post_var=np.ctypeslib.as_array(r.post_var, shape=(D + settings.nDerived,)).copy(),
                nlike_grade=[int(v) for v in r.nlike_grade], nlike_failed=r.nlike_failed, ncluster_peak=r.ncluster_peak, epoch_discard=r.epoch_discard, n_records=int(r.n_records) if r.d_records else None,
-               path={n: int(r.path[i]) for i, n in enumerate(PATH_NAMES)},
+               path={n: int(r.path[i]) for i, n in enumerate(PATH_NAMES + PATH_NAMES_MORE)},
                varlogZp=np.ctypeslib.as_array(r.varlogZp, shape=(max(r.nZp, 1),))[:r.nZp].copy(),
                logzero=settings.logzero,
                _owner=own)
diff --git a/polychordlite_amd/csrc/pc_engine.hip b/polychordlite_amd/csrc/pc_engine.hip
--- a/polychordlite_amd/csrc/pc_engine.hip
+++ b/polychordlite_amd/csrc/pc_engine.hip
@@ -388,6 +388,7 @@
 static std::atomic<long long> g_dbg_compact_ns{0}, g_dbg_nursery_ns{0}, g_dbg_capacity_ns{0}, g_dbg_endb_ns{0}, g_dbg_destroy_ns{0}, g_dbg_evwait_ns{0}, g_dbg_d1{0}, g_dbg_d2{0};
 struct Engine {
     Cohort *co = nullptr;
+    PcBeside *d_bes = nullptr;
     Fiber *fib = nullptr;
     pchip_settings cfg{};
     std::atomic<int> stop{0};
@@ -1569,6 +1570,12 @@
                 if (need < 0.4 * (double)free_b) grow_phantoms(2LL * S.Pcap);
             }
         }
+        S.bes = nullptr; S.bes_n = 0; S.bes_pad = 0;
+        if (plan.pool && !co && plan.par_ok && h_ctl->ncluster == 1 && !cfg.do_clustering && !(cfg.ablate & PC_ABL_EVIDENCE_INLINE) && pc_par_beside_fits(&S)) {
+            if (!d_bes) d_bes = dalloc<PcBeside>(1);
+            S.bes = d_bes;
+            (void)pc_launch_beside_init(&S, st);
+        }
         r_rc = 0;
         return -1;
     }
@@ -1760,6 +1767,7 @@
                 S.nn_valid = 0;
                 if (!sort_valid) { rc2 = stage(rec_sort(S)); sort_valid = true; }
                 rc2 = rc2 || stage(rec_consume(S));
+                if (S.bes) S.bes_n++;
                 break;
             case PC_CONTRACT_FAST:
                 if (co) co->flush();
@@ -1851,6 +1859,7 @@
         if (h_ctl->ncluster == 0) {
         } else if (plan.par_ok && h_ctl->ncluster == 1) {
             path[PCHIP_PATH_KILLOFF_PAR]++;
+            if (S.bes) (void)pc_launch_evidence_pending(&S, st);
             if (co && sort_valid) { co->rec(rec_final(S)); if (!fused_final) co->flush(); }
             else {
             if (!sort_valid) (void)pc_launch_sort_live(&S, st);
@@ -1906,6 +1915,7 @@
         out->nlike_failed = h_ctl->nlike_failed; out->ncluster_peak = ncluster_peak; out->epoch_discard = S.epoch_discard;
         path[PCHIP_PATH_NN_FALLBACKS] = (long)h_ctl->nn_fallbacks; path[PCHIP_PATH_POOL_MODE] = S.pool; path[PCHIP_PATH_DEFER_UPDATE] = S.defer_update;
         path[PCHIP_PATH_SLICE_STEP] = step_note.shared;
+        path[PCHIP_PATH_EVIDENCE_BESIDE] = S.bes ? (long)h_ctl->bes_made : 0;
         for (int k = 0; k < PCHIP_PATH_COUNT; ++k) out->path[k] = path[k];
         grade_counts(out->nlike_grade);
         out->ncluster = nc_end; out->ncluster_dead = h_ctl->ncluster_dead; out->nbatches = tm.batches;
@@ -1916,6 +1926,7 @@
         if (dbg_lvl >= 3) std::fprintf(stderr, "polychord_hip dbg general: term %lld identify %lld kill+add %lld tail %lld cycles; %lld chains identified from the candidate lists, %lld of them fell back to the full search\n", h_ctl->gen_cyc[0], h_ctl->gen_cyc[1], h_ctl->gen_cyc[2], h_ctl->gen_cyc[3], h_ctl->nn_walks, h_ctl->nn_fallbacks);
         if (dbg_lvl == 4) std::fprintf(stderr, "polychord_hip dbg par: stage+search %lld rank-sort %lld accept %lld merge+slots %lld evidence %lld triggers %lld publish %lld cycles\n", h_ctl->dbg[0], h_ctl->dbg[1], h_ctl->dbg[2], h_ctl->dbg[3], h_ctl->dbg[4], h_ctl->dbg[5], h_ctl->dbg[6]);
         if (dbg_lvl == 4) std::fprintf(stderr, "polychord_hip dbg par: %lld evidence scans as pairs (terms beyond one scale)\n", h_ctl->dbg[7]);
+        if (dbg_lvl == 4 && S.bes) std::fprintf(stderr, "polychord_hip dbg par: evidence beside: %d launches by the second workgroup, %lld cycles\n", h_ctl->bes_made, (long long)h_ctl->bes_kcyc << 10);
         if (dbg_lvl == 4 && h_ctl->wave_cyc[0]) std::fprintf(stderr, "polychord_hip dbg clp (several clusters; the line above then reads: decisions | order of deaths + slots | counts + volumes | volume sum + step 0's phantoms | prefix sums + commit | waves 1-3 | write back | passes): wave 1 %lld wave 2 %lld wave 3 %lld phantom wave %lld cycles\n", h_ctl->wave_cyc[0], h_ctl->wave_cyc[1], h_ctl->wave_cyc[2], h_ctl->wave_cyc[3]);
         if (dbg_lvl == 2) std::fprintf(stderr, "polychord_hip dbg: loop cycles %lld passB %lld (%lld flushes) accept-steps %lld (%lld) ins-rescan %lld (%lld) reject-steps cycles %lld\n", h_ctl->dbg[0], h_ctl->dbg[1], h_ctl->dbg[4], h_ctl->dbg[2], h_ctl->dbg[3], h_ctl->dbg[5], h_ctl->dbg[6], h_ctl->dbg[7]);
         if ((size_t)h_ctl->ndead > h_dead_cap) {
@@ -1997,6 +2008,7 @@
         dfree(d_x0s); dfree(d_prop); dfree(d_ans); dfree(d_decks);
         if (hp_prop) { hfree(hp_prop); hp_prop = nullptr; } if (hp_ans) { hfree(hp_ans); hp_ans = nullptr; } if (hp_need) { hfree(hp_need); hp_need = nullptr; }
         dfree(upd_part); dfree(upd_shift); upd_part_cap = 0;
+        dfree(d_bes); S.bes = nullptr;
         clus.release(); dfree(c_subdims);
         for (void *h : staged_up) hfree(h);
         staged_up.clear();
diff --git a/polychordlite_amd/csrc/pc_guard.h b/polychordlite_amd/csrc/pc_guard.h
--- /dev/null
+++ b/polychordlite_amd/csrc/pc_guard.h
@@ -0,0 +1,17 @@
+#pragma once
+#include <cmath>
+
+#if defined(__HIP__) || defined(__CUDACC__)
+#define PC_GUARD_FN __attribute__((host)) __attribute__((device)) inline
+#else
+#define PC_GUARD_FN inline
+#endif
+
+PC_GUARD_FN bool pc_prec_guard_holds(double live_logZ, double logZ, double log_prec, int G, int n)
+{
+    if (n <= 0 || G < 0) return false;
+    const double arg = exp(-2.0 * G / (double)n) - exp(log_prec) * (double)G / ((double)n + 1.0);
+    if (!(arg > 0.0)) return false;
+    const double gthr = -log(arg) + 0.05;
+    return (live_logZ - (log_prec + logZ)) > gthr;
+}
diff --git a/polychordlite_amd/csrc/pc_launch.h b/polychordlite_amd/csrc/pc_launch.h
--- a/polychordlite_amd/csrc/pc_launch.h
+++ b/polychordlite_amd/csrc/pc_launch.h
@@ -61,6 +61,9 @@
 int pc_pack_lived_device(const double *dead, const double *logw, const double *entry, long long nd, int nT, double logzero, double *block, long long cap, long long *h_count, hipStream_t st);
 int pc_par_fits(const PcState *S);
 int pc_launch_consume_par(const PcState *S, hipStream_t st);
+int pc_par_beside_fits(const PcState *S);
+int pc_launch_beside_init(const PcState *S, hipStream_t st);
+int pc_launch_evidence_pending(const PcState *S, hipStream_t st);
 int pc_launch_consume_par_many(const PcState *S, const PcManyRec *dR, int R, hipStream_t st);
 int pc_launch_final_par(const PcState *S, hipStream_t st);
 int pc_launch_final_par_many(const PcManyRec *dR, int R, hipStream_t st);
diff --git a/polychordlite_amd/csrc/pc_par.hip b/polychordlite_amd/csrc/pc_par.hip
--- a/polychordlite_amd/csrc/pc_par.hip
+++ b/polychordlite_amd/csrc/pc_par.hip
@@ -1,6 +1,7 @@
 #include "pc_state.h"
 #include "pc_launch.h"
 #include "pc_keys.h"
+#include "pc_guard.h"
 
 typedef unsigned long long u64;
 #define PAR_NT 1024
@@ -187,7 +188,123 @@
     return v + p;
 }
 
-__device__ __forceinline__ void consume_par_body(const PcState &S)
+struct ParEvIn {
+    double logZ0, ZXp0, ZpXp0, lseRef0, lseSum0, Xp0, XX0, l0, l1, l2;
+};
+struct ParEvLds {
+    double *X0, *X1, *X2, *X3, *Xc, *X5, *wtot, *lsc, *ucv, *uexp; int *ucq; double *sZi, *sLse;
+};
+struct ParEv {
+    double tM, tS, Zi, Sd, zxM, zxS, zpxM, zpxS, wM, wS, wpM, wpS, lsM, lsS; int npair;
+};
+__device__ __forceinline__ void par_evidence(ParEv &o, const int tid, const int K, const double L, const double Ladd, const bool lin_on,
+                                             const ParEvIn &in, const ParEvLds &sc
+#ifdef PAR_DBG_EVID
+                                             , long long *ecy
+#endif
+                                             )
+{
+    const int lane = tid & 63, wv = tid >> 6;
+    const double logZ0 = in.logZ0, ZXp0 = in.ZXp0, ZpXp0 = in.ZpXp0, lseRef0 = in.lseRef0, lseSum0 = in.lseSum0, Xp0 = in.Xp0, XX0 = in.XX0;
+    const double l0 = in.l0, l1 = in.l1, l2 = in.l2, d01 = l0 - l1, d02 = l0 - l2;
+    const double log2v = 0.6931471805599453;
+    double *const wtot = sc.wtot, *const lsc = sc.lsc, *const ucv = sc.ucv, *const uexp = sc.uexp, *const sZi = sc.sZi, *const sLse = sc.sLse;
+    int *const ucq = sc.ucq;
+    const bool isd = tid < K;
+    const double jd = (double)tid;
+    const double Xb = Xp0 + jd * d01, XXb = XX0 + jd * d02;
+    const double Sd = (jd + 1.0) * d01;
+#ifdef PAR_DBG_EVID
+    ecy[1] = clock64();
+#endif
+    double tM = isd ? Xb + L - l1 : NEGBIG, tS = isd ? 1.0 : 0.0;
+    double vM = isd ? (XXb + L + l0 - l1 - l2) - Sd : NEGBIG, vS = tS;
+    double *const X0 = sc.X0, *const X1 = sc.X1, *const X2 = sc.X2, *const X3 = sc.X3;
+    double lsM = NEGBIG, lsS = 0.0;
+    if (isd) {
+        const double dl = L - Ladd, e = exp(-fabs(dl));
+        lsM = fmax(Ladd, L); lsS = (dl <= 0.0) ? 1.0 - e : e - 1.0;
+    }
+    bool lin1 = false;
+    auto comb_u = [&](double &m, double &s, double m2, double s2, int c) __attribute__((always_inline)) {
+        if (lin1) { const double e = uexp[c]; s = (m >= m2) ? s + s2 * e : s * e + s2; m = fmax(m, m2); }
+        else ls_comb(m, s, m2, s2);
+    };
+    int npair = 0;
+    {
+        double mm[3] = {tM, vM, lsM}, ss[3] = {tS, vS, lsS};
+        if (tid < 4) { ucv[tid] = tid == 0 ? logZ0 : tid == 1 ? ZXp0 : tid == 2 ? ZpXp0 : lseRef0; ucq[tid] = tid == 0 ? 0 : tid == 3 ? 2 : 1; }
+        lin1 = lin_on && block_scan_lin<3, 4>(mm, ss, tid, lsc, ucv, ucq, uexp);
+        if (lin1) { tM = mm[0]; tS = ss[0]; vM = mm[1]; vS = ss[1]; lsM = mm[2]; lsS = ss[2]; }
+        else {
+            npair++;
+            __syncthreads();
+            block_scan_ls3(tM, tS, vM, vS, lsM, lsS, tid, K, X0, X1, X2, X3, sc.Xc, sc.X5, wtot);
+        }
+    }
+#ifdef PAR_DBG_EVID
+    ecy[2] = clock64();
+#endif
+    const bool wact = wv * 64 < K;
+    double Zi = NEGBIG;
+    double zxM = vM, zxS = vS, zpxM = vM, zpxS = vS;
+    if (wact) {
+        double ziM = tM, ziS = tS;
+        comb_u(ziM, ziS, logZ0, 1.0, 0);
+        Zi = ls_val(ziM, ziS);
+        comb_u(zxM, zxS, ZXp0, 1.0, 1); comb_u(zpxM, zpxS, ZpXp0, 1.0, 2);
+    }
+    if (lane == 63) { wtot[wv] = zxM; wtot[PAR_W + wv] = zxS; wtot[2 * PAR_W + wv] = zpxM; wtot[3 * PAR_W + wv] = zpxS; }
+    __syncthreads();
+    double pzxM = __shfl_up(zxM, 1), pzxS = __shfl_up(zxS, 1), pzpxM = __shfl_up(zpxM, 1), pzpxS = __shfl_up(zpxS, 1);
+    if (lane == 0) {
+        pzxM = wv ? wtot[wv - 1] : ZXp0; pzxS = wv ? wtot[PAR_W + wv - 1] : 1.0;
+        pzpxM = wv ? wtot[2 * PAR_W + wv - 1] : ZpXp0; pzpxS = wv ? wtot[3 * PAR_W + wv - 1] : 1.0;
+    }
+    __syncthreads();
+#ifdef PAR_DBG_EVID
+    ecy[3] = clock64();
+#endif
+    const double cz = log2v + XXb + 2 * L - l1 - l2;
+    const double cw = log2v + L - l1 + jd * d01;
+    double wM = isd ? cw + pzxM : NEGBIG, wS = isd ? pzxS : 0.0;
+    double wpM = isd ? cw + pzpxM : NEGBIG, wpS = isd ? pzpxS : 0.0;
+    if (isd) { ls_comb(wM, wS, cz, 1.0); ls_comb(wpM, wpS, cz, 1.0); }
+    {
+        double mm[2] = {wM, wpM}, ss[2] = {wS, wpS};
+        if (lin_on && block_scan_lin<2, 0>(mm, ss, tid, lsc)) { wM = mm[0]; wS = ss[0]; wpM = mm[1]; wpS = ss[1]; }
+        else { npair++; block_scan_ls2(wM, wS, wpM, wpS, tid, K, X0, X1, X2, X3, wtot); }
+    }
+#ifdef PAR_DBG_EVID
+    ecy[4] = clock64();
+#endif
+    if (wact) comb_u(lsM, lsS, lseRef0, lseSum0, 3);
+#ifdef PAR_DBG_EVID
+    ecy[5] = clock64(); ecy[6] = ecy[5];
+#endif
+    const double lsei = wact ? lsM + log(lsS) : NEGBIG;
+    sZi[tid] = Zi; sLse[tid] = lsei;
+    __syncthreads();
+#ifdef PAR_DBG_EVID
+    ecy[7] = clock64();
+#endif
+
+    o.tM = tM; o.tS = tS; o.Zi = Zi; o.Sd = Sd; o.zxM = zxM; o.zxS = zxS; o.zpxM = zpxM; o.zpxS = zpxS;
+    o.wM = wM; o.wS = wS; o.wpM = wpM; o.wpS = wpS; o.lsM = lsM; o.lsS = lsS; o.npair = npair;
+}
+__device__ __forceinline__ void par_evidence_fin(double *fin, const ParEv &o, const double L, const double Zp0, const double logZ20, const double Zp20)
+{
+    double m = o.tM, q = o.tS;
+    ls_comb(m, q, Zp0, 1.0);
+    fin[0] = o.Zi; fin[1] = ls_val(m, q); fin[2] = o.Sd + ls_val(o.zxM, o.zxS); fin[3] = o.Sd + ls_val(o.zpxM, o.zpxS);
+    double wM = o.wM, wS = o.wS, wpM = o.wpM, wpS = o.wpS;
+    ls_comb(wM, wS, logZ20, 1.0); ls_comb(wpM, wpS, Zp20, 1.0);
+    fin[4] = ls_val(wM, wS); fin[5] = ls_val(wpM, wpS); fin[6] = o.lsM; fin[7] = L; fin[8] = o.lsS;
+}
+
+enum { PAR_INLINE = 0, PAR_RECORD = 1, PAR_CATCH_UP = 2 };
+template <int MODE>
+__device__ __forceinline__ void consume_par_body(const PcState &S, const double *est = nullptr, PcBesideHalf *wr = nullptr)
 {
     extern __shared__ __attribute__((aligned(16))) char smem[];
     const int tid = threadIdx.x, lane = tid & 63, wv = tid >> 6;
@@ -225,9 +342,11 @@
     const int epoch = ctl->admin_epoch;
     const int ndead0 = ctl->ndead, fail0 = ctl->failures, nph0 = ctl->nphantom;
     const long long nlike0 = ctl->nlike, niter0 = ctl->niter;
-    const double logZ0 = ctl->logZ, logZ20 = ctl->logZ2;
-    const double Xp0 = S.logXp[0], Zp0 = S.logZp[0], ZXp0 = S.logZXp[0], Zp20 = S.logZp2[0], ZpXp0 = S.logZpXp[0], XX0 = S.XpXq[0];
-    const double lseRef0 = S.lse_ref[0], lseSum0 = S.lse_sum[0];
+    const bool from_est = MODE == PAR_CATCH_UP;
+    const double logZ0 = from_est ? est[0] : ctl->logZ, logZ20 = from_est ? est[1] : ctl->logZ2;
+    const double Xp0 = S.logXp[0], Zp0 = from_est ? est[2] : S.logZp[0], ZXp0 = from_est ? est[3] : S.logZXp[0], Zp20 = from_est ? est[4] : S.logZp2[0],
+                 ZpXp0 = from_est ? est[5] : S.logZpXp[0], XX0 = S.XpXq[0];
+    const double lseRef0 = from_est ? est[6] : S.lse_ref[0], lseSum0 = from_est ? est[7] : S.lse_sum[0];
     const unsigned cuid = S.cl_uid[0];
     const double log2v = 0.6931471805599453;
     __shared__ int cumA[PAR_W + 1], cumV[PAR_W + 1], cumR[PAR_W + 1];
@@ -398,89 +517,23 @@
 #endif
     const bool isd = tid < K;
     double L = NEGBIG, Ladd = NEGBIG;
-    if (isd) { L = key2d(uKey[tid]); Ladd = key2d(cK[accStep[tid]]); }
-    const double jd = (double)tid;
-    const double Xb = Xp0 + jd * d01, XXb = XX0 + jd * d02;
-    const double Sd = (jd + 1.0) * d01;
-#ifdef PAR_DBG_EVID
-    ecy[1] = clock64();
-#endif
-    double tM = isd ? Xb + L - l1 : NEGBIG, tS = isd ? 1.0 : 0.0;
-    double vM = isd ? (XXb + L + l0 - l1 - l2) - Sd : NEGBIG, vS = tS;
-    double *X0 = (double *)srtK, *X1 = (double *)Gm, *X2 = sZi, *X3 = (double *)rnk;
-    double lsM = NEGBIG, lsS = 0.0;
-    if (isd) {
-        const double dl = L - Ladd, e = exp(-fabs(dl));
-        lsM = fmax(Ladd, L); lsS = (dl <= 0.0) ? 1.0 - e : e - 1.0;
-    }
     __shared__ double lsc[4 * PAR_W];
     const bool lin_on = !(S.ablate & PC_ABL_PAIR_SCANS);
     __shared__ double ucv[4], uexp[4];
     __shared__ int ucq[4];
-    bool lin1 = false;
-    auto comb_u = [&](double &m, double &s, double m2, double s2, int c) __attribute__((always_inline)) {
-        if (lin1) { const double e = uexp[c]; s = (m >= m2) ? s + s2 * e : s * e + s2; m = fmax(m, m2); }
-        else ls_comb(m, s, m2, s2);
-    };
-    int npair = 0;
-    {
-        double mm[3] = {tM, vM, lsM}, ss[3] = {tS, vS, lsS};
-        if (tid < 4) { ucv[tid] = tid == 0 ? logZ0 : tid == 1 ? ZXp0 : tid == 2 ? ZpXp0 : lseRef0; ucq[tid] = tid == 0 ? 0 : tid == 3 ? 2 : 1; }
-        lin1 = lin_on && block_scan_lin<3, 4>(mm, ss, tid, lsc, ucv, ucq, uexp);
-        if (lin1) { tM = mm[0]; tS = ss[0]; vM = mm[1]; vS = ss[1]; lsM = mm[2]; lsS = ss[2]; }
-        else {
-            npair++;
-            __syncthreads();
-            block_scan_ls3(tM, tS, vM, vS, lsM, lsS, tid, K, X0, X1, X2, X3, (double *)cK, X5, wtot);
-        }
-    }
+    ParEv ev; ev.npair = 0;
+    if (MODE != PAR_RECORD) {
+        if (isd) { L = key2d(uKey[tid]); Ladd = key2d(cK[accStep[tid]]); }
+        const ParEvIn in = {logZ0, ZXp0, ZpXp0, lseRef0, lseSum0, Xp0, XX0, l0, l1, l2};
+        const ParEvLds sc = {(double *)srtK, (double *)Gm, sZi, (double *)rnk, (double *)cK, X5, wtot, lsc, ucv, uexp, ucq, sZi, sLse};
 #ifdef PAR_DBG_EVID
-    ecy[2] = clock64();
-#endif
-    const bool wact = wv * 64 < K;
-    double Zi = NEGBIG;
-    double zxM = vM, zxS = vS, zpxM = vM, zpxS = vS;
-    if (wact) {
-        double ziM = tM, ziS = tS;
-        comb_u(ziM, ziS, logZ0, 1.0, 0);
-        Zi = ls_val(ziM, ziS);
-        comb_u(zxM, zxS, ZXp0, 1.0, 1); comb_u(zpxM, zpxS, ZpXp0, 1.0, 2);
-    }
-    if (lane == 63) { wtot[wv] = zxM; wtot[PAR_W + wv] = zxS; wtot[2 * PAR_W + wv] = zpxM; wtot[3 * PAR_W + wv] = zpxS; }
-    __syncthreads();
-    double pzxM = __shfl_up(zxM, 1), pzxS = __shfl_up(zxS, 1), pzpxM = __shfl_up(zpxM, 1), pzpxS = __shfl_up(zpxS, 1);
-    if (lane == 0) {
-        pzxM = wv ? wtot[wv - 1] : ZXp0; pzxS = wv ? wtot[PAR_W + wv - 1] : 1.0;
-        pzpxM = wv ? wtot[2 * PAR_W + wv - 1] : ZpXp0; pzpxS = wv ? wtot[3 * PAR_W + wv - 1] : 1.0;
-    }
-    __syncthreads();
-#ifdef PAR_DBG_EVID
-    ecy[3] = clock64();
-#endif
-    const double cz = log2v + XXb + 2 * L - l1 - l2;
-    const double cw = log2v + L - l1 + jd * d01;
-    double wM = isd ? cw + pzxM : NEGBIG, wS = isd ? pzxS : 0.0;
-    double wpM = isd ? cw + pzpxM : NEGBIG, wpS = isd ? pzpxS : 0.0;
-    if (isd) { ls_comb(wM, wS, cz, 1.0); ls_comb(wpM, wpS, cz, 1.0); }
-    {
-        double mm[2] = {wM, wpM}, ss[2] = {wS, wpS};
-        if (lin_on && block_scan_lin<2, 0>(mm, ss, tid, lsc)) { wM = mm[0]; wS = ss[0]; wpM = mm[1]; wpS = ss[1]; }
-        else { npair++; block_scan_ls2(wM, wS, wpM, wpS, tid, K, X0, X1, X2, X3, wtot); }
-    }
-#ifdef PAR_DBG_EVID
-    ecy[4] = clock64();
-#endif
-    if (wact) comb_u(lsM, lsS, lseRef0, lseSum0, 3);
-#ifdef PAR_DBG_EVID
-    ecy[5] = clock64(); ecy[6] = ecy[5];
-#endif
+        par_evidence(ev, tid, K, L, Ladd, lin_on, in, sc, ecy);
+#else
+        par_evidence(ev, tid, K, L, Ladd, lin_on, in, sc);
+#endif
+    }
+    const int npair = ev.npair;
     const double lse_log0 = lseRef0 + ulog[3];
-    const double lsei = wact ? lsM + log(lsS) : NEGBIG;
-    sZi[tid] = Zi; sLse[tid] = lsei;
-    __syncthreads();
-#ifdef PAR_DBG_EVID
-    ecy[7] = clock64();
-#endif
 
     cyc[ncy++] = clock64();
     const bool defer = S.defer_update != 0;
@@ -505,7 +558,7 @@
         bool more = true;
         if (S.max_ndead == 0) more = false;
         else if (S.max_ndead > 0 && ndead_b >= S.max_ndead) more = false;
-        else if (S.use_prec) {
+        else if (MODE != PAR_RECORD && S.use_prec) {
             const double lse_b = kb ? sLse[kb - 1] : lse_log0, Zb = kb ? sZi[kb - 1] : logZ0;
             const double live = lse_b - l0 + Xp0 + (double)kb * d01;
             more = !(live < S.log_prec + Zb);
@@ -563,12 +616,10 @@
     pc_lds_barrier();
     if (S.ctl_host && tid < PC_NOTE_WORDS)
         ((volatile unsigned long long *)S.ctl_host)[tid] = ((unsigned long long)S.notify_seq << 32) | note_early[tid];
-    if (Kp > 0 && tid == Kp - 1) {
-        double m = tM, q = tS;
-        ls_comb(m, q, Zp0, 1.0);
-        fin[0] = Zi; fin[1] = ls_val(m, q); fin[2] = Sd + ls_val(zxM, zxS); fin[3] = Sd + ls_val(zpxM, zpxS);
-        ls_comb(wM, wS, logZ20, 1.0); ls_comb(wpM, wpS, Zp20, 1.0);
-        fin[4] = ls_val(wM, wS); fin[5] = ls_val(wpM, wpS); fin[6] = lsM; fin[7] = L; fin[8] = lsS;
+    if (MODE != PAR_RECORD && Kp > 0 && tid == Kp - 1) par_evidence_fin(fin, ev, L, Zp0, logZ20, Zp20);
+    if (MODE == PAR_RECORD) {
+        if (tid < K) { const int stp = accStep[tid]; wr->L[tid] = key2d(uKey[tid]); wr->Ladd[tid] = key2d(cK[stp]); wr->didx[tid] = ndead0 + parA[stp]; }
+        if (tid == 0) { wr->head.pending = 1; wr->head.K = K; wr->head.Kp = Kp; wr->head.pad = 0; wr->head.Xp0 = Xp0; wr->head.XX0 = XX0; }
     }
     {
         int nls = (inT && tid < ts) ? nl : 0, nlf = (inT && tid < ts && !acc) ? nl : 0;
@@ -584,7 +635,7 @@
             const double Xd = Xp0 + (double)kt * d01;
             h.dead_src = (src >= 0) ? src : -(1 + (T - 1 - (-src - 1)));
             if (S.pool && src >= 0) S.slot_dead[src] = w;
-            h.logw = Xd - l1; h.postX = Xd + d01; h.postZ = sZi[kt]; h.dead_cuid = cuid;
+            h.logw = Xd - l1; h.postX = Xd + d01; h.postZ = MODE == PAR_RECORD ? 0.0 : sZi[kt]; h.dead_cuid = cuid;
         }
         h.ph_base = S.pool ? S.pool_base + w * nr : nph0 + tid * nr; h.ph_count = -2;
         *static_cast<PcPlanHead *>(S.plan + w) = h;
@@ -633,8 +684,23 @@
         const int usrc = uSrc[Kp];
         S.logLp[0] = key2d(uKey[Kp]); S.imin_slot[0] = (usrc >= 0) ? usrc : slotA[-usrc - 1];
         S.logXp[0] = Xp; S.XpXq[0] = XX;
+        if (MODE == PAR_INLINE) {
         if (Kp) { S.logZp[0] = fin[1]; S.logZXp[0] = fin[2]; S.logZpXp[0] = fin[3]; S.logZp2[0] = fin[5]; S.death_thr[0] = fin[7]; }
         S.lse_ref[0] = lse_m; S.lse_sum[0] = lse_s;
+        } else if (MODE == PAR_RECORD) {
+            if (Kp) S.death_thr[0] = key2d(uKey[Kp - 1]);
+        } else {
+            PcBesideEv e;
+            e.logZ = Kp ? fin[0] : logZ0; e.logZ2 = Kp ? fin[4] : logZ20; e.logZp = Kp ? fin[1] : Zp0; e.logZXp = Kp ? fin[2] : ZXp0;
+            e.logZp2 = Kp ? fin[5] : Zp20; e.logZpXp = Kp ? fin[3] : ZpXp0; e.lse_ref = lse_m; e.lse_sum = lse_s;
+            e.live_logZ = S.use_prec ? (Kp ? sLse[Kp - 1] : lseRef0 + ulog[3]) - l0 + Xp : est[8];
+            S.logZp[0] = e.logZp; S.logZXp[0] = e.logZXp; S.logZpXp[0] = e.logZpXp; S.logZp2[0] = e.logZp2;
+            if (Kp) S.death_thr[0] = fin[7];
+            S.lse_ref[0] = lse_m; S.lse_sum[0] = lse_s;
+            ctl->logZ = e.logZ; ctl->logZ2 = e.logZ2;
+            wr->ev = e;
+            wr->head.pending = 0; wr->head.K = 0; wr->head.Kp = 0; wr->head.pad = 0; wr->head.Xp0 = Xp; wr->head.XX0 = XX;
+        }
         int tl = -1;
         for (int x = PAR_W - 1; x >= 0; --x) {
             u64 word = amask[x];
@@ -645,7 +711,7 @@
         ctl->status = status; ctl->error = (pri == 2) ? PC_ERR_DEAD_CAP : PC_ERR_NONE;
         ctl->i_nursery = T - ts; ctl->ndead = ndead0 + vps; ctl->seg_hi = T - 1; ctl->seg_lo = T - ts; ctl->cluster_deleted = 0;
         ctl->nlike = nlike0 + ish[1]; ctl->niter = niter0 + ts; ctl->nphantom = ish[2]; ctl->nlike_failed += ish[3];
-        if (Kp) { ctl->logZ = fin[0]; ctl->logZ2 = fin[4]; }
+        if (MODE == PAR_INLINE && Kp) { ctl->logZ = fin[0]; ctl->logZ2 = fin[4]; }
         if (pri == 0) ctl->logX_last_update = Xp;
         ctl->upd_pending = 0; ctl->upd_marks = 0;
         if (marks_sh[1] > 0) {
@@ -655,7 +721,7 @@
             ctl->upd_thr = key2d(uKey[Kl - 1]); ctl->upd_keep_thr = (Kp > Kl) ? 1 : 0;
             ctl->logX_last_update = Xp0 + (double)Kl * d01;
         }
-        if (S.use_prec) ctl->live_logZ = (Kp ? sLse[Kp - 1] : lseRef0 + ulog[3]) - l0 + Xp;
+        if (MODE != PAR_RECORD && S.use_prec) ctl->live_logZ = (Kp ? sLse[Kp - 1] : lseRef0 + ulog[3]) - l0 + Xp;
         cyc[ncy++] = clock64();
 #ifdef PAR_NO_DBG
 #elif defined(PAR_DBG_EVID)
@@ -669,8 +735,115 @@
 #endif
     }
 }
-__global__ __launch_bounds__(PAR_NT) void k_consume_par(PcState S) { consume_par_body(S); }
-__global__ __launch_bounds__(PAR_NT) void k_consume_par_many(const PcManyRec *R) { consume_par_body(pc_many_state(R, blockIdx.y)); }
+__global__ __launch_bounds__(PAR_NT) void k_consume_par(PcState S) { consume_par_body<PAR_INLINE>(S); }
+__global__ __launch_bounds__(PAR_NT) void k_consume_par_many(const PcManyRec *R) { consume_par_body<PAR_INLINE>(pc_many_state(R, blockIdx.y)); }
+
+
+#define PAR_PEND_LDS (8 * (6 * PAR_NT + 64))
+__device__ __forceinline__ bool par_beside_guard(const PcState &S, const PcBesideHalf *rd, int n)
+{
+    bool hold = true;
+    if (S.use_prec) {
+        const double live = rd->ev.lse_ref + log(rd->ev.lse_sum) - log((double)n) + rd->head.Xp0;
+        hold = pc_prec_guard_holds(live, rd->ev.logZ, S.log_prec, (rd->head.pending ? rd->head.Kp : 0) + S.B, n);
+    }
+    return __builtin_amdgcn_readfirstlane((int)hold) != 0;
+}
+__device__ __forceinline__ void par_pending_evidence(const PcState &S, const PcBesideHalf *rd, double *est, char *smem)
+{
+    const int tid = threadIdx.x, lane = tid & 63, wv = tid >> 6;
+    const int pend = rd->head.pending, K = pend ? min(rd->head.K, PAR_NT) : 0, Kp = pend ? min(rd->head.Kp, K) : 0;
+    const int n = S.cl_n[0];
+    const double logZ0 = rd->ev.logZ, logZ20 = rd->ev.logZ2, Zp0 = rd->ev.logZp, ZXp0 = rd->ev.logZXp, Zp20 = rd->ev.logZp2, ZpXp0 = rd->ev.logZpXp;
+    const double lseRef0 = rd->ev.lse_ref, lseSum0 = rd->ev.lse_sum, Xp0 = rd->head.Xp0, XX0 = rd->head.XX0;
+    double *X0 = (double *)smem, *X1 = X0 + PAR_NT, *X2 = X1 + PAR_NT, *X3 = X2 + PAR_NT, *Xc = X3 + PAR_NT, *X5 = Xc + PAR_NT, *wtot = X5 + PAR_NT;
+    double *sZi = X2, *sLse = X1;
+    __shared__ double ulog[4], lsc[4 * PAR_W], ucv[4], uexp[4], fin[16];
+    __shared__ int ucq[4];
+    if (wv == PAR_W - 1 && lane < 4) ulog[lane] = log(lane == 3 ? lseSum0 : (double)n + (double)lane);
+    __syncthreads();
+    const double l0 = ulog[0], l1 = ulog[1], l2 = ulog[2], d01 = l0 - l1;
+    const bool isd = tid < K;
+    double L = NEGBIG, Ladd = NEGBIG;
+    if (isd) { L = rd->L[tid]; Ladd = rd->Ladd[tid]; }
+    const bool lin_on = !(S.ablate & PC_ABL_PAIR_SCANS);
+    ParEv ev; ev.npair = 0;
+    const ParEvIn in = {logZ0, ZXp0, ZpXp0, lseRef0, lseSum0, Xp0, XX0, l0, l1, l2};
+    const ParEvLds sc = {X0, X1, X2, X3, Xc, X5, wtot, lsc, ucv, uexp, ucq, sZi, sLse};
+#ifdef PAR_DBG_EVID
+    long long ecy[9];
+    par_evidence(ev, tid, K, L, Ladd, lin_on, in, sc, ecy);
+#else
+    par_evidence(ev, tid, K, L, Ladd, lin_on, in, sc);
+#endif
+    if (Kp > 0 && tid == Kp - 1) par_evidence_fin(fin, ev, L, Zp0, logZ20, Zp20);
+    if (tid < Kp) { const int di = rd->didx[tid]; if (di >= 0 && di < S.Dcap) S.dead_postZ[di] = ev.Zi; }
+    __syncthreads();
+    if (tid == 0) {
+        est[0] = Kp ? fin[0] : logZ0; est[1] = Kp ? fin[4] : logZ20; est[2] = Kp ? fin[1] : Zp0; est[3] = Kp ? fin[2] : ZXp0;
+        est[4] = Kp ? fin[5] : Zp20; est[5] = Kp ? fin[3] : ZpXp0; est[6] = Kp ? fin[6] : lseRef0; est[7] = Kp ? fin[8] : lseSum0;
+        const double Xp = Xp0 + (double)Kp * d01;
+        est[8] = (pend && S.use_prec) ? (Kp ? sLse[Kp - 1] : lseRef0 + ulog[3]) - l0 + Xp : rd->ev.live_logZ;
+    }
+    __syncthreads();
+}
+__global__ __launch_bounds__(PAR_NT) void k_consume_par_beside(PcState S)
+{
+    extern __shared__ __attribute__((aligned(16))) char smem[];
+    __shared__ double est[16];
+    const long long c0 = clock64();
+    const PcBesideHalf *rd = &S.bes->half[S.bes_n & 1];
+    PcBesideHalf *wr = &S.bes->half[(S.bes_n & 1) ^ 1];
+    const bool hold = par_beside_guard(S, rd, S.cl_n[0]);
+    if (blockIdx.x == 1) {
+        if (!hold) return;
+        const int pend = rd->head.pending;
+        par_pending_evidence(S, rd, est, smem);
+        if (threadIdx.x == 0) {
+            PcBesideEv e;
+            e.logZ = est[0]; e.logZ2 = est[1]; e.logZp = est[2]; e.logZXp = est[3]; e.logZp2 = est[4]; e.logZpXp = est[5];
+            e.lse_ref = est[6]; e.lse_sum = est[7]; e.live_logZ = est[8];
+            wr->ev = e;
+            if (pend) { S.bes->cnt.made += 1; S.bes->cnt.cyc += clock64() - c0; }
+        }
+        return;
+    }
+    if (hold) consume_par_body<PAR_RECORD>(S, nullptr, wr);
+    else {
+        par_pending_evidence(S, rd, est, smem);
+        consume_par_body<PAR_CATCH_UP>(S, est, wr);
+    }
+}
+__global__ __launch_bounds__(PAR_NT) void k_evidence_pending(PcState S)
+{
+    extern __shared__ __attribute__((aligned(16))) char smem[];
+    __shared__ double est[16];
+    const PcBesideHalf *rd = &S.bes->half[S.bes_n & 1];
+    const int pend = rd->head.pending;
+    if (pend) par_pending_evidence(S, rd, est, smem);
+    if (threadIdx.x == 0) {
+        PcCtl *ctl = S.ctl;
+        if (pend) {
+            ctl->logZ = est[0]; ctl->logZ2 = est[1]; S.logZp[0] = est[2]; S.logZXp[0] = est[3]; S.logZp2[0] = est[4]; S.logZpXp[0] = est[5];
+            S.lse_ref[0] = est[6]; S.lse_sum[0] = est[7];
+            if (S.use_prec) ctl->live_logZ = est[8];
+        }
+        ctl->bes_made = (int)S.bes->cnt.made; ctl->bes_kcyc = (int)(S.bes->cnt.cyc >> 10);
+    }
+}
+__global__ void k_beside_init(PcState S)
+{
+    if (threadIdx.x != 0 || blockIdx.x != 0) return;
+    PcBeside *b = S.bes;
+    for (int h = 0; h < 2; ++h) {
+        PcBesideHead &hd = b->half[h].head;
+        hd.pending = 0; hd.K = 0; hd.Kp = 0; hd.pad = 0; hd.Xp0 = S.logXp[0]; hd.XX0 = S.XpXq[0];
+        PcBesideEv &e = b->half[h].ev;
+        e.logZ = S.ctl->logZ; e.logZ2 = S.ctl->logZ2; e.logZp = S.logZp[0]; e.logZXp = S.logZXp[0]; e.logZp2 = S.logZp2[0]; e.logZpXp = S.logZpXp[0];
+        e.lse_ref = S.lse_ref[0]; e.lse_sum = S.lse_sum[0]; e.live_logZ = S.ctl->live_logZ;
+    }
+    b->cnt.made = 0; b->cnt.cyc = 0;
+}
 
 
 __device__ __forceinline__ void final_par_body(const PcState &S)
@@ -765,12 +938,32 @@
 #define PAR_STATIC_LDS 2048
 extern "C" int pc_par_fits(const PcState *S) { return par_lds(S) + PAR_STATIC_LDS <= 160 * 1024 && S->B <= PAR_NT; }
 
+#define PAR_BESIDE_STATIC_LDS 4096
+extern "C" int pc_par_beside_fits(const PcState *S) { return pc_par_fits(S) && par_lds(S) + PAR_BESIDE_STATIC_LDS <= 160 * 1024 && par_lds(S) >= PAR_PEND_LDS; }
+
 extern "C" int pc_launch_consume_par(const PcState *S, hipStream_t st)
 {
     const size_t sh = par_lds(S);
     if (sh + PAR_STATIC_LDS > 160 * 1024 || S->B > PAR_NT) return 1;
+    if (S->bes) {
+        if (!pc_par_beside_fits(S)) return 1;
+        pc_need_dyn_lds((const void *)k_consume_par_beside, sh);
+        hipLaunchKernelGGL(k_consume_par_beside, dim3(2), dim3(PAR_NT), sh, st, *S);
+        return 0;
+    }
     pc_need_dyn_lds((const void *)k_consume_par, sh);
     hipLaunchKernelGGL(k_consume_par, dim3(1), dim3(PAR_NT), sh, st, *S);
+    return 0;
+}
+extern "C" int pc_launch_beside_init(const PcState *S, hipStream_t st)
+{
+    hipLaunchKernelGGL(k_beside_init, dim3(1), dim3(64), 0, st, *S);
+    return 0;
+}
+extern "C" int pc_launch_evidence_pending(const PcState *S, hipStream_t st)
+{
+    pc_need_dyn_lds((const void *)k_evidence_pending, PAR_PEND_LDS);
+    hipLaunchKernelGGL(k_evidence_pending, dim3(1), dim3(PAR_NT), PAR_PEND_LDS, st, *S);
     return 0;
 }
 
diff --git a/polychordlite_amd/csrc/pc_state.h b/polychordlite_amd/csrc/pc_state.h
--- a/polychordlite_amd/csrc/pc_state.h
+++ b/polychordlite_amd/csrc/pc_state.h
@@ -7,7 +7,7 @@
 enum { PC_ABL_FUNCTOR = 1 << 0, PC_ABL_NO_POOL = 1 << 1, PC_ABL_NO_DEFER = 1 << 2, PC_ABL_NO_FUSED_UPDATE = 1 << 3, PC_ABL_PAIR_SCANS = 1 << 4,
        PC_ABL_CONSUME_GENERAL = 1 << 5, PC_ABL_SLICE_LANE = 1 << 6, PC_ABL_BASES_PACKED = 1 << 7, PC_ABL_CL_END_AT_DEATH = 1 << 8,
        PC_ABL_KILLOFF_GENERAL = 1 << 9, PC_ABL_CONSUME_CL_SERIAL = 1 << 10, PC_ABL_RETIRED_11 = 1 << 11, PC_ABL_RETIRED_12 = 1 << 12,
-       PC_ABL_NO_HELPER = 1 << 13, PC_ABL_QC_BY_CHAIN = 1 << 14, PC_ABL_RTC_BUILTINS = 1 << 15, PC_ABL_UPDATE_CHAIN = 1 << 16, PC_ABL_TRACE_CHOL = 1 << 30 };
+       PC_ABL_NO_HELPER = 1 << 13, PC_ABL_QC_BY_CHAIN = 1 << 14, PC_ABL_RTC_BUILTINS = 1 << 15, PC_ABL_UPDATE_CHAIN = 1 << 16, PC_ABL_EVIDENCE_INLINE = 1 << 17, PC_ABL_TRACE_CHOL = 1 << 30 };
 
 #define PC_MASK_WORDS 16
 
@@ -40,9 +40,11 @@
     int upd_tmark;
     int upd_T, upd_ts;
     int upd_nph0;
-    int upd_keep_thr, upd_pad;
+    int upd_keep_thr;
+    int bes_made;
     double upd_thr;
-    int chol_suspect, chol_pad;
+    int chol_suspect;
+    int bes_kcyc;
     long long wave_cyc[4];
 };
 
@@ -67,6 +69,26 @@
     unsigned long long ph_mask[PC_MASK_WORDS];
 };
 static_assert(sizeof(PcPlanHead) == 64 && sizeof(PcPlan) == 64 + 8 * PC_MASK_WORDS, "plan record layout");
+
+#define PC_BES_N 1024
+struct alignas(128) PcBesideEv {
+    double logZ, logZ2, logZp, logZXp, logZp2, logZpXp, lse_ref, lse_sum, live_logZ;
+};
+struct alignas(128) PcBesideHead {
+    int pending;
+    int K, Kp;
+    int pad;
+    double Xp0, XX0;
+};
+struct alignas(128) PcBesideHalf {
+    PcBesideHead head;
+    PcBesideEv ev;
+    alignas(128) double L[PC_BES_N];
+    alignas(128) double Ladd[PC_BES_N];
+    alignas(128) int didx[PC_BES_N];
+};
+struct alignas(128) PcBesideCount { long long made, cyc; };
+struct PcBeside { PcBesideHalf half[2]; PcBesideCount cnt; };
 
 struct PcState {
     int D, nDer, nT, nr, N, Ncap, B, maxc, Pcap, Dcap;
@@ -137,6 +159,7 @@
     PcCtl *ctl_host; unsigned notify_seq;
     int src_id, src_pad;
     const double *src_data; long long src_ndata;
+    PcBeside *bes; int bes_n, bes_pad;
 };
 
 struct PcManyRec { PcState S; void *p[10]; int ia[6]; int pad[2]; };
@@ -155,7 +178,7 @@
     typedef __attribute__((address_space(1))) char gchar;
     return (T *)(gchar *)(uintptr_t)p;
 }
-static_assert(sizeof(PcState) == 968, "PcState changed: add the new pointer members to pc_many_state, then update this size");
+static_assert(sizeof(PcState) == 984, "PcState changed: add the new pointer members to pc_many_state, then update this size");
 __device__ __forceinline__ PcState pc_many_state(const PcManyRec *R, int run)
 {
     PcState S = R[run].S;
@@ -168,7 +191,7 @@
     G(babies); G(baby_logL); G(baby_logL_T); G(ch_cluster); G(ch_epoch); G(ch_nlike); G(ch_seed_slot); G(ch_contour);
     G(nhat); G(nhat_w); G(nhat_raw); G(nhat_Ms); G(ch_My); G(plan); G(sort_slot); G(sort_key);
     G(slot_src); G(slot_dead); G(slot_step); G(ch_nlike_g); G(logn); G(nn_list); G(nn_slot_owner); G(nn_chain_slot);
-    G(nn_pts); G(nn_code); G(ctl); G(ctl_host); G(src_data);
+    G(nn_pts); G(nn_code); G(ctl); G(ctl_host); G(src_data); G(bes);
 #undef G
     return S;
 }
```

Result: no change. 1.328 billion likelihood evals/s, median of 3 (+0.5%).
